# cherise215/advchain

Hardware: AMD Instinct MI355X
Metric: augmented images/sec (N adv steps, chain=noise+bias+morph+affine) (higher is better)
Workload: dtype f32

## Files before the change

advchain_amd/_lib.py:

```python
import ctypes
import os
from ctypes import c_char_p, c_double, c_float, c_int, c_int64, c_void_p

_HERE = os.path.dirname(os.path.abspath(__file__))
LIB_PATH = os.path.join(_HERE, "csrc", "libadvchain_hip.so")

_P, _I, _L, _F, _D = c_void_p, c_int, c_int64, c_float, c_double

PROTOTYPES = {
    "advchain_version": (_I, []),
    "advchain_last_error": (c_char_p, []),
    "advchain_set_deterministic": (None, [_I]),
    "advchain_get_deterministic": (_I, []),
    "advchain_grid_sample_fwd": (_I, [_P, _P, _P, _L, _L, _I, _P, _P, _I, _I, _I, _P]),
    "advchain_grid_sample_fwd_ride": (_I, [_P, _P, _P, _P, _P, _L, _L, _I, _P, _P, _I, _I, _I, _I, _P]),
    "advchain_scatter_workspace": (_L, [_L, _I, _P]),
    "advchain_grid_sample_bwd": (_I, [_P, _P, _P, _P, _P, _P, _L, _L, _I, _P, _P, _I, _I, _I, _I, _P]),
    "advchain_window_stage_workspace": (_L, [_L, _L, _I, _P]),
    "advchain_grid_sample_bwd_staged": (_I, [_P, _P, _P, _P, _P, _P, _L, _L, _I, _P, _P, _I, _I, _I, _I, _P, _P]),
    "advchain_last_bwd_route": (_I, []),
    "advchain_det_warp_workspace": (_L, [_L, _L, _I, _P]),
    "advchain_grid_sample_bwd_det": (_I, [_P, _P, _P, _P, _P, _P, _L, _L, _I, _P, _P, _I, _I, _I, _P]),
    "advchain_compose_self_fwd": (_I, [_P, _P, _P, _L, _I, _P, _I, _P, _P]),
    "advchain_compose_self_bwd": (_I, [_P, _P, _P, _P, _I, _I, _L, _I, _P, _P]),
    "advchain_affine_warp_fwd": (_I, [_P, _P, _P, _L, _L, _I, _P, _I, _I, _P]),
    "advchain_affine_warp_fwd_ride": (_I, [_P, _P, _P, _P, _P, _L, _L, _I, _P, _I, _I, _I, _P]),
    "advchain_affine_warp_bwd_workspace": (_L, [_L, _I, _P]),
    "advchain_affine_warp_bwd": (_I, [_P, _P, _P, _P, _P, _P, _L, _L, _I, _P, _I, _I, _P]),
    "advchain_affine_warp_bwd_det": (_I, [_P, _P, _P, _P, _P, _P, _P, _L, _L, _I, _P, _I, _I, _P]),
    "advchain_affine_theta_fwd": (_I, [_P, _P, _F, _P, _P, _L, _I, _P]),
    "advchain_affine_theta_bwd": (_I, [_P, _P, _F, _P, _P, _P, _L, _I, _P]),
    "advchain_tp_interp_fwd": (_I, [_P, _P, _P, _P, _P, _P, _P, _L, _L, _I, _I, _F, _P, _P, _P]),
    "advchain_tp_interp_fwd_smoothed_pair": (_I, [_P, _P, _P, _P, _P, _P, _P, _P, _L, _L, _I, _F, _P, _P, _F, _P]),
    "advchain_band_reduce_axis": (_I, [_P, _P, _P, _P, _P, _P, _P, _P, _I, _L, _L, _F, _P]),
    "advchain_band_reduce_rows_dense": (_I, [_P, _P, _P, _P, _P, _L, _L, _L, _L, _F, _P]),
    "advchain_bias_field_fwd": (_I, [_P, _P, _P, _P, _P, _P, _P, _P, _P, _L, _L, _F, _I, _F, _P]),
    "advchain_bias_field_bwd": (_I, [_P, _P, _P, _P, _P, _P, _P, _P, _P, _P, _L, _L, _F, _I, _F, _P]),
    "advchain_bias_rows_per_wg": (_I, [_P, _L]),
    "advchain_bias_field_fwd_rows": (_I, [_P, _P, _P, _P, _P, _P, _P, _P, _P, _L, _L, _F, _I, _F, _I, _P]),
    "advchain_bias_field_bwd_rows": (_I, [_P, _P, _P, _P, _P, _P, _P, _P, _P, _P, _L, _L, _F, _I, _F, _I, _P]),
    "advchain_bias_field_bwd_reduced": (_I, [_P, _P, _P, _P, _P, _P, _P, _P, _P, _P, _L, _L, _F, _I, _F, _P, _P, _L, _I, _P]),
    "advchain_gauss_axis": (_I, [_P, _P, _P, _L, _L, _I, _P, _I, _P, _I, _I, _F, _P]),
    "advchain_gauss_axis_generic": (_I, [_P, _P, _L, _I, _P, _I, _P, _I, _F, _P]),
    "advchain_max_displacement": (_I, [_P, _P, _L, _I, _P, _P]),
    "advchain_grid_sample_bicubic2d_fwd": (_I, [_P, _P, _P, _L, _L, _P, _P, _I, _P]),
    "advchain_grid_sample_bicubic2d_bwd": (_I, [_P, _P, _P, _P, _P, _L, _L, _P, _P, _I, _P]),
    "advchain_affine_grid2d_fwd": (_I, [_P, _P, _L, _P, _P]),
    "advchain_affine_grid2d_bwd_workspace": (_L, [_L, _P]),
    "advchain_affine_grid2d_bwd": (_I, [_P, _P, _P, _L, _P, _P]),
    "advchain_slot_rows_max": (_I, [_P, _P, _L, _L, _I, _P]),
    "advchain_demons_compose_pair_fwd": (_I, [_P, _P, _P, _P, _P, _P, _P, _P, _P, _P, _P, _P, _P, _L, _I, _I, _P, _P, _F, _F, _I, _P]),
    "advchain_demons_compose_pair_bwd": (_I, [_P, _P, _P, _P, _P, _P, _P, _P, _P, _P, _P, _P, _P, _P, _P, _P, _P, _L, _P, _P, _P, _L,
                                              _I, _I, _P, _F, _F, _P]),
    "advchain_bounds_check": (_I, [_P, _P, _P, _L, _P, _P]),
    "advchain_expo_chain_fused_levels": (_I, [_L, _I, _P, _I, _P]),
    "advchain_expo_chain_fwd": (_I, [_P, _P, _P, _L, _I, _P, _I, _P, _P, _P, _P]),
    "advchain_expo_chain_bwd": (_I, [_P, _P, _P, _P, _P, _P, _P, _L, _I, _P, _I, _P]),
    "advchain_gauss_xy": (_I, [_P, _P, _P, _L, _L, _I, _P, _P, _I, _I, _F, _P, _P, _L]),
    "advchain_gauss_xy_staged": (_I, [_P, _P, _P, _L, _L, _I, _P, _P, _I, _I, _F, _P, _P, _L]),
    "advchain_gauss_xy_lanes": (_I, [_P, _P, _P, _L, _L, _I, _P, _P, _I, _I, _F, _P, _P, _L, _I, _I]),
    "advchain_gauss_xy_plan": (_I, [_I, _P, _L, _P, _P, _P]),
    "advchain_gauss_small": (_I, [_P, _P, _L, _I, _P, _P, _I, _F, _P]),
    "advchain_gauss_small_pair": (_I, [_P, _P, _L, _I, _P, _P, _F, _I, _P]),
    "advchain_axpy": (_I, [_P, _P, _P, _F, _L, _P]),
    "advchain_sign_axpy": (_I, [_P, _P, _P, _F, _L, _P, _P, _P]),
    "advchain_nonzero_mask": (_I, [_P, _P, _L, _P]),
    "advchain_consistency_finish": (_I, [_P, _P, _P, _P, _I, _P]),
    "advchain_norm_workspace": (_L, [_L, _L]),
    "advchain_norm_axpy": (_I, [_P, _P, _P, _P, _F, _L, _L, _P]),
    "advchain_norm_axpy_gated": (_I, [_P, _P, _P, _P, _F, _L, _L, _P, _P, _P]),
    "advchain_update_multi": (_I, [_P, _I, _P, _P]),
    "advchain_consistency_fwd": (_I, [_P, _P, _P, _P, _P, _P, _P, _L, _L, _I, _P, _I, _I, _I, _I, _P]),
    "advchain_consistency_bwd": (_I, [_P, _P, _P, _P, _P, _P, _F, _F, _F, _F, _I, _L, _L, _I, _P, _I, _P]),
    "advchain_consistency_fused_fwd": (_I, [_P, _P, _P, _P, _P, _L, _L, _I, _P, _I, _I, _I, _I, _P]),
    "advchain_consistency_fused_bwd": (_I, [_P, _P, _P, _P, _P, _P, _F, _F, _F, _F, _I, _L, _L, _I, _P, _I, _P]),
    "advchain_consistency_wide_fwd": (_I, [_P, _P, _P, _P, _P, _P, _L, _L, _I, _P, _I, _I, _I, _I, _P]),
    "advchain_consistency_wide_bwd": (_I, [_P, _P, _P, _P, _P, _P, _P, _F, _F, _F, _F, _I, _L, _L, _I, _P, _I, _P]),
    "advchain_consistency_ref_bwd": (_I, [_P, _P, _P, _P, _P, _P, _P, _F, _F, _F, _F, _I, _L, _L, _I, _P, _I, _P]),
    "advchain_set_ref_grad_reg_max_k": (None, [_I]),
    "advchain_get_ref_grad_reg_max_k": (_I, []),
    "advchain_consistency_lp_fwd": (_I, [_P, _I, _P, _I, _P, _P, _P, _P, _L, _L, _I, _P, _I, _I, _I, _I, _P]),
    "advchain_consistency_lp_bwd": (_I, [_P, _I, _P, _I, _P, _P, _P, _P, _P, _F, _F, _F, _F, _I, _L, _L, _I, _P, _I, _P]),
    "advchain_consistency_lp_ref_bwd": (_I, [_P, _I, _P, _I, _P, _P, _P, _P, _P, _F, _F, _F, _F, _I, _L, _L, _I, _P, _I, _P]),
    "advchain_consistency_cw_fwd": (_I, [_P, _I, _P, _I, _P, _P, _P, _P, _L, _L, _I, _P, _I, _I, _I, _I, _P, _P]),
    "advchain_consistency_cw_bwd": (_I, [_P, _I, _P, _I, _P, _P, _P, _P, _P, _F, _F, _F, _F, _I, _L, _L, _I, _P, _I, _P, _P]),
    "advchain_consistency_cw_ref_bwd": (_I, [_P, _I, _P, _I, _P, _P, _P, _P, _P, _F, _F, _F, _F, _I, _L, _L, _I, _P, _I, _P, _P]),
    "advchain_consistency_fused_fwd_bf16": (_I, [_P, _P, _P, _P, _P, _L, _L, _I, _P, _P]),
    "advchain_consistency_fused_bwd_bf16": (_I, [_P, _P, _P, _P, _P, _P, _F, _F, _F, _L, _L, _I, _P, _P]),
    "advchain_seg_loss_workspace": (_L, [_L, _I, _P]),
    "advchain_ce2d_fwd": (_I, [_P, _I, _P, _P, _P, _P, _P, _P, _L, _L, _P, _F, _P]),
    "advchain_ce2d_bwd": (_I, [_P, _I, _P, _P, _P, _P, _P, _P, _P, _L, _L, _P, _F, _P]),
    "advchain_contour_fwd": (_I, [_P, _P, _P, _P, _P, _P, _P, _L, _L, _I, _P, _I, _I, _P]),
    "advchain_contour_bwd": (_I, [_P, _P, _P, _P, _L, _L, _I, _P, _I, _P]),
    "advchain_one_hot": (_I, [_P, _P, _L, _L, _L, _P]),
    "advchain_dice_workspace": (_L, [_L, _L, _I, _P]),
    "advchain_dice_fwd": (_I, [_P, _I, _P, _P, _P, _P, _P, _P, _P, _L, _L, _I, _P, _I, _F, _F, _F, _P]),
    "advchain_dice_bwd": (_I, [_P, _I, _P, _P, _P, _P, _P, _P, _P, _P, _L, _L, _I, _P, _F, _F, _P]),
    "advchain_edt": (_I, [_P, _I, _P, _I, _P, _L, _I, _P, _P]),
    "advchain_signed_maps_workspace": (_L, [_L, _L, _I, _P]),
    "advchain_signed_maps": (_I, [_P, _P, _P, _P, _L, _L, _I, _P, _P]),
    "advchain_surface_metrics_workspace": (_L, [_L, _L, _I, _P]),
    "advchain_surface_metrics": (_I, [_P, _P, _P, _D, _P, _P, _P, _P, _P, _P, _P, _P, _P, _L, _L, _I, _P, _P]),
    "advchain_surface_dice_route": (_I, [_L, _L, _I, _P, _P, _D, _I]),
    "advchain_surface_dice_workspace": (_L, [_L, _L, _I, _P, _P, _D, _I]),
    "advchain_surface_dice": (_I, [_P, _P, _P, _P, _D, _I, _P, _P, _P, _P, _L, _L, _I, _P, _P]),
    "advchain_components_workspace": (_L, [_L, _I, _P]),
    "advchain_components": (_I, [_P, _P, _P, _P, _P, _L, _I, _P, _I, _L, _L, _P]),
    "advchain_keep_largest": (_I, [_P, _P, _P, _P, _L, _L, _I, _P, _I, _L, _P]),
    "advchain_remove_small": (_I, [_P, _P, _P, _L, _I, _P, _I, _L, _L, _L, _P]),
    "advchain_fill_holes_workspace": (_L, [_L, _I, _P]),
    "advchain_fill_holes": (_I, [_P, _P, _P, _P, _P, _P, _L, _L, _I, _P, _I, _L, _L, _P]),
    "advchain_instance_match_workspace": (_L, [_L, _I, _P]),
    "advchain_instance_match": (_I, [_P] * 14 + [_L, _L, _I, _P, _I, _L, _D, _P]),
    "advchain_betti_workspace": (_L, [_L, _I, _P]),
    "advchain_betti": (_I, [_P, _P, _P, _P, _P, _P, _L, _L, _I, _P, _I, _P]),
    "advchain_morph_workspace": (_L, [_I, _L, _L, _I, _P]),
    "advchain_morph": (_I, [_P, _P, _D, _I, _P, _P, _L, _L, _L, _I, _P, _P]),
    "advchain_boundary_workspace": (_L, [_L, _L, _I, _P]),
    "advchain_boundary_fwd": (_I, [_P, _I, _P, _P, _P, _P, _P, _P, _L, _L, _I, _P, _I, _P]),
    "advchain_boundary_bwd": (_I, [_P, _I, _P, _P, _P, _P, _P, _P, _L, _L, _I, _P, _I, _P]),
    "advchain_image_diff2d_fwd": (_I, [_P, _P, _P, _L, _L, _P, _P]),
    "advchain_image_diff2d_bwd": (_I, [_P, _P, _P, _L, _L, _P, _P]),
    "advchain_jacobian_det2d_fwd": (_I, [_P, _P, _L, _P, _P]),
    "advchain_jacobian_det2d_bwd": (_I, [_P, _P, _P, _L, _P, _P]),
    "advchain_expo_start": (_I, [_P, _P, _F, _L, _I, _P, _P]),
    "advchain_image_diff3d_fwd": (_I, [_P, _P, _P, _P, _L, _L, _P, _P]),
    "advchain_image_diff3d_bwd": (_I, [_P, _P, _P, _P, _L, _L, _P, _P]),
    "advchain_jacobian_det_fwd": (_I, [_P, _P, _L, _I, _P, _I, _P]),
    "advchain_jacobian_det_bwd": (_I, [_P, _P, _P, _P, _L, _I, _P, _I, _P]),
    "advchain_jacobian_det_workspace": (_L, [_L, _I, _P]),
    "advchain_jacobian_stats_workspace": (_L, [_L, _I, _P]),
    "advchain_jacobian_stats": (_I, [_P, _P, _P, _P, _P, _P, _L, _I, _P, _I, _P]),
    "advchain_sumsq_ordered": (_I, [_P, _L, _P, _P, _P]),
    "advchain_bicubic2d_det_workspace": (_L, [_L, _L, _P]),
    "advchain_grid_sample_bicubic2d_bwd_det": (_I, [_P, _P, _P, _P, _P, _P, _L, _L, _P, _P, _I, _P]),
    "advchain_tp_interp_sumsq_partials": (_L, [_P, _L]),
    "advchain_tp_interp_sumsq_ordered": (_I, [_P, _P, _P, _P, _P, _P, _L, _L, _P, _P, _P]),
    "advchain_consistency_fwd_partials": (_L, [_L, _L, _I, _P, _I, _I, _I]),
    "advchain_consistency_fwd_ord": (_I, [_P, _P, _P, _P, _P, _P, _P, _L, _P, _L, _L, _I, _P, _I, _I, _I, _I, _P]),
    "advchain_consistency_fused_fwd_partials": (_L, [_L, _L, _I, _P, _I, _I, _I, _I]),
    "advchain_consistency_fused_fwd_ord": (_I, [_P, _P, _P, _P, _P, _L, _P, _L, _L, _I, _P, _I, _I, _I, _I, _P]),
    "advchain_consistency_wide_fwd_partials": (_L, [_L, _L, _I, _P, _I, _I]),
    "advchain_consistency_wide_fwd_ord": (_I, [_P, _P, _P, _P, _P, _P, _L, _P, _L, _L, _I, _P, _I, _I, _I, _I, _P]),
    "advchain_consistency_lp_fwd_partials": (_L, [_L, _L, _I, _P, _I]),
    "advchain_consistency_lp_fwd_ord": (_I, [_P, _I, _P, _I, _P, _P, _P, _P, _L, _P, _L, _L, _I, _P, _I, _I, _I, _I, _P, _P]),
    "advchain_consistency_finish_ord": (_I, [_P, _L, _P, _P, _P, _P, _P]),
}

class UpdateDesc(ctypes.Structure):
    _fields_ = [("base", c_void_p), ("x", c_void_p), ("out", c_void_p), ("old", c_void_p), ("N", c_int64), ("M", c_int64),
                ("kind", ctypes.c_int32), ("step", c_float)]


_lib = None


class AdvchainHipError(RuntimeError):
    pass


class _Lib(object):

    def __init__(self, cdll):
        self._cdll = cdll
        self._raw = {}
        self.records = []

    def _bind(self, name, res, args):
        fn = getattr(self._cdll, name)
        fn.restype = res
        fn.argtypes = args
        self._raw[name] = fn
        setattr(self, name, fn)

    def timed(self, names=None, every=1):
        import contextlib
        import torch

        @contextlib.contextmanager
        def ctx():
            chosen = [n for n in self._raw if (names is None or n in names) and self._raw[n].restype is c_int
                      and len(self._raw[n].argtypes) > 0]
            for n in chosen:
                raw = self._raw[n]

                count = [0]

                def wrapped(*a, _raw=raw, _n=n, _count=count):
                    _count[0] += 1
                    if _count[0] % every:
                        return _raw(*a)
                    e0 = torch.cuda.Event(enable_timing=True)
                    e1 = torch.cuda.Event(enable_timing=True)
                    e0.record()
                    rc = _raw(*a)
                    e1.record()
                    self.records.append((_n, a, e0, e1))
                    return rc
                setattr(self, n, wrapped)
            try:
                yield self
            finally:
                for n in chosen:
                    setattr(self, n, self._raw[n])
        return ctx()


def load():
    global _lib
    if _lib is not None:
        return _lib
    if not os.path.exists(LIB_PATH):
        raise AdvchainHipError(
            "libadvchain_hip.so not found at %s -- build it with `python -m advchain_amd.build` "
            "(there is no CPU / PyTorch fallback for the advchain_amd kernels)" % LIB_PATH)
    import torch
    tl = os.path.join(os.path.dirname(torch.__file__), "lib", "libamdhip64.so")
    if os.path.exists(tl):
        ctypes.CDLL(tl, mode=ctypes.RTLD_GLOBAL)
    lib = _Lib(ctypes.CDLL(LIB_PATH))
    for name, (res, args) in PROTOTYPES.items():
        lib._bind(name, res, args)
    _lib = lib
    return lib


def check(rc, what):
    if rc != 0:
        msg = load().advchain_last_error()
        raise AdvchainHipError("%s failed (rc=%d): %s" % (what, rc, msg.decode() if msg else ""))


_DIMS = {}


def dims_array(dims):
    key = tuple(dims)
    arr = _DIMS.get(key)
    if arr is None:
        arr = _DIMS[key] = (c_int64 * len(key))(*[int(d) for d in key])
    return arr


def float_array(vals):
    return (c_float * len(vals))(*[float(v) for v in vals])
```

advchain_amd/csrc/fields.hip:

```cpp
#include "sampler_common.h"

namespace advchain {

constexpr int kBandMax = 8;

struct BandAxis {
  const int* start;
  const float* w;
  const int* lo;
  const int* hi;
  int S, g, B;
};
struct BandTables { BandAxis a[3]; };

__device__ __forceinline__ void decode3(int v, const Dims& d, int& i0, int& i1, int& i2) {
  i2 = v % d.s2;
  const int r = v / d.s2;
  i1 = r % d.s1;
  i0 = r / d.s1;
}

__device__ __forceinline__ float tp_eval(const float* __restrict__ coef, const BandTables& T, int i0, int i1, int i2) {
  const BandAxis& A0 = T.a[0];
  const BandAxis& A1 = T.a[1];
  const BandAxis& A2 = T.a[2];
  const int s0 = A0.start[i0], s1 = A1.start[i1], s2 = A2.start[i2];
  const float* w0 = A0.w + i0 * A0.B;
  const float* w1 = A1.w + i1 * A1.B;
  const float* w2 = A2.w + i2 * A2.B;
  float acc = 0.f;
  for (int a = 0; a < A0.B; ++a) {
    float acc1 = 0.f;
    for (int b = 0; b < A1.B; ++b) {
      const float* row = coef + ((int64_t)(s0 + a) * A1.g + (s1 + b)) * A2.g + s2;
      float acc2 = 0.f;
      for (int c = 0; c < A2.B; ++c) acc2 += row[c] * w2[c];
      acc1 += acc2 * w1[b];
    }
    acc += acc1 * w0[a];
  }
  return acc;
}

constexpr int kTpChunk = 32;
constexpr int kTpMaxLds = 2048;

struct TpGeom { int XT, ROWS; };

__host__ __device__ inline TpGeom tp_geom(int S2) {
  TpGeom g;
  (void)S2;
  g.XT = 64;
  g.ROWS = kBlock / g.XT;
  return g;
}

template <int VEC, class Epi>
__device__ __forceinline__ void tp_rows(const float* __restrict__ coef, const BandTables& T, const Dims& full, int i0,
                                        int i1_begin, int i1_end, float* lds, Epi&& epi) {
  const BandAxis& A0 = T.a[0];
  const BandAxis& A1 = T.a[1];
  const BandAxis& A2 = T.a[2];
  const int ncol = full.s2 / VEC;
  int XT = 64;
  if (VEC > 1) { XT = 1; while (XT < ncol && XT < 64) XT *= 2; }
  const int ROWS = kBlock / XT;
  const int tx = threadIdx.x % XT, ry = threadIdx.x / XT;
  const int g2 = A2.g;
  __shared__ int s1_s[kTpChunk];
  __shared__ float w1_s[kTpChunk * kBandMax];
  const int nrow = i1_end - i1_begin;
  for (int e = threadIdx.x; e < nrow * (A1.B + 1); e += kBlock) {
    const int r = e / (A1.B + 1), b = e - r * (A1.B + 1);
    if (b == 0) s1_s[r] = A1.start[i1_begin + r];
    else w1_s[r * kBandMax + b - 1] = A1.w[(i1_begin + r) * A1.B + b - 1];
  }
  const int s0 = A0.start[i0];
  const float* w0 = A0.w + i0 * A0.B;
  int s2f[VEC];
  float w2f[VEC][kBandMax];
#pragma unroll
  for (int q = 0; q < VEC; ++q) {
    const int col = min(tx * VEC + q, full.s2 - 1);
    s2f[q] = A2.start[col];
#pragma unroll
    for (int c = 0; c < kBandMax; ++c) w2f[q][c] = c < A2.B ? A2.w[col * A2.B + c] : 0.f;
  }
  __syncthreads();
  const int RPP = max(1, min(kTpChunk, kTpMaxLds / max(g2, 1)));
  for (int base = i1_begin; base < i1_end; base += RPP) {
    for (int e = threadIdx.x; e < RPP * g2; e += kBlock) {
      const int r = e / g2, k = e - r * g2;
      const int i1 = base + r;
      float acc = 0.f;
      if (i1 < i1_end) {
        const int s1 = s1_s[i1 - i1_begin];
        const float* w1 = w1_s + (i1 - i1_begin) * kBandMax;
        if (A0.B == 2 && A1.B == 2) {
          const float* cb = coef + ((int64_t)s0 * A1.g + s1) * g2 + k;
          const float c00 = cb[0], c01 = cb[g2], c10 = cb[(int64_t)A1.g * g2], c11 = cb[(int64_t)A1.g * g2 + g2];
          const float u0 = w1[0], u1 = w1[1], v0 = w0[0], v1 = w0[1];
          acc += v0 * (0.f + u0 * c00 + u1 * c01);
          acc += v1 * (0.f + u0 * c10 + u1 * c11);
        } else {
          for (int a = 0; a < A0.B; ++a) {
            float acc1 = 0.f;
            for (int b = 0; b < A1.B; ++b) acc1 += w1[b] * coef[((int64_t)(s0 + a) * A1.g + (s1 + b)) * g2 + k];
            acc += w0[a] * acc1;
          }
        }
      }
      lds[e] = acc;
    }
    __syncthreads();
    for (int xg = tx; xg < ncol; xg += XT) {
      int s2[VEC];
      float w2[VEC][kBandMax];
#pragma unroll
      for (int q = 0; q < VEC; ++q) {
        if (xg == tx) {
          s2[q] = s2f[q];
#pragma unroll
          for (int c = 0; c < kBandMax; ++c) w2[q][c] = w2f[q][c];
        } else {
          s2[q] = A2.start[xg * VEC + q];
#pragma unroll
          for (int c = 0; c < kBandMax; ++c) w2[q][c] = c < A2.B ? A2.w[(xg * VEC + q) * A2.B + c] : 0.f;
        }
      }
      for (int r = ry; r < RPP; r += ROWS) {
        const int i1 = base + r;
        if (i1 >= i1_end) break;
        float val[VEC];
#pragma unroll
        for (int q = 0; q < VEC; ++q) {
          float v = 0.f;
#pragma unroll
          for (int c = 0; c < kBandMax; ++c)
            if (c < A2.B) v += w2[q][c] * lds[r * g2 + s2[q] + c];
          val[q] = v;
        }
        epi(i1, xg * VEC, val);
      }
    }
    __syncthreads();
  }
}

struct SumsqOrdered {};
template <class... ORD>
__device__ __forceinline__ void tp_sumsq_put(float* __restrict__ sumsq, float v) {
  if constexpr (sizeof...(ORD) == 0)
    atomic_add_f32(sumsq + (blockIdx.x + blockIdx.y * 3u + blockIdx.z * 7u) % kSumSlots, v);
  else
    sumsq[((int64_t)blockIdx.z * gridDim.y + blockIdx.y) * gridDim.x + blockIdx.x] = v;
}
static __global__ void __launch_bounds__(kBlock) k_tp_partials_sum(const float* __restrict__ partials, int64_t nb, float* __restrict__ out) {
  __shared__ float smem[4];
  float v[1] = {0.f};
  for (int64_t i = threadIdx.x; i < nb; i += kBlock) v[0] += partials[i];
  block_sum<1>(v, smem);
  if (threadIdx.x == 0) out[0] = v[0];
}

template <int VEC, class... ORD>
__global__ void __launch_bounds__(kBlock)
k_tp_interp_fwd(const float* __restrict__ coef, float* __restrict__ out, BandTables T, Dims full, int C,
                int add_identity, float scale, float* __restrict__ sumsq, float* __restrict__ disp_out) {
  __shared__ float lds[kTpMaxLds];
  __shared__ float smem[4];
  const int plane = blockIdx.z, i0 = blockIdx.y;
  const int i1b = blockIdx.x * kTpChunk, i1e = min(i1b + kTpChunk, full.s1);
  const int64_t G = (int64_t)T.a[0].g * T.a[1].g * T.a[2].g;
  const int V = (int)full.voxels();
  const int c = plane % C;
  float sq[1] = {0.f};
  float dmax = 0.f;
  const float to_vox = fabsf(scale) * 0.5f * (float)((c == 0 ? full.s2 : (c == 1 ? full.s1 : full.s0)) - 1);
  tp_rows<VEC>(coef + (int64_t)plane * G, T, full, i0, i1b, i1e, lds, [&](int i1, int x, const float (&val)[VEC]) {
    float o[VEC];
#pragma unroll
    for (int q = 0; q < VEC; ++q) {
      sq[0] += val[q] * val[q];
      dmax = fmaxf(dmax, fabsf(val[q]));
      float base = 0.f;
      if (add_identity) base = c == 0 ? lin_coord(x + q, full.s2) : (c == 1 ? lin_coord(i1, full.s1) : lin_coord(i0, full.s0));
      o[q] = base + scale * val[q];
    }
    if (out) store_vec<VEC>(out + (int64_t)plane * V + ((int64_t)i0 * full.s1 + i1) * full.s2 + x, o);
  });
  if (disp_out) wave_max_to_slots(fminf(dmax * to_vox, 1.0e9f), disp_out);
  if (sumsq) {
    block_sum<1>(sq, smem);
    if (threadIdx.x == 0) tp_sumsq_put<ORD...>(sumsq, sq[0]);
  }
}

constexpr int kGsFuseMax = 1024;
struct GaussW9 { float w[9]; };
template <int VEC>
__global__ void __launch_bounds__(kBlock)
k_tp_interp_fwd_gs(const float* __restrict__ vel, float* __restrict__ s1, float* __restrict__ out, BandTables T, Dims full, int C,
                   int add_identity, float scale, float* __restrict__ disp_out, GaussW9 gw, float gscale, int P) {
  __shared__ float lds[kTpMaxLds];
  __shared__ float gs[2][kGsFuseMax];
  const int plane = blockIdx.z, i0 = blockIdx.y;
  const int i1b = blockIdx.x * kTpChunk, i1e = min(i1b + kTpChunk, full.s1);
  const int g1 = T.a[1].g, g2 = T.a[2].g, Vg = g1 * g2;
  const int V = (int)full.voxels();
  const int c = plane % C;
  {
    const float* src = vel + (int64_t)(plane % P) * Vg;
    const float sc = plane >= P ? -gscale : gscale;
    for (int i = threadIdx.x; i < Vg; i += kBlock) gs[0][i] = src[i] * sc;
    __syncthreads();
    int cur = 0;
#pragma unroll
    for (int pass = 0; pass < 2; ++pass) {
      const int Sa = pass == 0 ? g2 : g1, st = pass == 0 ? 1 : g2;
      for (int i = threadIdx.x; i < Vg; i += kBlock) {
        const int ia = (i / st) % Sa;
        float acc = 0.f;
#pragma unroll
        for (int k = -4; k <= 4; ++k) {
          const int j = ia + k;
          if (j >= 0 && j < Sa) acc += gw.w[k + 4] * gs[cur][i + k * st];
        }
        gs[cur ^ 1][i] = acc;
      }
      __syncthreads();
      cur ^= 1;
    }
    if (s1 && blockIdx.x == 0 && blockIdx.y == 0)
      for (int i = threadIdx.x; i < Vg; i += kBlock) s1[(int64_t)plane * Vg + i] = gs[0][i];
  }
  float dmax = 0.f;
  const float to_vox = fabsf(scale) * 0.5f * (float)((c == 0 ? full.s2 : (c == 1 ? full.s1 : full.s0)) - 1);
  tp_rows<VEC>(gs[0], T, full, i0, i1b, i1e, lds, [&](int i1, int x, const float (&val)[VEC]) {
    float o[VEC];
#pragma unroll
    for (int q = 0; q < VEC; ++q) {
      dmax = fmaxf(dmax, fabsf(val[q]));
      float base = 0.f;
      if (add_identity) base = c == 0 ? lin_coord(x + q, full.s2) : (c == 1 ? lin_coord(i1, full.s1) : lin_coord(i0, full.s0));
      o[q] = base + scale * val[q];
    }
    store_vec<VEC>(out + (int64_t)plane * V + ((int64_t)i0 * full.s1 + i1) * full.s2 + x, o);
  });
  if (disp_out) wave_max_to_slots(fminf(dmax * to_vox, 1.0e9f), disp_out);
}

constexpr int kTpZB = 4;
template <int VEC, class... ORD>
__global__ void __launch_bounds__(kBlock)
k_tp_interp_fwd_planes(const float* __restrict__ coef, float* __restrict__ out, BandTables T, Dims full, int C, int add_identity,
                       float scale, float* __restrict__ sumsq, float* __restrict__ disp_out) {
  __shared__ float lds[2][kTpMaxLds];
  __shared__ int s1_s[kTpChunk], s0_s[kTpZB];
  __shared__ float w1_s[kTpChunk * 2], w0_s[kTpZB * 2];
  __shared__ float smem[4];
  const BandAxis& A0 = T.a[0];
  const BandAxis& A1 = T.a[1];
  const BandAxis& A2 = T.a[2];
  const int plane = blockIdx.z;
  const int z0 = blockIdx.y * kTpZB, z1 = min(z0 + kTpZB, full.s0);
  const int i1b = blockIdx.x * kTpChunk, i1e = min(i1b + kTpChunk, full.s1);
  const int64_t G = (int64_t)A0.g * A1.g * A2.g;
  const int V = (int)full.voxels();
  const int c = plane % C;
  const float* cf = coef + (int64_t)plane * G;
  const int g2 = A2.g, nrow = i1e - i1b, NE = nrow * g2;
  constexpr int EPT = kTpMaxLds / kBlock;
  const int ncol = full.s2 / VEC;
  int XT = 64;
  if (VEC > 1) { XT = 1; while (XT < ncol && XT < 64) XT *= 2; }
  const int ROWS = kBlock / XT;
  const int tx = threadIdx.x % XT, ry = threadIdx.x / XT;
  for (int e = threadIdx.x; e < nrow * 3; e += kBlock) {
    const int r = e / 3, b = e - r * 3;
    if (b == 0) s1_s[r] = A1.start[i1b + r];
    else w1_s[r * 2 + b - 1] = A1.w[(i1b + r) * 2 + b - 1];
  }
  if (threadIdx.x < (z1 - z0) * 3) {
    const int r = threadIdx.x / 3, b = threadIdx.x - r * 3;
    if (b == 0) s0_s[r] = A0.start[z0 + r];
    else w0_s[r * 2 + b - 1] = A0.w[(z0 + r) * 2 + b - 1];
  }
  int s2f[VEC];
  float w2f[VEC][2];
#pragma unroll
  for (int q = 0; q < VEC; ++q) {
    const int col = min(tx * VEC + q, full.s2 - 1);
    s2f[q] = A2.start[col];
    w2f[q][0] = A2.w[col * 2];
    w2f[q][1] = A2.w[col * 2 + 1];
  }
  __syncthreads();
  float cc[EPT][4];
  auto request = [&](int zi) {
    const int s0 = s0_s[zi];
#pragma unroll
    for (int j = 0; j < EPT; ++j) {
      if (j * kBlock >= NE) break;
      const int e = min(threadIdx.x + j * kBlock, NE - 1);
      const int r = e / g2, k = e - r * g2;
      const float* cb = cf + ((int64_t)s0 * A1.g + s1_s[r]) * g2 + k;
      cc[j][0] = cb[0]; cc[j][1] = cb[g2]; cc[j][2] = cb[(int64_t)A1.g * g2]; cc[j][3] = cb[(int64_t)A1.g * g2 + g2];
    }
  };
  auto blend = [&](int zi, float* dst) {
    const float v0 = w0_s[zi * 2], v1 = w0_s[zi * 2 + 1];
#pragma unroll
    for (int j = 0; j < EPT; ++j) {
      const int e = threadIdx.x + j * kBlock;
      if (e >= NE) continue;
      const int r = e / g2;
      const float u0 = w1_s[r * 2], u1 = w1_s[r * 2 + 1];
      float acc = 0.f;
      acc += v0 * (0.f + u0 * cc[j][0] + u1 * cc[j][1]);
      acc += v1 * (0.f + u0 * cc[j][2] + u1 * cc[j][3]);
      dst[e] = acc;
    }
  };
  float sq[1] = {0.f};
  float dmax = 0.f;
  const bool track = sumsq != nullptr || disp_out != nullptr;
  const float to_vox = fabsf(scale) * 0.5f * (float)((c == 0 ? full.s2 : (c == 1 ? full.s1 : full.s0)) - 1);
  request(0);
  blend(0, lds[0]);
  __syncthreads();
  for (int zi = 0; zi < z1 - z0; ++zi) {
    const int i0 = z0 + zi;
    const float* cur = lds[zi & 1];
    const bool more = zi + 1 < z1 - z0;
    if (more) request(zi + 1);
    for (int xg = tx; xg < ncol; xg += XT) {
      int s2[VEC];
      float w2[VEC][2];
#pragma unroll
      for (int q = 0; q < VEC; ++q) {
        if (xg == tx) { s2[q] = s2f[q]; w2[q][0] = w2f[q][0]; w2[q][1] = w2f[q][1]; }
        else { s2[q] = A2.start[xg * VEC + q]; w2[q][0] = A2.w[(xg * VEC + q) * 2]; w2[q][1] = A2.w[(xg * VEC + q) * 2 + 1]; }
      }
      float basex[VEC];
#pragma unroll
      for (int q = 0; q < VEC; ++q) basex[q] = (add_identity && c == 0) ? lin_coord(xg * VEC + q, full.s2) : 0.f;
      const float basez = (add_identity && c == 2) ? lin_coord(i0, full.s0) : 0.f;
      float* orow = out ? out + (int64_t)plane * V + ((int64_t)i0 * full.s1 + i1b) * full.s2 + xg * VEC : nullptr;
      for (int r = ry; r < nrow; r += ROWS) {
        const float basey = (add_identity && c == 1) ? lin_coord(i1b + r, full.s1) : basez;
        const float* lr = cur + r * g2;
        float o[VEC];
#pragma unroll
        for (int q = 0; q < VEC; ++q) {
          float v = 0.f;
          v += w2[q][0] * lr[s2[q]];
          v += w2[q][1] * lr[s2[q] + 1];
          if (track) {
            sq[0] += v * v;
            dmax = fmaxf(dmax, fabsf(v));
          }
          o[q] = (c == 0 ? basex[q] : basey) + scale * v;
        }
        if (out) store_vec<VEC>(orow + r * full.s2, o);
      }
    }
    if (more) blend(zi + 1, lds[(zi + 1) & 1]);
    __syncthreads();
  }
  if (disp_out) wave_max_to_slots(fminf(dmax * to_vox, 1.0e9f), disp_out);
  if (sumsq) {
    block_sum<1>(sq, smem);
    if (threadIdx.x == 0) tp_sumsq_put<ORD...>(sumsq, sq[0]);
  }
}

constexpr int kBrMaxW = 4096;

__device__ __forceinline__ int stage_band(const BandAxis& A, float* Wd, int* lo_s) {
  const int lane = threadIdx.x & 63;
  if (A.g > 64) return 0;
  int WB = lane < A.g ? A.hi[lane] - A.lo[lane] : 0;
#pragma unroll
  for (int o = 32; o > 0; o >>= 1) WB = max(WB, __shfl_xor(WB, o, 64));
  if (A.g * WB > kBrMaxW) return 0;
  for (int i = threadIdx.x; i < A.g * WB; i += blockDim.x) {
    const int k = i / WB, j = i - k * WB;
    const int s2 = A.lo[k] + j;
    float w = 0.f;
    if (s2 < A.hi[k]) {
      const int b = k - A.start[s2];
      if (b >= 0 && b < A.B) w = A.w[s2 * A.B + b];
    }
    Wd[i] = w;
  }
  for (int i = threadIdx.x; i < A.g; i += blockDim.x) lo_s[i] = A.lo[i];
  __syncthreads();
  return WB;
}

__global__ void __launch_bounds__(kBlock)
k_band_reduce_axis(const float* __restrict__ in, const float* __restrict__ in2, float* __restrict__ out, int64_t outer,
                   int inner, BandAxis A, float scale) {
  __shared__ float Wd[kBrMaxW];
  __shared__ int lo_s[64];
  const int WB = stage_band(A, Wd, lo_s);
  const int64_t t = (int64_t)blockIdx.x * kBlock + threadIdx.x;
  const int64_t total = outer * A.g * inner;
  if (t >= total) return;
  const int i = (int)(t % inner);
  const int64_t r = t / inner;
  const int k = (int)(r % A.g);
  const int64_t o = r / A.g;
  const float* p = in + (o * A.S) * inner + i;
  const float* p2 = in2 ? in2 + (o * A.S) * inner + i : nullptr;
  float acc = 0.f;
  if (WB > 0) {
    const int lo = lo_s[k];
    const int len = min(WB, A.S - lo);
    const float* w = Wd + k * WB;
    for (int j = 0; j < len; ++j) {
      float x = p[(int64_t)(lo + j) * inner];
      if (p2) x -= p2[(int64_t)(lo + j) * inner];
      acc = fmaf(x, w[j], acc);
    }
  } else {
    const int lo = A.lo[k], hi = A.hi[k];
    for (int s = lo; s < hi; ++s) {
      const int b = k - A.start[s];
      if (b >= 0 && b < A.B) {
        float x = p[(int64_t)s * inner];
        if (p2) x -= p2[(int64_t)s * inner];
        acc += x * A.w[s * A.B + b];
      }
    }
  }
  out[t] = acc * scale;
}

constexpr int kBrSlabFloats = 12288;
__global__ void __launch_bounds__(kBlock)
k_band_reduce_axis_slab(const float* __restrict__ in, const float* __restrict__ in2, float* __restrict__ out, int inner, int IC,
                        BandAxis A, float scale) {
  extern __shared__ __attribute__((aligned(16))) float slab[];
  __shared__ float Wd[kBrMaxW];
  __shared__ int lo_s[64];
  const int64_t o = blockIdx.x;
  const int c0 = blockIdx.y * IC, cols = min(IC, inner - c0);
  const int q = cols >> 2, n4 = A.S * q, pitch = IC + 1;
  const float* p = in + o * (int64_t)A.S * inner + c0;
  const float* p2 = in2 ? in2 + o * (int64_t)A.S * inner + c0 : nullptr;
  constexpr int U = 4;
  float4 v[U];
  auto fetch = [&](int idx) -> float4 {
    const int e = min(idx, n4 - 1);
    const int sr = e / q, x4 = e - sr * q;
    float4 a = *reinterpret_cast<const float4*>(p + (int64_t)sr * inner + 4 * x4);
    if (p2) {
      const float4 b = *reinterpret_cast<const float4*>(p2 + (int64_t)sr * inner + 4 * x4);
      a.x -= b.x; a.y -= b.y; a.z -= b.z; a.w -= b.w;
    }
    return a;
  };
  auto put = [&](int idx, const float4& a) {
    if (idx >= n4) return;
    const int sr = idx / q, x4 = idx - sr * q;
    float* dst = slab + sr * pitch + 4 * x4;
    dst[0] = a.x; dst[1] = a.y; dst[2] = a.z; dst[3] = a.w;
  };
#pragma unroll
  for (int u = 0; u < U; ++u) v[u] = fetch(threadIdx.x + u * kBlock);
  const int WB = stage_band(A, Wd, lo_s);
#pragma unroll
  for (int u = 0; u < U; ++u) put(threadIdx.x + u * kBlock, v[u]);
  for (int i0 = threadIdx.x + U * kBlock; i0 < n4; i0 += U * kBlock) {
#pragma unroll
    for (int u = 0; u < U; ++u) v[u] = fetch(i0 + u * kBlock);
#pragma unroll
    for (int u = 0; u < U; ++u) put(i0 + u * kBlock, v[u]);
  }
  __syncthreads();
  for (int t = threadIdx.x; t < A.g * cols; t += kBlock) {
    const int k = t / cols, i = t - k * cols;
    float acc = 0.f;
    if (WB > 0) {
      const int lo = lo_s[k];
      const int len = min(WB, A.S - lo);
      const float* w = Wd + k * WB;
      const float* x = slab + lo * pitch + i;
      for (int j = 0; j < len; ++j) acc = fmaf(x[j * pitch], w[j], acc);
    } else {
      const int lo = A.lo[k], hi = A.hi[k];
      for (int sr = lo; sr < hi; ++sr) {
        const int b = k - A.start[sr];
        if (b >= 0 && b < A.B) acc += slab[sr * pitch + i] * A.w[sr * A.B + b];
      }
    }
    out[(o * A.g + k) * (int64_t)inner + c0 + i] = acc * scale;
  }
}

constexpr int kBrThreads = 128;
template <int KG>
__global__ void __launch_bounds__(kBrThreads)
k_band_reduce_rows(const float* __restrict__ in, const float* __restrict__ in2, float* __restrict__ out, int64_t rows,
                   BandAxis A, float scale, int iters) {
  extern __shared__ __attribute__((aligned(16))) float slabs[];
  __shared__ float Wd[kBrMaxW];
  __shared__ int lo_s[64];
  constexpr int RW = 64 / KG, NWV = kBrThreads / 64;
  const int lane = threadIdx.x & 63, wave = threadIdx.x >> 6;
  const int S = A.S, g = A.g, B = A.B;
  const int WB = stage_band(A, Wd, lo_s);
  const bool dense = WB > 0;
  const int q = S >> 2;
  const int pitch = S + 1;
  float* my = slabs + wave * RW * pitch;
  const int r = lane % RW, kg = lane / RW;
  for (int it = 0; it < iters; ++it) {
    const int64_t base = (((int64_t)blockIdx.x * iters + it) * NWV + wave) * RW;
    __syncthreads();
    for (int idx = lane; idx < RW * q; idx += 64) {
      const int rr = idx / q, x4 = idx - rr * q;
      const int64_t gr = base + rr;
      float4 v = make_float4(0.f, 0.f, 0.f, 0.f);
      if (gr < rows) {
        v = *reinterpret_cast<const float4*>(in + gr * S + 4 * x4);
        if (in2) {
          const float4 u = *reinterpret_cast<const float4*>(in2 + gr * S + 4 * x4);
          v = make_float4(v.x - u.x, v.y - u.y, v.z - u.z, v.w - u.w);
        }
      }
      float* dst = my + rr * pitch + 4 * x4;
      dst[0] = v.x; dst[1] = v.y; dst[2] = v.z; dst[3] = v.w;
    }
    __syncthreads();
    const int64_t gr = base + r;
    if (gr < rows) {
      const float* x = my + r * pitch;
      if (dense) {
        for (int k0 = kg; k0 < g; k0 += 2 * KG) {
          const int k1 = k0 + KG;
          const bool two = k1 < g;
          const int lo0 = lo_s[k0], lo1 = lo_s[two ? k1 : k0];
          const float* w0 = Wd + k0 * WB;
          const float* w1 = Wd + (two ? k1 : k0) * WB;
          float a0 = 0.f, a1 = 0.f;
          int j = 0;
          for (; j + 8 <= WB; j += 8) {
            float x0[8], x1[8], c0[8], c1[8];
#pragma unroll
            for (int u = 0; u < 8; ++u) {
              x0[u] = x[min(lo0 + j + u, S - 1)]; c0[u] = w0[j + u];
              x1[u] = x[min(lo1 + j + u, S - 1)]; c1[u] = w1[j + u];
            }
#pragma unroll
            for (int u = 0; u < 8; ++u) { a0 = fmaf(x0[u], c0[u], a0); a1 = fmaf(x1[u], c1[u], a1); }
          }
          for (; j < WB; ++j) {
            a0 = fmaf(x[min(lo0 + j, S - 1)], w0[j], a0);
            a1 = fmaf(x[min(lo1 + j, S - 1)], w1[j], a1);
          }
          out[gr * g + k0] = a0 * scale;
          if (two) out[gr * g + k1] = a1 * scale;
        }
      } else
      for (int k = kg; k < g; k += KG) {
        const int lo = A.lo[k];
        float acc = 0.f;
        {
          for (int s2 = lo; s2 < A.hi[k]; ++s2) {
            const int b = k - A.start[s2];
            if (b >= 0 && b < B) acc = fmaf(x[s2], A.w[s2 * B + b], acc);
          }
        }
        out[gr * g + k] = acc * scale;
      }
    }
  }
}

template <int KG>
__global__ void __launch_bounds__(kBrThreads)
k_band_reduce_rows_dense(const float* __restrict__ in, const float* __restrict__ in2, float* __restrict__ out, int64_t rows,
                         const float* __restrict__ wd, const int* __restrict__ lo_g, int S, int g, int WB, float scale, int iters) {
  extern __shared__ __attribute__((aligned(16))) float slabs[];
  __shared__ int lo_s[64];
  constexpr int RW = 64 / KG, NWV = kBrThreads / 64;
  constexpr int QMAX = 8;
  const int lane = threadIdx.x & 63, wave = threadIdx.x >> 6;
  const int q = S >> 2;
  const int pitch = S + 1;
  float* my = slabs + wave * RW * pitch;
  float* Wd = slabs + NWV * RW * pitch;
  const int r = lane % RW, kg = lane / RW;
  const int nq = RW * q;
  float4 v[QMAX];
  auto request = [&](int it) {
    const int64_t base = (((int64_t)blockIdx.x * iters + it) * NWV + wave) * RW;
#pragma unroll
    for (int u = 0; u < QMAX; ++u) {
      const int idx = lane + 64 * u;
      const int rr = idx / q, x4 = idx - rr * q;
      const int64_t gr = base + rr;
      const bool ok = idx < nq && gr < rows;
      const int64_t off = ok ? gr * S + 4 * x4 : 0;
      float4 a = *reinterpret_cast<const float4*>(in + off);
      if (in2) {
        const float4 b = *reinterpret_cast<const float4*>(in2 + off);
        a = make_float4(a.x - b.x, a.y - b.y, a.z - b.z, a.w - b.w);
      }
      v[u] = ok ? a : make_float4(0.f, 0.f, 0.f, 0.f);
    }
  };
  request(0);
  for (int i = threadIdx.x; i < g * WB; i += kBrThreads) Wd[i] = wd[i];
  if (threadIdx.x < g) lo_s[threadIdx.x] = lo_g[threadIdx.x];
  for (int it = 0; it < iters; ++it) {
    const int64_t base = (((int64_t)blockIdx.x * iters + it) * NWV + wave) * RW;
    if (it > 0) __syncthreads();
#pragma unroll
    for (int u = 0; u < QMAX; ++u) {
      const int idx = lane + 64 * u;
      if (idx >= nq) continue;
      const int rr = idx / q, x4 = idx - rr * q;
      float* dst = my + rr * pitch + 4 * x4;
      dst[0] = v[u].x; dst[1] = v[u].y; dst[2] = v[u].z; dst[3] = v[u].w;
    }
    __syncthreads();
    if (it + 1 < iters) request(it + 1);
    const int64_t gr = base + r;
    if (gr < rows) {
      const float* x = my + r * pitch;
      for (int k0 = kg; k0 < g; k0 += 2 * KG) {
        const int k1 = k0 + KG;
        const bool two = k1 < g;
        const int lo0 = lo_s[k0], lo1 = lo_s[two ? k1 : k0];
        const float* w0 = Wd + k0 * WB;
        const float* w1 = Wd + (two ? k1 : k0) * WB;
        float a0 = 0.f, a1 = 0.f;
        int j = 0;
        for (; j + 8 <= WB; j += 8) {
          float x0[8], x1[8], c0[8], c1[8];
#pragma unroll
          for (int u = 0; u < 8; ++u) {
            x0[u] = x[min(lo0 + j + u, S - 1)]; c0[u] = w0[j + u];
            x1[u] = x[min(lo1 + j + u, S - 1)]; c1[u] = w1[j + u];
          }
#pragma unroll
          for (int u = 0; u < 8; ++u) { a0 = fmaf(x0[u], c0[u], a0); a1 = fmaf(x1[u], c1[u], a1); }
        }
        for (; j < WB; ++j) {
          a0 = fmaf(x[min(lo0 + j, S - 1)], w0[j], a0);
          a1 = fmaf(x[min(lo1 + j, S - 1)], w1[j], a1);
        }
        out[gr * g + k0] = a0 * scale;
        if (two) out[gr * g + k1] = a1 * scale;
      }
    }
  }
}

__device__ __forceinline__ float bias_value(float L, int use_log, float eps, float& e, bool& pass) {
  e = use_log ? expf(L) : 1.f + L;
  const float b = e - 1.f;
  pass = (b >= -eps) && (b <= eps);
  return 1.f + fminf(fmaxf(b, -eps), eps);
}

template <int VEC>
__global__ void __launch_bounds__(kBlock)
k_bias_fwd(const float* __restrict__ cp, const float* __restrict__ data, float* __restrict__ out,
           float* __restrict__ field, BandTables T, Dims full, int C, float eps, int use_log, float cp_scale, int rows) {
  __shared__ float lds[kTpMaxLds];
  const int n = blockIdx.z, i0 = blockIdx.y;
  const int i1b = blockIdx.x * rows, i1e = min(i1b + rows, full.s1);
  const int64_t G = (int64_t)T.a[0].g * T.a[1].g * T.a[2].g;
  const int V = (int)full.voxels();
  tp_rows<VEC>(cp + (int64_t)n * G, T, full, i0, i1b, i1e, lds, [&](int i1, int x, const float (&val)[VEC]) {
    const int v = (i0 * full.s1 + i1) * full.s2 + x;
    float b[VEC];
#pragma unroll
    for (int q = 0; q < VEC; ++q) {
      float e;
      bool pass;
      b[q] = bias_value(cp_scale * val[q], use_log, eps, e, pass);
    }
    store_vec<VEC>(field + (int64_t)n * V + v, b);
    if (data) {
      for (int c = 0; c < C; ++c) {
        const int64_t o = ((int64_t)n * C + c) * V + v;
        float dv[VEC];
        load_vec<VEC>(data + o, dv);
#pragma unroll
        for (int q = 0; q < VEC; ++q) dv[q] *= b[q];
        store_vec<VEC>(out + o, dv);
      }
    }
  });
}

constexpr int kBiasRedWq = kBrMaxW / 4 / kBlock;
template <int VEC, bool RED>
__global__ void __launch_bounds__(kBlock)
k_bias_bwd(const float* __restrict__ cp, const float* __restrict__ data, const float* __restrict__ gout,
           float* __restrict__ gL, float* __restrict__ gdata, BandTables T, Dims full, int C, float eps, int use_log,
           float cp_scale, int rows, float* __restrict__ t1, const float* __restrict__ wd, const int* __restrict__ lo_g, int WB) {
  __shared__ float lds[kTpMaxLds];
  extern __shared__ __attribute__((aligned(16))) float red_lds[];
  __shared__ int lo_s[64];
  const int n = blockIdx.z, i0 = blockIdx.y;
  const int i1b = blockIdx.x * rows, i1e = min(i1b + rows, full.s1);
  const int64_t G = (int64_t)T.a[0].g * T.a[1].g * T.a[2].g;
  const int V = (int)full.voxels();
  const int g2 = T.a[2].g;
  const int nw = RED ? g2 * WB : 0;
  const int pitch = full.s2 + 1;
  float* Wd = red_lds;
  float* slab = red_lds + ((nw + 3) & ~3);
  const bool wvec = (nw & 3) == 0 && (reinterpret_cast<uintptr_t>(wd) & 15) == 0;
  float4 wq[kBiasRedWq];
  int lo_r = 0;
  if constexpr (RED) {
#pragma unroll
    for (int u = 0; u < kBiasRedWq; ++u) {
      const int idx = threadIdx.x + kBlock * u;
      wq[u] = wvec && 4 * idx < nw ? *reinterpret_cast<const float4*>(wd + 4 * idx) : make_float4(0.f, 0.f, 0.f, 0.f);
    }
    if (threadIdx.x < g2) lo_r = lo_g[threadIdx.x];
  }
  tp_rows<VEC>(cp + (int64_t)n * G, T, full, i0, i1b, i1e, lds, [&](int i1, int x, const float (&val)[VEC]) {
    const int v = (i0 * full.s1 + i1) * full.s2 + x;
    float b[VEC], e[VEC], sgo[VEC];
    bool pass[VEC];
#pragma unroll
    for (int q = 0; q < VEC; ++q) {
      b[q] = bias_value(cp_scale * val[q], use_log, eps, e[q], pass[q]);
      sgo[q] = 0.f;
    }
    for (int c = 0; c < C; ++c) {
      const int64_t o = ((int64_t)n * C + c) * V + v;
      float go[VEC], dv[VEC];
      load_vec<VEC>(gout + o, go);
      load_vec<VEC>(data + o, dv);
#pragma unroll
      for (int q = 0; q < VEC; ++q) { sgo[q] += go[q] * dv[q]; go[q] *= b[q]; }
      if (gdata) store_vec<VEC>(gdata + o, go);
    }
    if (RED || gL) {
      float gl[VEC];
#pragma unroll
      for (int q = 0; q < VEC; ++q) gl[q] = pass[q] ? sgo[q] * (use_log ? e[q] : 1.f) * cp_scale : 0.f;
      if constexpr (RED) {
        float* dst = slab + (i1 - i1b) * pitch + x;
#pragma unroll
        for (int q = 0; q < VEC; ++q) dst[q] = gl[q];
      } else {
        store_vec<VEC>(gL + (int64_t)n * V + v, gl);
      }
    }
  });
  if constexpr (RED) {
    if (wvec) {
#pragma unroll
      for (int u = 0; u < kBiasRedWq; ++u) {
        const int idx = threadIdx.x + kBlock * u;
        if (4 * idx < nw) *reinterpret_cast<float4*>(Wd + 4 * idx) = wq[u];
      }
    } else {
      for (int i = threadIdx.x; i < nw; i += kBlock) Wd[i] = wd[i];
    }
    if (threadIdx.x < g2) lo_s[threadIdx.x] = lo_r;
    __syncthreads();
    const int nrow = i1e - i1b, S2 = full.s2;
    for (int e = threadIdx.x; e < nrow * g2; e += kBlock) {
      const int r = e % nrow, k = e / nrow;
      const float* x = slab + r * pitch;
      const float* w = Wd + k * WB;
      const int lo = lo_s[k];
      float a = 0.f;
      int j = 0;
      for (; j + 16 <= WB; j += 16) {
        float xv[16], cv[16];
#pragma unroll
        for (int u = 0; u < 16; ++u) { xv[u] = x[min(lo + j + u, S2 - 1)]; cv[u] = w[j + u]; }
#pragma unroll
        for (int u = 0; u < 16; ++u) a = fmaf(xv[u], cv[u], a);
      }
      for (; j < WB; ++j) a = fmaf(x[min(lo + j, S2 - 1)], w[j], a);
      t1[(((int64_t)n * full.s0 + i0) * full.s1 + i1b + r) * g2 + k] = a;
    }
  }
}

struct GaussW { float w[9]; };

__device__ __forceinline__ float border_identity(float pos, int S, float& slope) {
  float mult;
  const float x = source_index<PAD_BORDER>(pos, S, mult);
  const float f = floorf(x);
  const int i0 = (int)f;
  const int i1 = min(i0 + 1, S - 1);
  const float a = lin_coord(i0, S), b = lin_coord(i1, S);
  slope = mult * (b - a);
  return ((f + 1.f) - x) * a + (x - f) * b;
}

template <int PRE, int POST>
__global__ void __launch_bounds__(kBlock)
k_gauss_axis(const float* __restrict__ in, float* __restrict__ out, const float* __restrict__ aux, int64_t total,
             Dims d, int C, int axis, GaussW gw, float scale) {
  const int64_t t = (int64_t)blockIdx.x * kBlock + threadIdx.x;
  if (t >= total) return;
  const int V = (int)d.voxels();
  const int plane = (int)(t / V);
  const int v = (int)(t - (int64_t)plane * V);
  int idx[3];
  decode3(v, d, idx[0], idx[1], idx[2]);
  const int S[3] = {d.s0, d.s1, d.s2};
  const int stride = axis == 2 ? 1 : (axis == 1 ? d.s2 : d.s1 * d.s2);
  const int c = plane % C;
  const int caxis = 2 - c;
  const int ia = idx[axis];
  float tap[9];
#pragma unroll
  for (int k = -4; k <= 4; ++k) {
    const int jc = min(max(ia + k, 0), S[axis] - 1);
    tap[k + 4] = in[t + (int64_t)(jc - ia) * stride];
  }
  float acc = 0.f;
#pragma unroll
  for (int k = -4; k <= 4; ++k) {
    const int j = ia + k;
    float x = tap[k + 4];
    if (PRE == 1) x *= scale;
    if (PRE == 2) {
      const int ci = (caxis == axis) ? j : idx[caxis];
      float slope;
      x = border_identity(x, S[caxis], slope) - lin_coord(ci, S[caxis]);
    }
    acc += (j >= 0 && j < S[axis]) ? gw.w[k + 4] * x : 0.f;
  }
  if (POST == 1) acc += lin_coord(idx[caxis], S[caxis]);
  if (POST == 2) {
    float slope;
    border_identity(aux[t], S[caxis], slope);
    acc *= slope;
  }
  out[t] = acc;
}

template <int PRE, int POST, int AXIS>
__global__ void __launch_bounds__(kBlock)
k_gauss_axis_v4(const float* __restrict__ in, float* __restrict__ out, const float* __restrict__ aux, int64_t total4,
                Dims d, int C, GaussW gw, float scale, int row_in_wave) {
  const int64_t t4 = (int64_t)blockIdx.x * kBlock + threadIdx.x;
  int64_t t;
  if (AXIS == 2 && row_in_wave == 2) {
    const int q = d.s2 >> 2, rpw = 64 / q;
    const int lane = (int)(t4 & 63);
    const int rl = lane / q;
    const int64_t row = (t4 >> 6) * rpw + rl;
    if (rl >= rpw || row >= total4 / q) return;
    t = row * d.s2 + (lane - rl * q) * 4;
  } else {
    if (t4 >= total4) return;
    t = t4 * 4;
  }
  const int V = (int)d.voxels();
  const int plane = (int)(t / V);
  const int v = (int)(t - (int64_t)plane * V);
  int idx[3];
  decode3(v, d, idx[0], idx[1], idx[2]);
  const int S[3] = {d.s0, d.s1, d.s2};
  const int c = plane % C;
  const int caxis = 2 - c;
  auto pre = [&](float x, int i0, int i1, int i2) -> float {
    if (PRE == 1) return x * scale;
    if (PRE == 2) {
      const int ci = caxis == 2 ? i2 : (caxis == 1 ? i1 : i0);
      float slope;
      return border_identity(x, S[caxis], slope) - lin_coord(ci, S[caxis]);
    }
    return x;
  };
  float acc[4] = {0.f, 0.f, 0.f, 0.f};
  if (AXIS == 2 && row_in_wave) {
    const float4 q = *reinterpret_cast<const float4*>(in + t);
    float win[12];
    win[4] = pre(q.x, idx[0], idx[1], idx[2]);
    win[5] = pre(q.y, idx[0], idx[1], idx[2] + 1);
    win[6] = pre(q.z, idx[0], idx[1], idx[2] + 2);
    win[7] = pre(q.w, idx[0], idx[1], idx[2] + 3);
    const bool first = idx[2] == 0, last = idx[2] + 4 >= d.s2;
#pragma unroll
    for (int k = 0; k < 4; ++k) {
      const float pv = lane_prev_f(win[4 + k]), nx = lane_next_f(win[4 + k]);
      win[k] = first ? 0.f : pv;
      win[8 + k] = last ? 0.f : nx;
    }
#pragma unroll
    for (int o = 0; o < 4; ++o)
#pragma unroll
      for (int k = 0; k < 9; ++k) acc[o] += gw.w[k] * win[o + k];
  } else if (AXIS == 2) {
    float win[12];
    float4 qb[3];
#pragma unroll
    for (int b = 0; b < 3; ++b) {
      const int x0 = idx[2] + (b - 1) * 4;
      qb[b] = *reinterpret_cast<const float4*>(in + t + ((x0 >= 0 && x0 < d.s2) ? (b - 1) * 4 : 0));
    }
#pragma unroll
    for (int b = 0; b < 3; ++b) {
      const int x0 = idx[2] + (b - 1) * 4;
      const bool inr = x0 >= 0 && x0 < d.s2;
      win[b * 4 + 0] = inr ? pre(qb[b].x, idx[0], idx[1], x0) : 0.f;
      win[b * 4 + 1] = inr ? pre(qb[b].y, idx[0], idx[1], x0 + 1) : 0.f;
      win[b * 4 + 2] = inr ? pre(qb[b].z, idx[0], idx[1], x0 + 2) : 0.f;
      win[b * 4 + 3] = inr ? pre(qb[b].w, idx[0], idx[1], x0 + 3) : 0.f;
    }
#pragma unroll
    for (int o = 0; o < 4; ++o)
#pragma unroll
      for (int k = 0; k < 9; ++k) acc[o] += gw.w[k] * win[o + k];
  } else {
    const int stride = AXIS == 1 ? d.s2 : d.s1 * d.s2;
    const int ia = idx[AXIS];
    float4 q[9];
#pragma unroll
    for (int k = -4; k <= 4; ++k) {
      const int jc = min(max(ia + k, 0), S[AXIS] - 1);
      q[k + 4] = *reinterpret_cast<const float4*>(in + t + (int64_t)(jc - ia) * stride);
    }
#pragma unroll
    for (int k = -4; k <= 4; ++k) {
      const int j = ia + k;
      const bool inr = j >= 0 && j < S[AXIS];
      const int j0 = AXIS == 0 ? j : idx[0], j1 = AXIS == 1 ? j : idx[1];
      const float w = gw.w[k + 4];
      acc[0] += inr ? w * pre(q[k + 4].x, j0, j1, idx[2]) : 0.f;
      acc[1] += inr ? w * pre(q[k + 4].y, j0, j1, idx[2] + 1) : 0.f;
      acc[2] += inr ? w * pre(q[k + 4].z, j0, j1, idx[2] + 2) : 0.f;
      acc[3] += inr ? w * pre(q[k + 4].w, j0, j1, idx[2] + 3) : 0.f;
    }
  }
  if (POST == 1) {
#pragma unroll
    for (int o = 0; o < 4; ++o) acc[o] += lin_coord(caxis == 2 ? idx[2] + o : idx[caxis], S[caxis]);
  }
  if (POST == 2) {
    const float4 a = *reinterpret_cast<const float4*>(aux + t);
    const float av[4] = {a.x, a.y, a.z, a.w};
#pragma unroll
    for (int o = 0; o < 4; ++o) {
      float slope;
      border_identity(av[o], S[caxis], slope);
      acc[o] *= slope;
    }
  }
  *reinterpret_cast<float4*>(out + t) = make_float4(acc[0], acc[1], acc[2], acc[3]);
}

template <int PRE, int POST>
__global__ void __launch_bounds__(kBlock)
k_gauss_xy(const float* __restrict__ in, float* __restrict__ out, const float* __restrict__ aux, Dims d, int C, GaussW gw,
           float scale, int TY, const float* __restrict__ in_hi, int planes_lo) {
  extern __shared__ float gx_lds[];
  const int W = d.s2, Q = W >> 2, PA = W + 8;
  const int R = TY + 8;
  float* A = gx_lds;
  float* B = gx_lds + R * PA;
  const int plane = blockIdx.z, iz = blockIdx.y;
  const int y0 = blockIdx.x * TY;
  const int caxis = 2 - plane % C;
  const int Sc = caxis == 2 ? d.s2 : (caxis == 1 ? d.s1 : d.s0);
  const int64_t base = ((int64_t)plane * d.s0 + iz) * d.s1 * (int64_t)W;
  const float* src = (in_hi && plane >= planes_lo) ? in_hi + (((int64_t)(plane - planes_lo) * d.s0 + iz) * d.s1 * (int64_t)W) : in + base;
  for (int e = threadIdx.x; e < R * 2; e += kBlock)
    *reinterpret_cast<float4*>(A + (e >> 1) * PA + ((e & 1) ? W + 4 : 0)) = make_float4(0.f, 0.f, 0.f, 0.f);
  for (int e = threadIdx.x; e < R * Q; e += kBlock) {
    const int r = e / Q, q = e - r * Q;
    const int gy = y0 - 4 + r;
    const bool inr = gy >= 0 && gy < d.s1;
    const float4 v = *reinterpret_cast<const float4*>(src + (int64_t)min(max(gy, 0), d.s1 - 1) * W + 4 * q);
    float t[4] = {v.x, v.y, v.z, v.w};
#pragma unroll
    for (int o = 0; o < 4; ++o) {
      if (PRE == 1) t[o] *= scale;
      if (PRE == 2) {
        float sl;
        t[o] = border_identity(t[o], Sc, sl) - lin_coord(caxis == 2 ? 4 * q + o : (caxis == 1 ? gy : iz), Sc);
      }
      if (!inr) t[o] = 0.f;
    }
    *reinterpret_cast<float4*>(A + r * PA + 4 + 4 * q) = make_float4(t[0], t[1], t[2], t[3]);
  }
  __syncthreads();
  for (int e = threadIdx.x; e < R * Q; e += kBlock) {
    const int r = e / Q, q = e - r * Q;
    const float* a = A + r * PA + 4 * q;
    const float4 a0 = *reinterpret_cast<const float4*>(a), a1 = *reinterpret_cast<const float4*>(a + 4),
                 a2 = *reinterpret_cast<const float4*>(a + 8);
    const float win[12] = {a0.x, a0.y, a0.z, a0.w, a1.x, a1.y, a1.z, a1.w, a2.x, a2.y, a2.z, a2.w};
    float acc[4] = {0.f, 0.f, 0.f, 0.f};
#pragma unroll
    for (int o = 0; o < 4; ++o)
#pragma unroll
      for (int k = 0; k < 9; ++k) acc[o] += gw.w[k] * win[o + k];
    *reinterpret_cast<float4*>(B + r * W + 4 * q) = make_float4(acc[0], acc[1], acc[2], acc[3]);
  }
  __syncthreads();
  for (int e = threadIdx.x; e < TY * Q; e += kBlock) {
    const int ry = e / Q, q = e - ry * Q;
    const int gy = y0 + ry;
    if (gy >= d.s1) continue;
    float acc[4] = {0.f, 0.f, 0.f, 0.f};
#pragma unroll
    for (int k = 0; k < 9; ++k) {
      const float4 b = *reinterpret_cast<const float4*>(B + (ry + k) * W + 4 * q);
      acc[0] += gw.w[k] * b.x; acc[1] += gw.w[k] * b.y; acc[2] += gw.w[k] * b.z; acc[3] += gw.w[k] * b.w;
    }
    const int64_t off = base + (int64_t)gy * W + 4 * q;
    if (POST == 1) {
#pragma unroll
      for (int o = 0; o < 4; ++o) acc[o] += lin_coord(caxis == 2 ? 4 * q + o : (caxis == 1 ? gy : iz), Sc);
    }
    if (POST == 2) {
      const float4 a4 = *reinterpret_cast<const float4*>(aux + off);
      const float av[4] = {a4.x, a4.y, a4.z, a4.w};
#pragma unroll
      for (int o = 0; o < 4; ++o) {
        float slope;
        border_identity(av[o], Sc, slope);
// ... 136 lines not shown
  for (int j0 = ja; j0 < jb; j0 += U) {
    float4 nw[U];
#pragma unroll
    for (int u = 0; u < U; ++u) nw[u] = fetch(j0 + 4 + u);
#pragma unroll
    for (int u = 0; u < U; ++u) w[8 + u] = prep(nw[u], j0 + 4 + u);
#pragma unroll
    for (int u = 0; u < U; ++u) {
      const int j = j0 + u;
      if (j >= jb) break;
      float acc[4] = {0.f, 0.f, 0.f, 0.f};
#pragma unroll
      for (int k = 0; k < 9; ++k) {
        acc[0] += gw.w[k] * w[u + k].x;
        acc[1] += gw.w[k] * w[u + k].y;
        acc[2] += gw.w[k] * w[u + k].z;
        acc[3] += gw.w[k] * w[u + k].w;
      }
      if (POST == 1) {
#pragma unroll
        for (int o = 0; o < 4; ++o) acc[o] += lin_coord(caxis == 2 ? ix + o : (caxis == 1 ? iy : j), Sc);
      }
      if (POST == 2) {
        const float4 a = *reinterpret_cast<const float4*>(ax + (int64_t)j * stride);
        const float av[4] = {a.x, a.y, a.z, a.w};
#pragma unroll
        for (int o = 0; o < 4; ++o) {
          float slope;
          border_identity(av[o], Sc, slope);
          acc[o] *= slope;
        }
      }
      *reinterpret_cast<float4*>(dst + (int64_t)j * stride) = make_float4(acc[0], acc[1], acc[2], acc[3]);
    }
#pragma unroll
    for (int k = 0; k < 8; ++k) w[k] = w[U + k];
  }
}

constexpr int kGaussSmallMax = 4096;

template <int NT>
__global__ void __launch_bounds__(NT)
k_gauss_small(const float* __restrict__ in, float* __restrict__ out, Dims d, int ndim, GaussW gw, float scale, int mirror,
              int P) {
  __shared__ float buf[2][kGaussSmallMax];
  const int V = (int)d.voxels();
  const int S[3] = {d.s0, d.s1, d.s2};
  const int stride[3] = {d.s1 * d.s2, d.s2, 1};
  const int b = blockIdx.x;
  float first[(kGaussSmallMax + NT - 1) / NT];
  const int rounds = mirror == 2 ? 2 : 1;
  for (int round = 0; round < rounds; ++round) {
    const float* src = in + (int64_t)(mirror == 1 ? b % P : b + round * P) * V;
    const float sc = (mirror == 1 && b >= P) ? -scale : scale;
    if (round) __syncthreads();
    for (int i = threadIdx.x; i < V; i += NT) buf[0][i] = src[i] * sc;
    __syncthreads();
    int cur = 0;
    for (int pass = 0; pass < ndim; ++pass) {
      const int axis = 2 - pass;
      const int Sa = S[axis], st = stride[axis];
      for (int i = threadIdx.x; i < V; i += NT) {
        const int ia = (i / st) % Sa;
        float acc = 0.f;
#pragma unroll
        for (int k = -4; k <= 4; ++k) {
          const int j = ia + k;
          if (j >= 0 && j < Sa) acc += gw.w[k + 4] * buf[cur][i + k * st];
        }
        buf[cur ^ 1][i] = acc;
      }
      __syncthreads();
      cur ^= 1;
    }
    float* dst = out + (int64_t)b * V;
    if (mirror != 2) {
      for (int i = threadIdx.x; i < V; i += NT) dst[i] = buf[cur][i];
    } else if (round == 0) {
#pragma unroll
      for (int q = 0; q < (kGaussSmallMax + NT - 1) / NT; ++q) {
        const int i = threadIdx.x + q * NT;
        first[q] = i < V ? buf[cur][i] : 0.f;
      }
    } else {
#pragma unroll
      for (int q = 0; q < (kGaussSmallMax + NT - 1) / NT; ++q) {
        const int i = threadIdx.x + q * NT;
        if (i < V) dst[i] = first[q] - buf[cur][i];
      }
    }
  }
}

__global__ void __launch_bounds__(kBlock)
k_axpy(const float* __restrict__ x, const float* __restrict__ y, float* __restrict__ out, float a, int64_t n4,
       int64_t n) {
  const int64_t i = (int64_t)blockIdx.x * kBlock + threadIdx.x;
  if (i < n4) {
    const float4 p = reinterpret_cast<const float4*>(y)[i];
    float4 q = x ? reinterpret_cast<const float4*>(x)[i] : make_float4(0.f, 0.f, 0.f, 0.f);
    q.x += a * p.x; q.y += a * p.y; q.z += a * p.z; q.w += a * p.w;
    reinterpret_cast<float4*>(out)[i] = q;
  }
  const int64_t j = n4 * 4 + i;
  if (j < n) out[j] = (x ? x[j] : 0.f) + a * y[j];
}

__global__ void __launch_bounds__(kBlock)
k_sign_axpy(const float* __restrict__ base, const float* __restrict__ x, float* __restrict__ out, float a, int64_t n,
            const float* __restrict__ gate, const float* __restrict__ old) {
  const int64_t i = (int64_t)blockIdx.x * kBlock + threadIdx.x;
  if (i >= n) return;
  if (gate && !(fabsf(gate[0]) <= 3.0e38f)) { out[i] = old[i]; return; }
  const float v = x[i];
  const float sg = v > 0.f ? 1.f : (v < 0.f ? -1.f : v);
  out[i] = (base ? base[i] : 0.f) + a * sg;
}

__global__ void __launch_bounds__(kBlock)
k_nonzero_mask(const float* __restrict__ x, float* __restrict__ out, int64_t n) {
  const int64_t i = (int64_t)blockIdx.x * kBlock + threadIdx.x;
  if (i < n) out[i] = x[i] != 0.f ? 1.f : 0.f;
}

__global__ void __launch_bounds__(kBlock)
k_sumsq_partial(const float* __restrict__ x, float* __restrict__ partial, int64_t M, int chunk) {
  __shared__ float smem[4];
  const int n = blockIdx.y, b = blockIdx.x;
  const float* xn = x + (int64_t)n * M;
  const int64_t lo = (int64_t)b * chunk, hi = min(lo + chunk, M);
  float s[1] = {0.f};
  for (int64_t i = lo + threadIdx.x; i < hi; i += kBlock) { const float q = xn[i]; s[0] += q * q; }
  block_sum<1>(s, smem);
  if (threadIdx.x == 0) partial[(int64_t)n * gridDim.x + b] = s[0];
}

__global__ void __launch_bounds__(kBlock)
k_norm_axpy(const float* __restrict__ base, const float* __restrict__ x, const float* __restrict__ partial,
            int nb, float step, float* __restrict__ out, int64_t M, int chunk, const float* __restrict__ gate,
            const float* __restrict__ old) {
  __shared__ float smem[4];
  __shared__ float inv_s;
  const int n = blockIdx.y, b = blockIdx.x;
  float s[1] = {0.f};
  for (int i = threadIdx.x; i < nb; i += kBlock) s[0] += partial[(int64_t)n * nb + i];
  block_sum<1>(s, smem);
  if (threadIdx.x == 0) inv_s = step / (sqrtf(s[0]) + 1e-20f);
  __syncthreads();
  const float inv = inv_s;
  const int64_t lo = (int64_t)b * chunk, hi = min(lo + chunk, M);
  const int64_t off = (int64_t)n * M;
  if (gate && !(fabsf(gate[0]) <= 3.0e38f)) {
    for (int64_t i = lo + threadIdx.x; i < hi; i += kBlock) out[off + i] = old[off + i];
    return;
  }
  for (int64_t i = lo + threadIdx.x; i < hi; i += kBlock) out[off + i] = (base ? base[off + i] : 0.f) + inv * x[off + i];
}

__global__ void __launch_bounds__(kBlock)
k_norm_axpy_row(const float* __restrict__ base, const float* __restrict__ x, float step, float* __restrict__ out, int64_t M,
                const float* __restrict__ gate, const float* __restrict__ old) {
  __shared__ float smem[4];
  __shared__ float inv_s;
  const int64_t off = (int64_t)blockIdx.x * M;
  float s[1] = {0.f};
  for (int64_t i = threadIdx.x; i < M; i += kBlock) { const float q = x[off + i]; s[0] += q * q; }
  block_sum<1>(s, smem);
  if (threadIdx.x == 0) inv_s = step / (sqrtf(s[0]) + 1e-20f);
  __syncthreads();
  const float inv = inv_s;
  if (gate && !(fabsf(gate[0]) <= 3.0e38f)) {
    for (int64_t i = threadIdx.x; i < M; i += kBlock) out[off + i] = old[off + i];
    return;
  }
  for (int64_t i = threadIdx.x; i < M; i += kBlock) out[off + i] = (base ? base[off + i] : 0.f) + inv * x[off + i];
}

struct UpdDesc {
  const float* base;
  const float* x;
  float* out;
  const float* old;
  long long M;
  int rows, kind, block0;
  float step;
};
constexpr int kUpdMax = 8;
struct UpdPack {
  UpdDesc d[kUpdMax];
  int n;
};

__global__ void __launch_bounds__(1024) k_update_multi(UpdPack p, const float* __restrict__ gate) {
  __shared__ float wsum[16];
  __shared__ float inv_s;
  int i = 0;
#pragma unroll
  for (int k = 1; k < kUpdMax; ++k)
    if (k < p.n && (int)blockIdx.x >= p.d[k].block0) i = k;
  const UpdDesc u = p.d[i];
  const long long off = (long long)((int)blockIdx.x - u.block0) * u.M;
  const float* __restrict__ x = u.x + off;
  const float* __restrict__ base = u.base ? u.base + off : nullptr;
  float* __restrict__ out = u.out + off;
  const int tid = threadIdx.x;
  if (gate && !(fabsf(gate[0]) <= 3.0e38f)) {
    for (long long j = tid; j < u.M; j += 1024) out[j] = u.old[off + j];
    return;
  }
  if (u.kind == 1) {
    for (long long j = tid; j < u.M; j += 1024) {
      const float v = x[j];
      const float sg = v > 0.f ? 1.f : (v < 0.f ? -1.f : v);
      out[j] = (base ? base[j] : 0.f) + u.step * sg;
    }
    return;
  }
  const bool al = ((reinterpret_cast<uintptr_t>(x) | reinterpret_cast<uintptr_t>(out) | reinterpret_cast<uintptr_t>(base)) & 15) == 0 &&
                  (u.M & 3) == 0;
  constexpr int UB = 8;
  float s = 0.f;
  if (al) {
    const long long M4 = u.M >> 2;
    for (long long j0 = tid; j0 < M4; j0 += (long long)UB * 1024) {
      float4 q[UB];
#pragma unroll
      for (int k = 0; k < UB; ++k) {
        const long long j = j0 + (long long)k * 1024;
        q[k] = reinterpret_cast<const float4*>(x)[j < M4 ? j : M4 - 1];
      }
#pragma unroll
      for (int k = 0; k < UB; ++k)
        if (j0 + (long long)k * 1024 < M4) s += (q[k].x * q[k].x + q[k].y * q[k].y) + (q[k].z * q[k].z + q[k].w * q[k].w);
    }
  } else {
    for (long long j = tid; j < u.M; j += 1024) { const float q = x[j]; s += q * q; }
  }
#pragma unroll
  for (int o = 32; o > 0; o >>= 1) s += __shfl_xor(s, o, 64);
  if ((tid & 63) == 0) wsum[tid >> 6] = s;
  __syncthreads();
  if (tid == 0) {
    float t = 0.f;
#pragma unroll
    for (int w = 0; w < 16; ++w) t += wsum[w];
    inv_s = u.step / (sqrtf(t) + 1e-20f);
  }
  __syncthreads();
  const float inv = inv_s;
  if (al) {
    const long long M4 = u.M >> 2;
    for (long long j0 = tid; j0 < M4; j0 += (long long)UB * 1024) {
      float4 q[UB], b[UB];
#pragma unroll
      for (int k = 0; k < UB; ++k) {
        const long long j = j0 + (long long)k * 1024, jc = j < M4 ? j : M4 - 1;
        q[k] = reinterpret_cast<const float4*>(x)[jc];
        b[k] = base ? reinterpret_cast<const float4*>(base)[jc] : make_float4(0.f, 0.f, 0.f, 0.f);
      }
#pragma unroll
      for (int k = 0; k < UB; ++k) {
        const long long j = j0 + (long long)k * 1024;
        if (j < M4)
          reinterpret_cast<float4*>(out)[j] = make_float4(b[k].x + inv * q[k].x, b[k].y + inv * q[k].y, b[k].z + inv * q[k].z,
                                                          b[k].w + inv * q[k].w);
      }
    }
  } else {
    for (long long j = tid; j < u.M; j += 1024) out[j] = (base ? base[j] : 0.f) + inv * x[j];
  }
}

}

using namespace advchain;

struct advchain_update_desc {
  const float* base;
  const float* x;
  float* out;
  const float* old;
  int64_t N;
  int64_t M;
  int32_t kind;
  float step;
};

static bool unpack_tables(const int32_t* itab, const float* ftab, const int64_t* S, const int64_t* g, const int64_t* B,
                          BandTables& T) {
  const int32_t* ip = itab;
  const float* fp = ftab;
  for (int a = 0; a < 3; ++a) {
    if (S[a] < 1 || g[a] < 1 || B[a] < 1 || B[a] > kBandMax || B[a] > g[a]) return false;
    T.a[a].S = (int)S[a]; T.a[a].g = (int)g[a]; T.a[a].B = (int)B[a];
    T.a[a].start = ip; ip += S[a];
    T.a[a].lo = ip; ip += g[a];
    T.a[a].hi = ip; ip += g[a];
    T.a[a].w = fp; fp += S[a] * B[a];
  }
  return true;
}

template <class... ORD>
static int tp_interp_fwd_launch(const float* coef, float* out, const int32_t* itab, const float* ftab,
                                const int64_t* S, const int64_t* g, const int64_t* B, int64_t planes, int64_t C, int add_identity,
                                float scale, float* sumsq, float* disp_out, int64_t* nwg, void* stream) {
  ADVCHAIN_CHECK_ARG(coef && itab && ftab && (out || sumsq), "tp_interp_fwd: null pointer");
  ADVCHAIN_CHECK_ARG(planes >= 0 && planes < 65536 && C >= 1 && S[0] < 65536, "tp_interp_fwd: bad planes/C");
  BandTables T;
  ADVCHAIN_CHECK_ARG(unpack_tables(itab, ftab, S, g, B, T), "tp_interp_fwd: bad band tables");
  *nwg = 0;
  if (planes == 0) return ADVCHAIN_OK;
  Dims full{(int)S[0], (int)S[1], (int)S[2]};
  ADVCHAIN_CHECK_ARG(full.voxels() < (1ll << 31), "tp_interp_fwd: volume too large");
  ADVCHAIN_CHECK_ARG(T.a[2].g <= kTpMaxLds, "tp_interp_fwd: coefficient row too long");
  dim3 grid((unsigned)((full.s1 + kTpChunk - 1) / kTpChunk), (unsigned)full.s0, (unsigned)planes);
  if (full.s0 >= 2 * kTpZB && T.a[0].B == 2 && T.a[1].B == 2 && T.a[2].B == 2 && kTpChunk * T.a[2].g <= kTpMaxLds) {
    dim3 gp(grid.x, (unsigned)((full.s0 + kTpZB - 1) / kTpZB), (unsigned)planes);
    *nwg = (int64_t)gp.x * gp.y * gp.z;
    if (full.s2 % 4 == 0 && (full.s2 >= 128 || full.s2 % 64 != 0) && (reinterpret_cast<uintptr_t>(out) & 15) == 0)
      hipLaunchKernelGGL((k_tp_interp_fwd_planes<4, ORD...>), gp, dim3(kBlock), 0, (hipStream_t)stream, coef, out, T, full, (int)C, add_identity,
                         scale, sumsq, disp_out);
    else
      hipLaunchKernelGGL((k_tp_interp_fwd_planes<1, ORD...>), gp, dim3(kBlock), 0, (hipStream_t)stream, coef, out, T, full, (int)C, add_identity,
                         scale, sumsq, disp_out);
    ADVCHAIN_LAUNCH_CHECK();
    return ADVCHAIN_OK;
  }
  *nwg = (int64_t)grid.x * grid.y * grid.z;
  if (full.s2 % 4 == 0 && full.s2 >= 128 && (reinterpret_cast<uintptr_t>(out) & 15) == 0)
    hipLaunchKernelGGL((k_tp_interp_fwd<4, ORD...>), grid, dim3(kBlock), 0, (hipStream_t)stream, coef, out, T, full, (int)C,
                       add_identity, scale, sumsq, disp_out);
  else
    hipLaunchKernelGGL((k_tp_interp_fwd<1, ORD...>), grid, dim3(kBlock), 0, (hipStream_t)stream, coef, out, T, full, (int)C,
                       add_identity, scale, sumsq, disp_out);
  ADVCHAIN_LAUNCH_CHECK();
  return ADVCHAIN_OK;
}

extern "C" {

int advchain_tp_interp_fwd(const float* coef, float* out, const int32_t* itab, const float* ftab, const int64_t* S,
                           const int64_t* g, const int64_t* B, int64_t planes, int64_t C, int ndim, int add_identity,
                           float scale, float* sumsq, float* disp_out, void* stream) {
  (void)ndim;
  int64_t nwg;
  return tp_interp_fwd_launch<>(coef, out, itab, ftab, S, g, B, planes, C, add_identity, scale, sumsq, disp_out,
                                &nwg, stream);
}

int64_t advchain_tp_interp_sumsq_partials(const int64_t* S, int64_t planes) {
  if (!S || planes < 0 || planes >= 65536 || S[0] < 1 || S[1] < 1 || S[2] < 1 || S[0] >= 65536) return -1;
  return ((S[1] + kTpChunk - 1) / kTpChunk) * S[0] * planes;
}

int advchain_tp_interp_sumsq_ordered(const float* coef, const int32_t* itab, const float* ftab, const int64_t* S, const int64_t* g,
                                     const int64_t* B, int64_t planes, int64_t C, float* partials, float* out, void* stream) {
  ADVCHAIN_CHECK_ARG(partials && out, "tp_interp_sumsq_ordered: null pointer");
  ADVCHAIN_CHECK_ARG(S && g && B, "tp_interp_sumsq_ordered: null dims");
  int64_t nwg = 0;
  const int rc = tp_interp_fwd_launch<SumsqOrdered>(coef, nullptr, itab, ftab, S, g, B, planes, C, 0,
                                                    1.f, partials, nullptr, &nwg, stream);
  if (rc != ADVCHAIN_OK) return rc;
  hipLaunchKernelGGL(k_tp_partials_sum, dim3(1), dim3(kBlock), 0, (hipStream_t)stream, partials, nwg, out);
  ADVCHAIN_LAUNCH_CHECK();
  return ADVCHAIN_OK;
}

int advchain_tp_interp_fwd_smoothed_pair(const float* vel, float* s1, float* out, const int32_t* itab, const float* ftab,
                                         const int64_t* S, const int64_t* g, const int64_t* B, int64_t P, int64_t C,
                                         int add_identity, float scale, float* disp_out, const float* weights9, float gscale,
                                         void* stream) {
  ADVCHAIN_CHECK_ARG(vel && out && itab && ftab && weights9, "tp_interp_fwd_smoothed_pair: null pointer");
  ADVCHAIN_CHECK_ARG(P >= 0 && 2 * P < 65536 && C >= 1, "tp_interp_fwd_smoothed_pair: bad planes/C");
  BandTables T;
  ADVCHAIN_CHECK_ARG(unpack_tables(itab, ftab, S, g, B, T), "tp_interp_fwd_smoothed_pair: bad band tables");
  if (S[0] != 1 || g[0] != 1 || g[1] * g[2] > kGsFuseMax || T.a[2].g > kTpMaxLds) return ADVCHAIN_ERR_UNSUPPORTED;
  if (P == 0) return ADVCHAIN_OK;
  Dims full{(int)S[0], (int)S[1], (int)S[2]};
  ADVCHAIN_CHECK_ARG(full.voxels() < (1ll << 31), "tp_interp_fwd_smoothed_pair: volume too large");
  GaussW9 gw;
  for (int k = 0; k < 9; ++k) gw.w[k] = weights9[k];
  dim3 grid((unsigned)((full.s1 + kTpChunk - 1) / kTpChunk), 1u, (unsigned)(2 * P));
  if (full.s2 % 4 == 0 && full.s2 >= 128 && (reinterpret_cast<uintptr_t>(out) & 15) == 0)
    hipLaunchKernelGGL(k_tp_interp_fwd_gs<4>, grid, dim3(kBlock), 0, (hipStream_t)stream, vel, s1, out, T, full, (int)C, add_identity,
                       scale, disp_out, gw, gscale, (int)P);
  else
    hipLaunchKernelGGL(k_tp_interp_fwd_gs<1>, grid, dim3(kBlock), 0, (hipStream_t)stream, vel, s1, out, T, full, (int)C, add_identity,
                       scale, disp_out, gw, gscale, (int)P);
  ADVCHAIN_LAUNCH_CHECK();
  return ADVCHAIN_OK;
}

int advchain_band_reduce_axis(const float* in, const float* in2, float* out, const int32_t* itab, const float* ftab,
                              const int64_t* S, const int64_t* g, const int64_t* B, int axis, int64_t outer,
                              int64_t inner, float scale, void* stream) {
  ADVCHAIN_CHECK_ARG(in && out && itab && ftab, "band_reduce_axis: null pointer");
  ADVCHAIN_CHECK_ARG(axis >= 0 && axis < 3 && outer >= 0 && inner >= 1 && inner < (1ll << 31), "band_reduce_axis: bad axis/outer/inner");
  BandTables T;
  ADVCHAIN_CHECK_ARG(unpack_tables(itab, ftab, S, g, B, T), "band_reduce_axis: bad band tables");
  const int64_t total = outer * T.a[axis].g * inner;
  if (total == 0) return ADVCHAIN_OK;
  const BandAxis& A = T.a[axis];
  const bool aligned = ((reinterpret_cast<uintptr_t>(in) | reinterpret_cast<uintptr_t>(in2)) & 15) == 0;
  if (inner == 1 && A.S % 4 == 0 && A.S <= 1024 && A.g <= 64 && aligned) {
    int KG = A.g >= 4 ? 4 : (A.g >= 2 ? 2 : 1);
    while (KG < 16 && KG * 2 <= A.g && ((size_t)(64 / KG) * (A.S + 1) * sizeof(float) > 16 * 1024 + 512 || outer / (64 / KG) < 4096)) KG *= 2;
    const int RW = 64 / KG;
    int iters = (int)(outer / ((int64_t)RW * (kBrThreads / 64) * 2048));
    iters = iters < 1 ? 1 : (iters > 4 ? 4 : iters);
    const int64_t rows_per_block = (int64_t)(kBrThreads / 64) * RW * iters;
    const size_t lds = (size_t)(kBrThreads / 64) * RW * (A.S + 1) * sizeof(float);
    dim3 grid(advchain_blocks(outer, (int)rows_per_block)), block(kBrThreads);
    hipStream_t st = (hipStream_t)stream;
    switch (KG) {
      case 1: hipLaunchKernelGGL(k_band_reduce_rows<1>, grid, block, lds, st, in, in2, out, outer, A, scale, iters); break;
      case 2: hipLaunchKernelGGL(k_band_reduce_rows<2>, grid, block, lds, st, in, in2, out, outer, A, scale, iters); break;
      case 4: hipLaunchKernelGGL(k_band_reduce_rows<4>, grid, block, lds, st, in, in2, out, outer, A, scale, iters); break;
      case 8: hipLaunchKernelGGL(k_band_reduce_rows<8>, grid, block, lds, st, in, in2, out, outer, A, scale, iters); break;
      default: hipLaunchKernelGGL(k_band_reduce_rows<16>, grid, block, lds, st, in, in2, out, outer, A, scale, iters); break;
    }
    ADVCHAIN_LAUNCH_CHECK();
    return ADVCHAIN_OK;
  }
  if (total <= 131072 && inner > 1 && inner % 4 == 0 && aligned && outer < (1ll << 31) && (int64_t)A.S * 5 <= kBrSlabFloats) {
    int IC = (int)inner;
    while ((int64_t)A.S * (IC + 1) > kBrSlabFloats) IC = (IC / 2 + 3) / 4 * 4;
    const int chunks = (int)((inner + IC - 1) / IC);
    if (chunks <= 65535) {
      const size_t lds = (size_t)A.S * (IC + 1) * sizeof(float);
      hipLaunchKernelGGL(k_band_reduce_axis_slab, dim3((unsigned)outer, (unsigned)chunks), dim3(kBlock), lds, (hipStream_t)stream, in, in2,
                         out, (int)inner, IC, A, scale);
      ADVCHAIN_LAUNCH_CHECK();
      return ADVCHAIN_OK;
    }
  }
  hipLaunchKernelGGL(k_band_reduce_axis, dim3(advchain_blocks(total, kBlock)), dim3(kBlock), 0, (hipStream_t)stream, in,
                     in2, out, outer, (int)inner, T.a[axis], scale);
  ADVCHAIN_LAUNCH_CHECK();
  return ADVCHAIN_OK;
}

int advchain_band_reduce_rows_dense(const float* in, const float* in2, float* out, const float* wd, const int32_t* lo,
                                    int64_t rows, int64_t S, int64_t g, int64_t WB, float scale, void* stream) {
  ADVCHAIN_CHECK_ARG(in && out && wd && lo, "band_reduce_rows_dense: null pointer");
  ADVCHAIN_CHECK_ARG(rows >= 0 && S >= 1 && g >= 1 && WB >= 1, "band_reduce_rows_dense: bad shape");
  if (rows == 0) return ADVCHAIN_OK;
  const bool aligned = ((reinterpret_cast<uintptr_t>(in) | reinterpret_cast<uintptr_t>(in2)) & 15) == 0;
  if (S % 4 != 0 || S > 1024 || g > 64 || g * WB > kBrMaxW || !aligned) return ADVCHAIN_ERR_UNSUPPORTED;
  int KG = g >= 4 ? 4 : (g >= 2 ? 2 : 1);
  while (KG < 16 && ((64 / KG) * (S / 4) > 512 || rows / (64 / KG) < 4096)) KG *= 2;
  const int RW = 64 / KG;
  if (RW * (S / 4) > 512) return ADVCHAIN_ERR_UNSUPPORTED;
  int iters = (int)(rows / ((int64_t)RW * (kBrThreads / 64) * 2048));
  iters = iters < 1 ? 1 : (iters > 4 ? 4 : iters);
  const int64_t rows_per_block = (int64_t)(kBrThreads / 64) * RW * iters;
  const size_t lds = ((size_t)(kBrThreads / 64) * RW * (S + 1) + (size_t)(g * WB)) * sizeof(float);
  dim3 grid(advchain_blocks(rows, (int)rows_per_block)), block(kBrThreads);
  hipStream_t st = (hipStream_t)stream;
#define BRD_GO(KG_) hipLaunchKernelGGL(k_band_reduce_rows_dense<KG_>, grid, block, lds, st, in, in2, out, rows, wd, lo, (int)S, (int)g, (int)WB, scale, iters)
  switch (KG) {
    case 1: BRD_GO(1); break;
    case 2: BRD_GO(2); break;
    case 4: BRD_GO(4); break;
    case 8: BRD_GO(8); break;
    default: BRD_GO(16); break;
  }
#undef BRD_GO
  ADVCHAIN_LAUNCH_CHECK();
  return ADVCHAIN_OK;
}

constexpr int64_t kBiasMinWg = 512;
static int bias_rows_rule(int64_t S0, int64_t S1, int64_t N) {
  for (int rows = 32; rows > 4; rows /= 2)
    if (((S1 + rows - 1) / rows) * S0 * N >= kBiasMinWg) return rows;
  return 4;
}
static inline bool bias_rows_ok(int rows) { return rows == 0 || rows == 4 || rows == 8 || rows == 16 || rows == 32; }

int advchain_bias_rows_per_wg(const int64_t* S, int64_t N) {
  if (!S || N < 0 || N >= 65536 || S[0] < 1 || S[1] < 1 || S[2] < 1) return -1;
  return bias_rows_rule(S[0], S[1], N);
}

int advchain_bias_field_fwd_rows(const float* cp, const float* data, float* out, float* field, const int32_t* itab,
                                 const float* ftab, const int64_t* S, const int64_t* g, const int64_t* B, int64_t N,
                                 int64_t C, float eps, int use_log, float cp_scale, int rows_per_wg, void* stream) {
  ADVCHAIN_CHECK_ARG(cp && field && itab && ftab && (!data || out), "bias_field_fwd: null pointer");
  ADVCHAIN_CHECK_ARG(S && g && B, "bias_field_fwd: null dims");
  ADVCHAIN_CHECK_ARG(N >= 0 && N < 65536 && C >= 1, "bias_field_fwd: bad N/C");
  ADVCHAIN_CHECK_ARG(bias_rows_ok(rows_per_wg), "bias_field_fwd: rows_per_wg must be 0, 4, 8, 16 or 32");
  BandTables T;
  ADVCHAIN_CHECK_ARG(unpack_tables(itab, ftab, S, g, B, T), "bias_field_fwd: bad band tables");
  if (N == 0) return ADVCHAIN_OK;
  Dims full{(int)S[0], (int)S[1], (int)S[2]};
  ADVCHAIN_CHECK_ARG(full.voxels() < (1ll << 31), "bias_field_fwd: volume too large");
  ADVCHAIN_CHECK_ARG(T.a[2].g <= kTpMaxLds, "bias_field_fwd: too many control points per row");
  const int rows = rows_per_wg ? rows_per_wg : bias_rows_rule(S[0], S[1], N);
  ADVCHAIN_CHECK_ARG(S[0] < 65536 && (S[1] + rows - 1) / rows < (1ll << 31), "bias_field_fwd: grid too large");
  dim3 grid((unsigned)((full.s1 + rows - 1) / rows), (unsigned)full.s0, (unsigned)N);
  if (full.s2 % 4 == 0 && ((reinterpret_cast<uintptr_t>(data) | reinterpret_cast<uintptr_t>(out) | reinterpret_cast<uintptr_t>(field)) & 15) == 0)
    hipLaunchKernelGGL(k_bias_fwd<4>, grid, dim3(kBlock), 0, (hipStream_t)stream, cp, data, out, field, T, full, (int)C, eps,
                       use_log, cp_scale, rows);
  else
    hipLaunchKernelGGL(k_bias_fwd<1>, grid, dim3(kBlock), 0, (hipStream_t)stream, cp, data, out, field, T, full, (int)C, eps,
                       use_log, cp_scale, rows);
  ADVCHAIN_LAUNCH_CHECK();
  return ADVCHAIN_OK;
}

int advchain_bias_field_fwd(const float* cp, const float* data, float* out, float* field, const int32_t* itab,
                            const float* ftab, const int64_t* S, const int64_t* g, const int64_t* B, int64_t N,
                            int64_t C, float eps, int use_log, float cp_scale, void* stream) {
  return advchain_bias_field_fwd_rows(cp, data, out, field, itab, ftab, S, g, B, N, C, eps, use_log, cp_scale, 0, stream);
}

int advchain_bias_field_bwd_rows(const float* cp, const float* data, const float* grad_out, float* grad_L, float* grad_data,
                                 const int32_t* itab, const float* ftab, const int64_t* S, const int64_t* g,
                                 const int64_t* B, int64_t N, int64_t C, float eps, int use_log, float cp_scale,
                                 int rows_per_wg, void* stream) {
  ADVCHAIN_CHECK_ARG(cp && data && grad_out && itab && ftab && (grad_L || grad_data), "bias_field_bwd: null pointer");
  ADVCHAIN_CHECK_ARG(S && g && B, "bias_field_bwd: null dims");
  ADVCHAIN_CHECK_ARG(N >= 0 && N < 65536 && C >= 1, "bias_field_bwd: bad N/C");
  ADVCHAIN_CHECK_ARG(bias_rows_ok(rows_per_wg), "bias_field_bwd: rows_per_wg must be 0, 4, 8, 16 or 32");
  BandTables T;
  ADVCHAIN_CHECK_ARG(unpack_tables(itab, ftab, S, g, B, T), "bias_field_bwd: bad band tables");
  if (N == 0) return ADVCHAIN_OK;
  Dims full{(int)S[0], (int)S[1], (int)S[2]};
  ADVCHAIN_CHECK_ARG(full.voxels() < (1ll << 31), "bias_field_bwd: volume too large");
  ADVCHAIN_CHECK_ARG(T.a[2].g <= kTpMaxLds, "bias_field_bwd: too many control points per row");
  const int rows = rows_per_wg ? rows_per_wg : bias_rows_rule(S[0], S[1], N);
  ADVCHAIN_CHECK_ARG(S[0] < 65536 && (S[1] + rows - 1) / rows < (1ll << 31), "bias_field_bwd: grid too large");
  dim3 grid((unsigned)((full.s1 + rows - 1) / rows), (unsigned)full.s0, (unsigned)N);
  if (full.s2 % 4 == 0 && ((reinterpret_cast<uintptr_t>(data) | reinterpret_cast<uintptr_t>(grad_out) |
                            reinterpret_cast<uintptr_t>(grad_L) | reinterpret_cast<uintptr_t>(grad_data)) & 15) == 0)
    hipLaunchKernelGGL((k_bias_bwd<4, false>), grid, dim3(kBlock), 0, (hipStream_t)stream, cp, data, grad_out, grad_L, grad_data, T,
                       full, (int)C, eps, use_log, cp_scale, rows, (float*)nullptr, (const float*)nullptr, (const int*)nullptr, 0);
  else
    hipLaunchKernelGGL((k_bias_bwd<1, false>), grid, dim3(kBlock), 0, (hipStream_t)stream, cp, data, grad_out, grad_L, grad_data, T,
                       full, (int)C, eps, use_log, cp_scale, rows, (float*)nullptr, (const float*)nullptr, (const int*)nullptr, 0);
  ADVCHAIN_LAUNCH_CHECK();
  return ADVCHAIN_OK;
}

int advchain_bias_field_bwd(const float* cp, const float* data, const float* grad_out, float* grad_L, float* grad_data,
                            const int32_t* itab, const float* ftab, const int64_t* S, const int64_t* g,
                            const int64_t* B, int64_t N, int64_t C, float eps, int use_log, float cp_scale,
                            void* stream) {
  return advchain_bias_field_bwd_rows(cp, data, grad_out, grad_L, grad_data, itab, ftab, S, g, B, N, C, eps, use_log, cp_scale, 0,
                                      stream);
}

constexpr size_t kBiasRedLds = 48 * 1024;
int advchain_bias_field_bwd_reduced(const float* cp, const float* data, const float* grad_out, float* t1, float* grad_data,
                                    const int32_t* itab, const float* ftab, const int64_t* S, const int64_t* g,
                                    const int64_t* B, int64_t N, int64_t C, float eps, int use_log, float cp_scale,
                                    const float* wd, const int32_t* lo, int64_t WB, int rows_per_wg, void* stream) {
  ADVCHAIN_CHECK_ARG(cp && data && grad_out && itab && ftab && wd && lo, "bias_field_bwd_reduced: null pointer");
  ADVCHAIN_CHECK_ARG(S && g && B, "bias_field_bwd_reduced: null dims");
  ADVCHAIN_CHECK_ARG(N >= 0 && N < 65536 && C >= 1 && WB >= 1, "bias_field_bwd_reduced: bad N/C/WB");
  ADVCHAIN_CHECK_ARG(bias_rows_ok(rows_per_wg), "bias_field_bwd_reduced: rows_per_wg must be 0, 4, 8, 16 or 32");
  BandTables T;
  ADVCHAIN_CHECK_ARG(unpack_tables(itab, ftab, S, g, B, T), "bias_field_bwd_reduced: bad band tables");
  if (!t1) return ADVCHAIN_ERR_UNSUPPORTED;
  const bool aligned = ((reinterpret_cast<uintptr_t>(data) | reinterpret_cast<uintptr_t>(grad_out) |
                         reinterpret_cast<uintptr_t>(grad_data)) & 15) == 0;
  if (S[2] % 4 != 0 || S[2] > 1024 || g[2] > 64 || g[2] * WB > kBrMaxW || !aligned) return ADVCHAIN_ERR_UNSUPPORTED;
  const size_t wbytes = (size_t)((g[2] * WB + 3) / 4 * 4) * sizeof(float);
  int rows = rows_per_wg ? rows_per_wg : bias_rows_rule(S[0], S[1], N);
  while (rows > 4 && wbytes + (size_t)rows * (S[2] + 1) * sizeof(float) > kBiasRedLds) rows /= 2;
  const size_t lds = wbytes + (size_t)rows * (S[2] + 1) * sizeof(float);
  if (lds > kBiasRedLds) return ADVCHAIN_ERR_UNSUPPORTED;
  if (N == 0) return ADVCHAIN_OK;
  Dims full{(int)S[0], (int)S[1], (int)S[2]};
  ADVCHAIN_CHECK_ARG(full.voxels() < (1ll << 31), "bias_field_bwd_reduced: volume too large");
  ADVCHAIN_CHECK_ARG(S[0] < 65536 && (S[1] + rows - 1) / rows < (1ll << 31), "bias_field_bwd_reduced: grid too large");
  dim3 grid((unsigned)((full.s1 + rows - 1) / rows), (unsigned)full.s0, (unsigned)N);
  hipLaunchKernelGGL((k_bias_bwd<4, true>), grid, dim3(kBlock), lds, (hipStream_t)stream, cp, data, grad_out, (float*)nullptr,
                     grad_data, T, full, (int)C, eps, use_log, cp_scale, rows, t1, wd, (const int*)lo, (int)WB);
  ADVCHAIN_LAUNCH_CHECK();
  return ADVCHAIN_OK;
}

constexpr int kGenericMaxTaps = 129;
struct GaussWN { float w[kGenericMaxTaps]; };

namespace advchain {
__global__ void __launch_bounds__(kBlock) k_gauss_axis_generic(const float* __restrict__ in, float* __restrict__ out, int64_t total,
                                                               Dims d, int axis, GaussWN gw, int ntaps, float scale) {
  const int64_t i = (int64_t)blockIdx.x * kBlock + threadIdx.x;
  if (i >= total) return;
  const int V = (int)d.voxels();
  const int v = (int)(i % V);
  const int x = v % d.s2, y = (v / d.s2) % d.s1, z = v / (d.s2 * d.s1);
  const int S = axis == 2 ? d.s2 : (axis == 1 ? d.s1 : d.s0);
  const int c = axis == 2 ? x : (axis == 1 ? y : z);
  const int stride = axis == 2 ? 1 : (axis == 1 ? d.s2 : d.s1 * d.s2);
  const int R = ntaps / 2;
  const float* p = in + (i - (int64_t)c * stride);
  float acc = 0.f;
  for (int t = 0; t < ntaps; ++t) {
    const int q = c + t - R;
    if (q >= 0 && q < S) acc = fmaf(gw.w[t], p[(int64_t)q * stride] * scale, acc);
  }
  out[i] = acc;
}
}

int advchain_gauss_axis_generic(const float* in, float* out, int64_t planes, int ndim, const int64_t* dims, int axis,
                                const float* weights, int ntaps, float scale, void* stream) {
  ADVCHAIN_CHECK_ARG(in && out && in != out && weights, "gauss_axis_generic: null/aliased pointer");
  ADVCHAIN_CHECK_ARG(dims_ok(ndim, dims), "gauss_axis_generic: bad dims");
  ADVCHAIN_CHECK_ARG(axis >= 0 && axis < 3, "gauss_axis_generic: bad axis");
  ADVCHAIN_CHECK_ARG(ntaps >= 1 && ntaps <= kGenericMaxTaps && (ntaps & 1) == 1, "gauss_axis_generic: the window must have 1..129 taps, odd");
  const Dims d = make_dims(ndim, dims);
  ADVCHAIN_CHECK_ARG(d.voxels() < (1ll << 31), "gauss_axis_generic: volume too large");
  const int64_t total = planes * d.voxels();
  if (total == 0) return ADVCHAIN_OK;
  GaussWN gw;
  for (int k = 0; k < ntaps; ++k) gw.w[k] = weights[k];
  hipLaunchKernelGGL(advchain::k_gauss_axis_generic, dim3(advchain_blocks(total, kBlock)), dim3(kBlock), 0, (hipStream_t)stream, in, out,
                     total, d, axis, gw, ntaps, scale);
  ADVCHAIN_LAUNCH_CHECK();
  return ADVCHAIN_OK;
}

int advchain_gauss_axis(const float* in, float* out, const float* aux, int64_t planes, int64_t C, int ndim,
                        const int64_t* dims, int axis, const float* weights9, int pre, int post, float scale,
                        void* stream) {
  ADVCHAIN_CHECK_ARG(in && out && in != out && weights9, "gauss_axis: null/aliased pointer");
  ADVCHAIN_CHECK_ARG(dims_ok(ndim, dims), "gauss_axis: bad dims");
  ADVCHAIN_CHECK_ARG(axis >= 0 && axis < 3 && C >= 1 && C <= 3, "gauss_axis: bad axis/C");
  ADVCHAIN_CHECK_ARG(pre >= 0 && pre <= 2 && post >= 0 && post <= 2 && (post != 2 || aux), "gauss_axis: bad pre/post");
  const Dims d = make_dims(ndim, dims);
  const int64_t total = planes * d.voxels();
  ADVCHAIN_CHECK_ARG(d.voxels() < (1ll << 31), "gauss_axis: volume too large");
  if (total == 0) return ADVCHAIN_OK;
  GaussW gw;
  for (int k = 0; k < 9; ++k) gw.w[k] = weights9[k];
  hipStream_t st = (hipStream_t)stream;
  dim3 blk(kBlock);
  const bool v4 = (d.s2 % 4 == 0) && ((reinterpret_cast<uintptr_t>(in) | reinterpret_cast<uintptr_t>(out) |
                                       reinterpret_cast<uintptr_t>(aux)) & 15) == 0;
  dim3 grid(advchain_blocks(v4 ? total / 4 : total, kBlock));
  int riw = (v4 && d.s2 >= 4 && 64 % (d.s2 / 4) == 0 && (total / 4) % 64 == 0) ? 1 : 0;
  if (!riw && v4 && axis == 2 && d.s2 >= 8 && d.s2 / 4 <= 64) {
    riw = 2;
    const int64_t rows = total / d.s2, rpw = 64 / (d.s2 / 4);
    grid = dim3(advchain_blocks(((rows + rpw - 1) / rpw) * 64, kBlock));
  }
  if (v4 && axis == 0 && d.s0 >= 32) {
    const int zc = 27;
    const int nchunk = (d.s0 + zc - 1) / zc;
    const int64_t threads = planes * nchunk * d.s1 * (d.s2 / 4);
    dim3 gm(advchain_blocks(threads, kBlock));
#define GM(PRE, POST) hipLaunchKernelGGL((k_gauss_march_z<PRE, POST>), gm, blk, 0, st, in, out, aux, planes, d, (int)C, gw, scale, zc, nchunk)
    switch (pre * 3 + post) {
      case 0: GM(0, 0); break;
      case 1: GM(0, 1); break;
      case 2: GM(0, 2); break;
      case 3: GM(1, 0); break;
      case 4: GM(1, 1); break;
      case 5: GM(1, 2); break;
      case 6: GM(2, 0); break;
      case 7: GM(2, 1); break;
      default: GM(2, 2); break;
    }
#undef GM
    ADVCHAIN_LAUNCH_CHECK();
    return ADVCHAIN_OK;
  }
#define GA(PRE, POST)                                                                                                     \
  do {                                                                                                                    \
    if (!v4) hipLaunchKernelGGL((k_gauss_axis<PRE, POST>), grid, blk, 0, st, in, out, aux, total, d, (int)C, axis, gw, scale); \
    else if (axis == 2) hipLaunchKernelGGL((k_gauss_axis_v4<PRE, POST, 2>), grid, blk, 0, st, in, out, aux, total / 4, d, (int)C, gw, scale, riw); \
    else if (axis == 1) hipLaunchKernelGGL((k_gauss_axis_v4<PRE, POST, 1>), grid, blk, 0, st, in, out, aux, total / 4, d, (int)C, gw, scale, 0); \
    else hipLaunchKernelGGL((k_gauss_axis_v4<PRE, POST, 0>), grid, blk, 0, st, in, out, aux, total / 4, d, (int)C, gw, scale, 0); \
  } while (0)
  switch (pre * 3 + post) {
    case 0: GA(0, 0); break;
    case 1: GA(0, 1); break;
    case 2: GA(0, 2); break;
    case 3: GA(1, 0); break;
    case 4: GA(1, 1); break;
    case 5: GA(1, 2); break;
    case 6: GA(2, 0); break;
    case 7: GA(2, 1); break;
    default: GA(2, 2); break;
  }
#undef GA
  ADVCHAIN_LAUNCH_CHECK();
  return ADVCHAIN_OK;
}

}

bool advchain_gauss_xy_takes(int ndim, const int64_t* dims, int64_t planes) {
  if (!dims_ok(ndim, dims)) return false;
  const Dims d = make_dims(ndim, dims);
  if ((d.s2 & 3) != 0 || d.s2 < 8 || d.s2 > 512 || d.s1 < 8 || planes > 65535 || d.s0 > 65535) return false;
  int TY = 32;
  while (TY > 8 && (size_t)(TY + 8) * (2 * d.s2 + 8) * 4 > 53248) TY >>= 1;
  if (TY > d.s1) TY = (d.s1 + 7) / 8 * 8;
  return (size_t)(TY + 8) * (2 * d.s2 + 8) * sizeof(float) <= 65536;
}

static bool gauss_xy_lane_shape(const Dims& d) {
  const int Q = d.s2 >> 2;
  return (d.s2 & 3) == 0 && Q >= 2 && Q <= 64 && (Q & (Q - 1)) == 0 && d.s1 >= 8;
}
static bool gauss_xy_lane_tile_ok(int ty, int nt) {
  return (ty == 16 && (nt == 256 || nt == 512)) || (ty == 32 && (nt == 256 || nt == 512)) || (ty == 64 && nt == 1024);
}
static bool gauss_xy_lane_rule(const Dims& d, int64_t planes, int& ty, int& nt) {
  (void)planes;
  if (!gauss_xy_lane_shape(d) || d.s2 != 256) return false;
  ty = 32; nt = 512;
  return true;
}
static inline int gauss_xy_clamp_ty(int TY, const Dims& d) { return TY > d.s1 ? (d.s1 + 7) / 8 * 8 : TY; }

enum { kGxyAuto = 0, kGxyStaged = 1, kGxyLanes = 2 };

static int gauss_xy_launch(const float* in, float* out, const float* aux, int64_t planes, int64_t C, int ndim, const int64_t* dims,
                           const float* weights9, int pre, int post, float scale, void* stream, const float* in_hi, int64_t planes_lo,
                           int want, int ty, int nt) {
  ADVCHAIN_CHECK_ARG(in && out && in != out && weights9, "gauss_xy: null/aliased pointer");
  ADVCHAIN_CHECK_ARG(dims_ok(ndim, dims), "gauss_xy: bad dims");
  ADVCHAIN_CHECK_ARG(C >= 1 && C <= 3 && pre >= 0 && pre <= 2 && post >= 0 && post <= 2 && (post != 2 || aux), "gauss_xy: bad C/pre/post");
  ADVCHAIN_CHECK_ARG(post == 0 || ndim == 2, "gauss_xy: post belongs to the last axis");
  const Dims d = make_dims(ndim, dims);
  if ((d.s2 & 3) != 0 || d.s2 < 8 || d.s2 > 512 || d.s1 < 8 || planes > 65535 || d.s0 > 65535 ||
      ((reinterpret_cast<uintptr_t>(in) | reinterpret_cast<uintptr_t>(out) | reinterpret_cast<uintptr_t>(aux) |
        reinterpret_cast<uintptr_t>(in_hi)) & 15) != 0)
    return ADVCHAIN_ERR_UNSUPPORTED;
  ADVCHAIN_CHECK_ARG(!in_hi || (planes_lo > 0 && planes_lo < planes), "gauss_xy: bad split of the input planes");
  if (want == kGxyLanes) {
    ADVCHAIN_CHECK_ARG(gauss_xy_lane_tile_ok(ty, nt), "gauss_xy_lanes: (ty, nt) must be (16,256), (16,512), (32,256), (32,512) or (64,1024)");
    if (!gauss_xy_lane_shape(d)) return ADVCHAIN_ERR_UNSUPPORTED;
  }
  if (planes == 0 || d.voxels() == 0) return ADVCHAIN_OK;
  GaussW gw;
  for (int k = 0; k < 9; ++k) gw.w[k] = weights9[k];
  hipStream_t st = (hipStream_t)stream;
  if (want == kGxyLanes || (want == kGxyAuto && gauss_xy_lane_rule(d, planes, ty, nt))) {
    const int TY = gauss_xy_clamp_ty(ty, d);
    const size_t lds = (size_t)(TY + 8) * d.s2 * sizeof(float);
    dim3 grid((unsigned)((d.s1 + TY - 1) / TY), (unsigned)d.s0, (unsigned)planes);
#define GXL(PRE, POST, NT_, U_) do { \
    auto kern = k_gauss_xy_lanes<PRE, POST, NT_, U_>; \
    if (lds > 65536) (void)hipFuncSetAttribute(reinterpret_cast<const void*>(kern), hipFuncAttributeMaxDynamicSharedMemorySize, (int)lds); \
    hipLaunchKernelGGL(kern, grid, dim3(NT_), lds, st, in, out, aux, d, (int)C, gw, scale, TY, in_hi, (int)planes_lo); } while (0)
#define GXL_TILE(PRE, POST) do { \
    if (ty == 16 && nt == 256) GXL(PRE, POST, 256, 6); \
    else if (ty == 16) GXL(PRE, POST, 512, 3); \
    else if (ty == 32 && nt == 256) GXL(PRE, POST, 256, 10); \
    else if (ty == 32) GXL(PRE, POST, 512, 5); \
    else GXL(PRE, POST, 1024, 5); } while (0)
    switch (pre * 3 + post) {
      case 0: GXL_TILE(0, 0); break;
      case 1: GXL_TILE(0, 1); break;
      case 2: GXL_TILE(0, 2); break;
      case 3: GXL_TILE(1, 0); break;
      case 4: GXL_TILE(1, 1); break;
      case 5: GXL_TILE(1, 2); break;
      case 6: GXL_TILE(2, 0); break;
      case 7: GXL_TILE(2, 1); break;
      default: GXL_TILE(2, 2); break;
    }
#undef GXL_TILE
#undef GXL
    ADVCHAIN_LAUNCH_CHECK();
    return ADVCHAIN_OK;
  }
  int TY = 32;
  while (TY > 8 && (size_t)(TY + 8) * (2 * d.s2 + 8) * 4 > 53248) TY >>= 1;
  if (TY > d.s1) TY = (d.s1 + 7) / 8 * 8;
  const size_t lds = (size_t)(TY + 8) * (2 * d.s2 + 8) * sizeof(float);
  if (lds > 65536) return ADVCHAIN_ERR_UNSUPPORTED;
  dim3 grid((unsigned)((d.s1 + TY - 1) / TY), (unsigned)d.s0, (unsigned)planes);
#define GXY(PRE, POST) hipLaunchKernelGGL((k_gauss_xy<PRE, POST>), grid, dim3(kBlock), lds, st, in, out, aux, d, (int)C, gw, scale, TY, in_hi, (int)planes_lo)
  switch (pre * 3 + post) {
    case 0: GXY(0, 0); break;
    case 1: GXY(0, 1); break;
    case 2: GXY(0, 2); break;
    case 3: GXY(1, 0); break;
    case 4: GXY(1, 1); break;
    case 5: GXY(1, 2); break;
    case 6: GXY(2, 0); break;
    case 7: GXY(2, 1); break;
    default: GXY(2, 2); break;
  }
#undef GXY
  ADVCHAIN_LAUNCH_CHECK();
  return ADVCHAIN_OK;
}

extern "C" {

int advchain_gauss_xy(const float* in, float* out, const float* aux, int64_t planes, int64_t C, int ndim, const int64_t* dims,
                      const float* weights9, int pre, int post, float scale, void* stream, const float* in_hi, int64_t planes_lo) {
  return gauss_xy_launch(in, out, aux, planes, C, ndim, dims, weights9, pre, post, scale, stream, in_hi, planes_lo, kGxyAuto, 0, 0);
}

int advchain_gauss_xy_staged(const float* in, float* out, const float* aux, int64_t planes, int64_t C, int ndim,
                             const int64_t* dims, const float* weights9, int pre, int post, float scale, void* stream,
                             const float* in_hi, int64_t planes_lo) {
  return gauss_xy_launch(in, out, aux, planes, C, ndim, dims, weights9, pre, post, scale, stream, in_hi, planes_lo, kGxyStaged, 0, 0);
}

int advchain_gauss_xy_lanes(const float* in, float* out, const float* aux, int64_t planes, int64_t C, int ndim,
                            const int64_t* dims, const float* weights9, int pre, int post, float scale, void* stream,
                            const float* in_hi, int64_t planes_lo, int ty, int nt) {
  return gauss_xy_launch(in, out, aux, planes, C, ndim, dims, weights9, pre, post, scale, stream, in_hi, planes_lo, kGxyLanes, ty, nt);
}

int advchain_gauss_xy_plan(int ndim, const int64_t* dims, int64_t planes, int* form, int* ty, int* nt) {
  if (!form || !ty || !nt || !dims_ok(ndim, dims) || planes < 0) return -1;
  *form = 0; *ty = 0; *nt = 0;
  if (!advchain_gauss_xy_takes(ndim, dims, planes)) return 0;
  const Dims d = make_dims(ndim, dims);
  int t = 0, n = 0;
  if (gauss_xy_lane_rule(d, planes, t, n)) {
    *form = 2; *ty = gauss_xy_clamp_ty(t, d); *nt = n;
    return 0;
  }
  int TY = 32;
  while (TY > 8 && (size_t)(TY + 8) * (2 * d.s2 + 8) * 4 > 53248) TY >>= 1;
  *form = 1; *ty = gauss_xy_clamp_ty(TY, d); *nt = kBlock;
  return 0;
}

static int gauss_small_launch(const float* in, float* out, int64_t planes, int ndim, const int64_t* dims,
                              const float* weights9, int pre, float scale, int mirror, void* stream) {
  ADVCHAIN_CHECK_ARG(in && out && in != out && weights9, "gauss_small: null/aliased pointer");
  ADVCHAIN_CHECK_ARG(dims_ok(ndim, dims), "gauss_small: bad dims");
  ADVCHAIN_CHECK_ARG(pre == 0 || pre == 1, "gauss_small: pre must be 0 or 1");
  const Dims d = make_dims(ndim, dims);
  ADVCHAIN_CHECK_ARG(d.voxels() <= kGaussSmallMax, "gauss_small: plane larger than 4096 voxels");
  ADVCHAIN_CHECK_ARG(planes >= 0 && planes < (1ll << 30), "gauss_small: bad plane count");
  if (planes == 0) return ADVCHAIN_OK;
  GaussW gw;
  for (int k = 0; k < 9; ++k) gw.w[k] = weights9[k];
  const unsigned blocks = (unsigned)(mirror == 1 ? 2 * planes : planes);
  if (d.voxels() > 1024)
    hipLaunchKernelGGL(k_gauss_small<1024>, dim3(blocks), dim3(1024), 0, (hipStream_t)stream, in, out, d, ndim, gw,
                       pre == 1 ? scale : 1.f, mirror, (int)planes);
  else
    hipLaunchKernelGGL(k_gauss_small<kBlock>, dim3(blocks), dim3(kBlock), 0, (hipStream_t)stream, in, out, d, ndim, gw,
                       pre == 1 ? scale : 1.f, mirror, (int)planes);
  ADVCHAIN_LAUNCH_CHECK();
  return ADVCHAIN_OK;
}

int advchain_gauss_small(const float* in, float* out, int64_t planes, int ndim, const int64_t* dims,
                         const float* weights9, int pre, float scale, void* stream) {
  return gauss_small_launch(in, out, planes, ndim, dims, weights9, pre, scale, 0, stream);
}

int advchain_gauss_small_pair(const float* in, float* out, int64_t planes, int ndim, const int64_t* dims,
                              const float* weights9, float scale, int adjoint, void* stream) {
  return gauss_small_launch(in, out, planes, ndim, dims, weights9, 1, scale, adjoint ? 2 : 1, stream);
}

int advchain_sign_axpy(const float* base, const float* x, float* out, float a, int64_t n, const float* gate, const float* old,
                       void* stream) {
  ADVCHAIN_CHECK_ARG(x && out && n >= 0 && (!gate || old), "sign_axpy: null pointer");
  if (n == 0) return ADVCHAIN_OK;
  hipLaunchKernelGGL(k_sign_axpy, dim3(advchain_blocks(n, kBlock)), dim3(kBlock), 0, (hipStream_t)stream, base, x, out, a, n, gate, old);
  ADVCHAIN_LAUNCH_CHECK();
  return ADVCHAIN_OK;
}

int advchain_nonzero_mask(const float* x, float* out, int64_t n, void* stream) {
  ADVCHAIN_CHECK_ARG(x && out && n >= 0, "nonzero_mask: null pointer");
  if (n == 0) return ADVCHAIN_OK;
  hipLaunchKernelGGL(k_nonzero_mask, dim3(advchain_blocks(n, kBlock)), dim3(kBlock), 0, (hipStream_t)stream, x, out, n);
  ADVCHAIN_LAUNCH_CHECK();
  return ADVCHAIN_OK;
}

int advchain_axpy(const float* x, const float* y, float* out, float a, int64_t n, void* stream) {
// ... 62 lines not shown
```

advchain_amd/ops.py:

```python
import collections
import ctypes
import functools
import math
import numbers
import struct

import numpy as np
import torch

from . import _lib
from .bands import gaussian_weights_1d

_INTERP = {"bilinear": 0, "trilinear": 0, "linear": 0, "nearest": 1, "bicubic": 2}
_PAD = {"zeros": 0, "border": 1, "reflection": 2}
_GAUSS9 = _lib.float_array(gaussian_weights_1d(1.0))
_GAUSS9_CACHE = {}


GENERIC_MAX_TAPS = 129


def gauss9(sigma, taps=None):
    sigma = float(sigma)
    if taps is None:
        taps = 2 * int(4 * sigma + 0.5) + 1
    taps = int(taps)
    if sigma == 1.0 and taps == 9:
        return _GAUSS9
    w = _GAUSS9_CACHE.get((sigma, taps))
    if w is None:
        if not sigma > 0.0:
            raise ValueError("Gaussian smoothing needs sigma > 0, got %r" % (sigma,))
        if taps % 2 == 0:
            raise NotImplementedError("Gaussian smoothing with an even window (%d taps) is not implemented" % taps)
        if taps > GENERIC_MAX_TAPS:
            raise NotImplementedError("Gaussian smoothing with sigma=%g needs a %d-tap window (at most %d)"
                                      % (sigma, taps, GENERIC_MAX_TAPS))
        if len(_GAUSS9_CACHE) > 16:
            _GAUSS9_CACHE.clear()
        w = _GAUSS9_CACHE[(sigma, taps)] = _lib.float_array(gaussian_weights_1d(sigma, taps))
    return w


def _ptr(t):
    return None if t is None else ctypes.c_void_p(t.data_ptr())


_raw_stream = getattr(torch._C, "_cuda_getCurrentRawStream", None)
_raw_device = getattr(torch._C, "_cuda_getDevice", None)


def _stream():
    if _raw_stream is not None and _raw_device is not None:
        return ctypes.c_void_p(_raw_stream(_raw_device()))
    return ctypes.c_void_p(torch.cuda.current_stream().cuda_stream)


_STREAM_OBJ = {}


def _stream_obj():
    if _raw_stream is None or _raw_device is None:
        return torch.cuda.current_stream()
    dev = _raw_device()
    s = _STREAM_OBJ.get(dev)
    if s is None or s.cuda_stream != _raw_stream(dev):
        s = _STREAM_OBJ[dev] = torch.cuda.current_stream()
    return s


def _require_device(t, name):
    if not isinstance(t, torch.Tensor) or not t.is_cuda:
        raise _lib.AdvchainHipError("%s must be a CUDA/ROCm tensor: the advchain_amd kernels have no CPU path" % name)
    return t


def _dev(t, name="tensor"):
    _require_device(t, name)
    if t.dtype != torch.float32:
        raise _lib.AdvchainHipError("%s must be float32, got %s" % (name, t.dtype))
    return t if t.is_contiguous() else t.contiguous()


def _same_device(*tensors):
    dev = None
    for t in tensors:
        if t is None:
            continue
        if dev is None:
            dev = t.device
        elif t.device != dev:
            raise RuntimeError("Expected all tensors to be on the same device, but found at least two devices, "
                               "%s and %s!" % (dev, t.device))


def _on_tensor_device(fn):
    @functools.wraps(fn)
    def guarded(*args, **kwargs):
        for a in args:
            if isinstance(a, (tuple, list)) and a and isinstance(a[0], torch.Tensor):
                a = a[0]
            if isinstance(a, torch.Tensor):
                if a.is_cuda:
                    cur = _raw_device() if _raw_device is not None else torch.cuda.current_device()
                    if a.device.index != cur:
                        with torch.cuda.device(a.device):
                            return fn(*args, **kwargs)
                break
        return fn(*args, **kwargs)
    return guarded


def interp_code(interp):
    if interp not in _INTERP:
        raise NotImplementedError("interpolation mode %r is not implemented by the HIP sampler "
                                  "(supported: bilinear/trilinear, nearest, bicubic (2D))" % (interp,))
    return _INTERP[interp]


def pad_code(padding_mode):
    if padding_mode not in _PAD:
        raise NotImplementedError("padding_mode %r" % (padding_mode,))
    return _PAD[padding_mode]


def _hint_bits(disp):
    if disp is None or not disp == disp or disp < 0:
        return 0
    return min(int(disp) + 1, 255) << 8


def _fine_bits(disp):
    if disp is None or not disp == disp or disp < 0:
        return 0
    return max(1, min(int(disp * 1024.0) + 1, (1 << 22) - 1))


def raw_grid_sample_fwd(inp, grid, interp, padding, clamp_grid, disp_hint=None):
    N, C = inp.shape[:2]
    nd = inp.dim() - 2
    odims = grid.shape[2:]
    out = torch.empty((N, C) + tuple(odims), device=inp.device, dtype=torch.float32)
    _lib.check(_lib.load().advchain_grid_sample_fwd(_ptr(inp), _ptr(grid), _ptr(out), N, C, nd,
                                                    _lib.dims_array(inp.shape[2:]), _lib.dims_array(odims),
                                                    interp, padding, int(clamp_grid) | _hint_bits(disp_hint), _stream()),
               "grid_sample_fwd")
    return out


def raw_grid_sample_fwd_ride(inp, grid, ride, interp, padding, clamp_grid, nonzero, disp_hint=None):
    N, C = inp.shape[:2]
    nd = inp.dim() - 2
    odims = tuple(grid.shape[2:])
    out = torch.empty((N, C) + odims, device=inp.device, dtype=torch.float32)
    rout = torch.empty((N, 1) + odims, device=inp.device, dtype=torch.float32)
    _lib.check(_lib.load().advchain_grid_sample_fwd_ride(_ptr(inp), _ptr(grid), _ptr(out), _ptr(ride), _ptr(rout), N, C, nd,
                                                         _lib.dims_array(inp.shape[2:]), _lib.dims_array(odims), interp, padding,
                                                         int(clamp_grid) | _hint_bits(disp_hint), int(bool(nonzero)), _stream()),
               "grid_sample_fwd_ride")
    return out, rout


DISP_SLOTS = 4096
ADAPTIVE_HALO = True
PAIR_FIELDS = True
TILED_SCATTER = True
FUSED_LOSS = True
WIDE_LOSS_MIN_K = 17
REF_GRAD_REG_MAX_K = 4
FUSE_2D = True
COMPOSITE = True
RIDE_MASK = True
RIDE_INTERPS = ("bilinear", "trilinear", "linear", "nearest")
WINDOW_STAGED = True
WINDOW_STAGED_CHANNELS = (1, 2, 4)
BIAS_REDUCED = True
GAUSS_XY_LANES = True

BWD_ROUTES = ("none", "general", "rows", "gather", "march", "window_float", "window_int64", "window_staged", "tiled")


def last_bwd_route():
    return BWD_ROUTES[_lib.load().advchain_last_bwd_route()]


def set_deterministic(on):
    _lib.load().advchain_set_deterministic(1 if on else 0)


def is_deterministic():
    return bool(_lib.load().advchain_get_deterministic())


def _scatter_workspace(N, dims, device):
    n = _lib.load().advchain_scatter_workspace(N, len(dims), _lib.dims_array(dims))
    return torch.empty(n, device=device, dtype=torch.int32)


def _det_warp_workspace(N, C, dims, device):
    n = _lib.load().advchain_det_warp_workspace(N, C, len(dims), _lib.dims_array(dims))
    return torch.empty(max(1, n), device=device, dtype=torch.int32)


def _general_warp_kernel(C, interp, in_dims, out_dims):
    return C > 4 or interp != 0 or tuple(in_dims) != tuple(out_dims)


def raw_grid_sample_bwd(gout, inp, grid, interp, padding, clamp_grid, need_gin, need_ggrid, halo=0):
    N, C = inp.shape[:2]
    nd = inp.dim() - 2
    if need_gin and is_deterministic() and _general_warp_kernel(C, interp, inp.shape[2:], grid.shape[2:]):
        ws = _det_warp_workspace(N, C, inp.shape[2:], inp.device)
        gin = torch.empty_like(inp)
        ggrid = torch.empty_like(grid) if need_ggrid else None
        _lib.check(_lib.load().advchain_grid_sample_bwd_det(_ptr(gout), _ptr(inp), _ptr(grid), _ptr(gin), _ptr(ggrid), _ptr(ws),
                                                            N, C, nd, _lib.dims_array(inp.shape[2:]),
                                                            _lib.dims_array(grid.shape[2:]), interp, padding, int(clamp_grid),
                                                            _stream()), "grid_sample_bwd_det")
        return gin, ggrid
    tiled = TILED_SCATTER and need_gin
    ws = _scatter_workspace(N, inp.shape[2:], inp.device) if tiled else None
    gin = (torch.empty_like(inp) if tiled else torch.zeros_like(inp)) if need_gin else None
    ggrid = torch.empty_like(grid) if need_ggrid else None
    if (tiled and WINDOW_STAGED and nd == 2 and C in WINDOW_STAGED_CHANNELS and is_deterministic()
            and not _general_warp_kernel(C, interp, inp.shape[2:], grid.shape[2:])):
        lib = _lib.load()
        n = lib.advchain_window_stage_workspace(N, C, nd, _lib.dims_array(inp.shape[2:]))
        stage = torch.empty(max(4, n), device=inp.device, dtype=torch.int32)
        _lib.check(lib.advchain_grid_sample_bwd_staged(_ptr(gout), _ptr(inp), _ptr(grid), _ptr(gin), _ptr(ggrid), _ptr(ws),
                                                       N, C, nd, _lib.dims_array(inp.shape[2:]),
                                                       _lib.dims_array(grid.shape[2:]), interp, padding, int(clamp_grid),
                                                       int(halo), _stream(), _ptr(stage)), "grid_sample_bwd_staged")
        return gin, ggrid
    _lib.check(_lib.load().advchain_grid_sample_bwd(_ptr(gout), _ptr(inp), _ptr(grid), _ptr(gin), _ptr(ggrid), _ptr(ws),
                                                    N, C, nd, _lib.dims_array(inp.shape[2:]),
                                                    _lib.dims_array(grid.shape[2:]), interp, padding, int(clamp_grid),
                                                    int(halo), _stream()), "grid_sample_bwd")
    return gin, ggrid


def raw_compose_self_fwd(phi, phi0=None, final_mode=0, disp_out=None, disp_hint=None):
    N = phi.shape[0]
    nd = phi.dim() - 2
    out = torch.empty_like(phi)
    _lib.check(_lib.load().advchain_compose_self_fwd(_ptr(phi), _ptr(out), _ptr(phi0), N, nd,
                                                     _lib.dims_array(phi.shape[2:]), final_mode | _hint_bits(disp_hint), _ptr(disp_out),
                                                     _stream()), "compose_self_fwd")
    return out


def raw_compose_self_bwd(gout, phi, ws=None, chain=False, halo=0):
    N = phi.shape[0]
    nd = phi.dim() - 2
    if TILED_SCATTER and ws is None:
        ws, chain = _scatter_workspace(N, phi.shape[2:], phi.device), False
    gphi = torch.empty_like(phi) if ws is not None else torch.zeros_like(phi)
    _lib.check(_lib.load().advchain_compose_self_bwd(_ptr(gout), _ptr(phi), _ptr(gphi), _ptr(ws), int(bool(chain)), int(halo), N, nd,
                                                     _lib.dims_array(phi.shape[2:]), _stream()), "compose_self_bwd")
    return gphi


def raw_max_displacement(phi, out=None):
    if out is None:
        out = torch.zeros(1, device=phi.device, dtype=torch.float32)
    _lib.check(_lib.load().advchain_max_displacement(_ptr(phi), _ptr(out), phi.shape[0], phi.dim() - 2,
                                                     _lib.dims_array(phi.shape[2:]), _stream()), "max_displacement")
    return out


def raw_slot_rows_max(slots, reset=False, out=None):
    if out is None:
        out = torch.empty(slots.shape[0], device=slots.device, dtype=torch.float32)
    _lib.check(_lib.load().advchain_slot_rows_max(_ptr(slots), _ptr(out), slots.shape[0], slots.shape[1], int(bool(reset)),
                                                  _stream()), "slot_rows_max")
    return out


_PERSISTENT = {}


def _persistent_zeros(tag, shape, device):
    stream = _raw_stream(_raw_device()) if (_raw_stream and _raw_device) else torch.cuda.current_stream().cuda_stream
    key = (tag, tuple(shape), str(device), stream)
    plan = _PLAN
    if plan is not None and plan.is_frozen:
        key = key[:3]
        buf = plan.persistent.get(key)
        if buf is None:
            buf = plan.persistent[key] = torch.zeros(shape, device=device, dtype=torch.float32)
        return buf
    if plan is not None and plan.recording:
        plan.wanted_zeros.add(key[:3])
    buf = _PERSISTENT.get(key)
    if buf is None:
        if len(_PERSISTENT) > 64:
            _PERSISTENT.clear()
        buf = _PERSISTENT[key] = torch.zeros(shape, device=device, dtype=torch.float32)
    return buf


def _forget_persistent(buf):
    stores = [_PERSISTENT] + ([_PLAN.persistent] if _PLAN is not None else [])
    for store in stores:
        for k in [k for k, v in store.items() if v is buf]:
            del store[k]


def raw_gauss_small_pair(x, scale, adjoint=False, weights=None):
    if x[0, 0].numel() > 4096 or not x.is_contiguous() or (weights is not None and len(weights) != 9):
        return None
    nd = x.dim() - 2
    n_in = x.shape[0]
    n_out = n_in // 2 if adjoint else 2 * n_in
    out = torch.empty((n_out,) + tuple(x.shape[1:]), device=x.device, dtype=torch.float32)
    planes = (n_out if adjoint else n_in) * x.shape[1]
    _lib.check(_lib.load().advchain_gauss_small_pair(_ptr(x), _ptr(out), planes, nd, _lib.dims_array(x.shape[2:]),
                                                     weights or _GAUSS9, float(scale), int(bool(adjoint)), _stream()),
               "gauss_small_pair")
    return out


def raw_gauss_small_pair_into(x, out, scale, weights=None):
    _lib.check(_lib.load().advchain_gauss_small_pair(_ptr(x), _ptr(out), x.shape[0] * x.shape[1], x.dim() - 2,
                                                     _lib.dims_array(x.shape[2:]), weights or _GAUSS9, float(scale), 0, _stream()),
               "gauss_small_pair")


@_on_tensor_device
def sign_axpy(base, x, a, gate=None, old=None):
    x = _dev(x.detach(), "x")
    base = None if base is None else _dev(base.detach(), "base")
    gate, old = _gate_args(gate, old, x)
    out = torch.empty_like(x)
    _lib.check(_lib.load().advchain_sign_axpy(_ptr(base), _ptr(x), _ptr(out), float(a), x.numel(), _ptr(gate), _ptr(old),
                                              _stream()), "sign_axpy")
    return out


@_on_tensor_device
def nonzero_mask(x):
    x = _dev(x.detach(), "x")
    out = torch.empty_like(x)
    _lib.check(_lib.load().advchain_nonzero_mask(_ptr(x), _ptr(out), x.numel(), _stream()), "nonzero_mask")
    return out


_ONES = {}


def cached_ones(shape, device):
    key = (tuple(shape), str(device))
    plan = _PLAN
    store = plan.persistent if (plan is not None and plan.is_frozen) else _ONES
    t = store.get(("ones",) + key) if store is not _ONES else _ONES.get(key)
    if t is None:
        if store is _ONES:
            if len(_ONES) > 16:
                _ONES.clear()
            t = _ONES[key] = torch.ones(shape, device=device, dtype=torch.float32)
        else:
            t = _ONES.get(key)
            if t is None:
                t = torch.ones(shape, device=device, dtype=torch.float32)
            store[("ones",) + key] = t
    return t


_CLASS_W = {}


def class_weights_device(values, device):
    key = (str(device), values)
    t = _CLASS_W.get(key)
    if t is None:
        if len(_CLASS_W) > 64:
            _CLASS_W.clear()
        t = _CLASS_W[key] = torch.tensor(values, dtype=torch.float32, device=device)
    plan = _PLAN
    if plan is not None and plan.is_frozen:
        plan.persistent.setdefault(("class_w",) + key, t)
    return t


def squaring_halo(disp, d):
    if not disp == disp:
        return 0
    if disp < 0.999:
        return -1
    if d == 3:
        return _halo_3d(disp)
    if 16 - 0.001 <= disp < 32 - 0.001:
        return -24 if disp < 24 - 0.001 else -32
    return _halo_2d(disp)


def _halo_3d(disp):
    for h in (2, 3, 4):
        if disp < h - 0.001:
            return -h
    return 8


def _halo_2d(disp):
    for h in (2, 3, 4, 6, 8, 12, 16):
        if disp < h - 0.001:
            return -h
    return 16


def raw_gauss(x, C, pre=0, post=0, scale=1.0, aux=None, weights=None):
    w9 = weights or _GAUSS9
    x_hi = None
    if isinstance(x, (tuple, list)):
        x, x_hi = x
        shape = (x.shape[0] + x_hi.shape[0],) + tuple(x.shape[1:])
    else:
        shape = tuple(x.shape)
    nd = x.dim() - 2
    planes = shape[0] * shape[1]
    dims = _lib.dims_array(x.shape[2:])
    axes = [2, 1, 0][:nd]
    lib = _lib.load()
    if len(w9) != 9:
        if post != 0 or pre not in (0, 1):
            raise NotImplementedError("the fused prologue / epilogue of the Gaussian exists for the 9-tap window only")
        cur = torch.cat([x, x_hi], 0) if x_hi is not None else x
        cur = cur if cur.is_contiguous() else cur.contiguous()
        for i, ax in enumerate(axes):
            out = torch.empty_like(cur)
            _lib.check(lib.advchain_gauss_axis_generic(_ptr(cur), _ptr(out), planes, nd, dims, ax, w9, len(w9),
                                                       float(scale) if (pre == 1 and i == 0) else 1.0, _stream()),
                       "gauss_axis_generic")
            cur = out
        return cur
    if x_hi is not None and (x[0, 0].numel() <= 4096 or not (x.is_contiguous() and x_hi.is_contiguous())):
        x, x_hi = torch.cat([x, x_hi], 0), None
    if post == 0 and pre in (0, 1) and x[0, 0].numel() <= 4096:
        out = torch.empty_like(x)
        _lib.check(lib.advchain_gauss_small(_ptr(x), _ptr(out), planes, nd, dims, w9, pre, float(scale), _stream()),
                   "gauss_small")
        return out
    cur = x
    out = torch.empty(shape, device=x.device, dtype=torch.float32)
    gauss_xy = lib.advchain_gauss_xy if GAUSS_XY_LANES else lib.advchain_gauss_xy_staged
    rc = gauss_xy(_ptr(x),_ptr(out), _ptr(aux) if (post == 2 and nd == 2) else None, planes, C, nd, dims, w9,
                               pre, post if nd == 2 else 0, float(scale) if pre == 1 else 1.0, _stream(), _ptr(x_hi),
                               x.shape[0] * x.shape[1])
    if rc == 0:
        if nd == 2:
            return out
        out2 = torch.empty_like(out)
        _lib.check(lib.advchain_gauss_axis(_ptr(out), _ptr(out2), _ptr(aux) if post == 2 else None, planes, C, nd, dims, 0,
                                           w9, 0, post, 1.0, _stream()), "gauss_axis")
        return out2
    if rc != -2:
        _lib.check(rc, "gauss_xy")
    if x_hi is not None:
        x = cur = torch.cat([x, x_hi], 0)
    for i, ax in enumerate(axes):
        out = torch.empty_like(x)
        p = pre if i == 0 else 0
        q = post if i == len(axes) - 1 else 0
        _lib.check(lib.advchain_gauss_axis(_ptr(cur), _ptr(out), _ptr(aux) if q == 2 else None, planes, C, nd, dims, ax,
                                           w9, p, q, float(scale) if p == 1 else 1.0, _stream()), "gauss_axis")
        cur = out
    return cur


def raw_tp_interp(coef, tables, C, add_identity=False, scale=1.0, want_out=True, sumsq=None, disp_out=None, out=None):
    planes = coef.shape[0] * coef.shape[1]
    if want_out and out is None:
        out = torch.empty((coef.shape[0], coef.shape[1]) + tuple(tables.full_dims), device=coef.device,
                          dtype=torch.float32)
    _lib.check(_lib.load().advchain_tp_interp_fwd(_ptr(coef), _ptr(out), _ptr(tables.itab), _ptr(tables.ftab),
                                                  _lib.dims_array(tables.S), _lib.dims_array(tables.g),
                                                  _lib.dims_array(tables.B), planes, C, tables.ndim,
                                                  int(add_identity), float(scale), _ptr(sumsq), _ptr(disp_out),
                                                  _stream()),
               "tp_interp_fwd")
    return out


def field_sumsq(coef, tables, C):
    coef = _dev(coef, "coefficients")
    if is_deterministic():
        lib = _lib.load()
        planes = coef.shape[0] * coef.shape[1]
        S = _lib.dims_array(tables.S)
        partials = torch.empty(max(1, lib.advchain_tp_interp_sumsq_partials(S, planes)), device=coef.device, dtype=torch.float32)
        out = torch.empty(1, device=coef.device, dtype=torch.float32)
        _lib.check(lib.advchain_tp_interp_sumsq_ordered(_ptr(coef), _ptr(tables.itab), _ptr(tables.ftab), S,
                                                        _lib.dims_array(tables.g), _lib.dims_array(tables.B), planes, C,
                                                        _ptr(partials), _ptr(out), _stream()), "tp_interp_sumsq_ordered")
        return out
# ... 2181 lines not shown
```

include/advchain_hip.h:

```cpp
#ifndef ADVCHAIN_HIP_H_
#define ADVCHAIN_HIP_H_

#include <stdint.h>

#ifdef __cplusplus
extern "C" {
#endif

#define ADVCHAIN_INTERP_LINEAR 0
#define ADVCHAIN_INTERP_NEAREST 1
#define ADVCHAIN_INTERP_BICUBIC 2
#define ADVCHAIN_PAD_ZEROS 0
#define ADVCHAIN_PAD_BORDER 1
#define ADVCHAIN_PAD_REFLECTION 2

int advchain_version(void);
const char* advchain_last_error(void);

void advchain_set_deterministic(int on);
int advchain_get_deterministic(void);

int advchain_grid_sample_fwd(const float* in, const float* grid, float* out, int64_t N, int64_t C, int ndim,
                             const int64_t* in_dims, const int64_t* out_dims, int interp, int padding,
                             int clamp_grid, void* stream);
int advchain_grid_sample_fwd_ride(const float* in, const float* grid, float* out, const float* ride_in, float* ride_out,
                                  int64_t N, int64_t C, int ndim, const int64_t* in_dims, const int64_t* out_dims,
                                  int interp, int padding, int clamp_grid, int flags, void* stream);
int64_t advchain_scatter_workspace(int64_t N, int ndim, const int64_t* dims);
int advchain_grid_sample_bwd(const float* grad_out, const float* in, const float* grid, float* grad_in,
                             float* grad_grid, int32_t* workspace, int64_t N, int64_t C, int ndim,
                             const int64_t* in_dims, const int64_t* out_dims, int interp, int padding, int clamp_grid,
                             int halo, void* stream);
int64_t advchain_window_stage_workspace(int64_t N, int64_t C, int ndim, const int64_t* in_dims);
int advchain_grid_sample_bwd_staged(const float* grad_out, const float* in, const float* grid, float* grad_in,
                                    float* grad_grid, int32_t* workspace, int64_t N, int64_t C, int ndim,
                                    const int64_t* in_dims, const int64_t* out_dims, int interp, int padding, int clamp_grid,
                                    int halo, void* stream, int32_t* stage_ws);
#define ADVCHAIN_ROUTE_NONE 0
#define ADVCHAIN_ROUTE_GENERAL 1
#define ADVCHAIN_ROUTE_ROWS 2
#define ADVCHAIN_ROUTE_GATHER 3
#define ADVCHAIN_ROUTE_MARCH 4
#define ADVCHAIN_ROUTE_WINDOW_FLOAT 5
#define ADVCHAIN_ROUTE_WINDOW_INT64 6
#define ADVCHAIN_ROUTE_WINDOW_STAGED 7
#define ADVCHAIN_ROUTE_TILED 8
int advchain_last_bwd_route(void);
int64_t advchain_det_warp_workspace(int64_t N, int64_t C, int ndim, const int64_t* in_dims);
int advchain_grid_sample_bwd_det(const float* grad_out, const float* in, const float* grid, float* grad_in,
                                 float* grad_grid, int32_t* det_ws, int64_t N, int64_t C, int ndim,
                                 const int64_t* in_dims, const int64_t* out_dims, int interp, int padding, int clamp_grid,
                                 void* stream);

#define ADVCHAIN_DISP_SLOTS 4096
int advchain_compose_self_fwd(const float* phi, float* out, const float* phi0, int64_t N, int ndim,
                              const int64_t* dims, int final_mode, float* disp_out, void* stream);
int advchain_compose_self_bwd(const float* grad_out, const float* phi, float* grad_phi, int32_t* workspace, int chain,
                              int halo, int64_t N, int ndim, const int64_t* dims, void* stream);
int advchain_expo_chain_fused_levels(int64_t N, int ndim, const int64_t* dims, int n, const int32_t* hints);
int advchain_expo_chain_fwd(const float* phi0, float* fields, float* pos, int64_t N, int ndim, const int64_t* dims, int n,
                            float* disp_rows, const int32_t* hints, float* fuse_flag, void* stream);
int advchain_expo_chain_bwd(const float* grad_pos, const float* phi0, const float* fields, float* grad_phi0, float* scratch,
                            int32_t* workspace, const int32_t* halos, int64_t N, int ndim, const int64_t* dims, int n,
                            void* stream);
int advchain_demons_compose_pair_fwd(const float* vel, float* s1, float* phi0, float* fields, float* pos, float* q,
                                     float* disp, float* rows_max, const int32_t* itab, const float* ftab,
                                     const int64_t* S3, const int64_t* g3, const int64_t* B3, int64_t N, int ndim, int n,
                                     const int32_t* hints, const float* weights9_host, float scale, float inv, int fuse,
                                     void* stream);
int advchain_demons_compose_pair_bwd(const float* gq_lo, const float* gq_hi, const float* pos, const float* phi0,
                                     const float* fields, float* gpos, float* g, float* scratch, int32_t* ws, float* t1,
                                     float* gs1, float* gvel, const int32_t* halos, const int32_t* itab, const float* ftab,
                                     const float* wd, const int32_t* wlo, int64_t WB, const int64_t* S3, const int64_t* g3,
                                     const int64_t* B3, int64_t N, int ndim, int n, const float* weights9_host, float scale,
                                     float inv, void* stream);
int advchain_max_displacement(const float* phi, float* out, int64_t N, int ndim, const int64_t* dims, void* stream);
int advchain_slot_rows_max(float* slots, float* out, int64_t rows, int64_t cols, int reset, void* stream);
int advchain_bounds_check(const float* values, const float* lo, const float* hi, int64_t n, int32_t* flag, void* stream);

int advchain_affine_warp_fwd(const float* in, const float* theta, float* out, int64_t N, int64_t C, int ndim,
                             const int64_t* dims, int interp, int padding, void* stream);
int advchain_affine_warp_fwd_ride(const float* in, const float* theta, float* out, const float* ride_in, float* ride_out,
                                  int64_t N, int64_t C, int ndim, const int64_t* dims, int interp, int padding, int flags,
                                  void* stream);
int64_t advchain_affine_warp_bwd_workspace(int64_t N, int ndim, const int64_t* dims);
int advchain_affine_warp_bwd(const float* grad_out, const float* in, const float* theta, float* grad_in,
                             float* grad_theta, float* workspace, int64_t N, int64_t C, int ndim,
                             const int64_t* dims, int interp, int padding, void* stream);
int advchain_affine_warp_bwd_det(const float* grad_out, const float* in, const float* theta, float* grad_in,
                                 float* grad_theta, float* workspace, int32_t* det_ws, int64_t N, int64_t C, int ndim,
                                 const int64_t* dims, int interp, int padding, void* stream);

int advchain_grid_sample_bicubic2d_fwd(const float* in, const float* grid, float* out, int64_t N, int64_t C,
                                       const int64_t* in_dims, const int64_t* out_dims, int padding, void* stream);
int advchain_grid_sample_bicubic2d_bwd(const float* grad_out, const float* in, const float* grid, float* grad_in,
                                       float* grad_grid, int64_t N, int64_t C, const int64_t* in_dims,
                                       const int64_t* out_dims, int padding, void* stream);
int64_t advchain_bicubic2d_det_workspace(int64_t N, int64_t C, const int64_t* in_dims);
int advchain_grid_sample_bicubic2d_bwd_det(const float* grad_out, const float* in, const float* grid, float* grad_in,
                                           float* grad_grid, int32_t* det_ws, int64_t N, int64_t C, const int64_t* in_dims,
                                           const int64_t* out_dims, int padding, void* stream);
int advchain_affine_grid2d_fwd(const float* theta, float* grid, int64_t N, const int64_t* dims, void* stream);
int64_t advchain_affine_grid2d_bwd_workspace(int64_t N, const int64_t* dims);
int advchain_affine_grid2d_bwd(const float* grad_grid, float* grad_theta, float* workspace, int64_t N, const int64_t* dims,
                               void* stream);

int advchain_affine_theta_fwd(const float* param, const float* cfg_host, float param_scale, float* theta,
                              float* theta_inv, int64_t N, int ndim, void* stream);
int advchain_affine_theta_bwd(const float* param, const float* cfg_host, float param_scale, const float* grad_theta,
                              const float* grad_theta_inv, float* grad_param, int64_t N, int ndim, void* stream);

int advchain_tp_interp_fwd(const float* coef, float* out, const int32_t* itab, const float* ftab, const int64_t* S,
                           const int64_t* g, const int64_t* B, int64_t planes, int64_t C, int ndim, int add_identity,
                           float scale, float* sumsq, float* disp_out, void* stream);
int64_t advchain_tp_interp_sumsq_partials(const int64_t* S, int64_t planes);
int advchain_tp_interp_sumsq_ordered(const float* coef, const int32_t* itab, const float* ftab, const int64_t* S, const int64_t* g,
                                     const int64_t* B, int64_t planes, int64_t C, float* partials, float* out, void* stream);
int advchain_tp_interp_fwd_smoothed_pair(const float* vel, float* s1, float* out, const int32_t* itab, const float* ftab,
                                         const int64_t* S, const int64_t* g, const int64_t* B, int64_t P, int64_t C,
                                         int add_identity, float scale, float* disp_out, const float* weights9, float gscale,
                                         void* stream);
int advchain_band_reduce_axis(const float* in, const float* in2, float* out, const int32_t* itab, const float* ftab,
                              const int64_t* S, const int64_t* g, const int64_t* B, int axis, int64_t outer,
                              int64_t inner, float scale, void* stream);
int advchain_band_reduce_rows_dense(const float* in, const float* in2, float* out, const float* wd, const int32_t* lo,
                                    int64_t rows, int64_t S, int64_t g, int64_t WB, float scale, void* stream);

int advchain_bias_field_fwd(const float* cp, const float* data, float* out, float* field, const int32_t* itab,
                            const float* ftab, const int64_t* S, const int64_t* g, const int64_t* B, int64_t N,
                            int64_t C, float eps, int use_log, float cp_scale, void* stream);
int advchain_bias_field_bwd(const float* cp, const float* data, const float* grad_out, float* grad_L, float* grad_data,
                            const int32_t* itab, const float* ftab, const int64_t* S, const int64_t* g,
                            const int64_t* B, int64_t N, int64_t C, float eps, int use_log, float cp_scale,
                            void* stream);
int advchain_bias_rows_per_wg(const int64_t* S, int64_t N);
int advchain_bias_field_fwd_rows(const float* cp, const float* data, float* out, float* field, const int32_t* itab,
                                 const float* ftab, const int64_t* S, const int64_t* g, const int64_t* B, int64_t N,
                                 int64_t C, float eps, int use_log, float cp_scale, int rows_per_wg, void* stream);
int advchain_bias_field_bwd_rows(const float* cp, const float* data, const float* grad_out, float* grad_L, float* grad_data,
                                 const int32_t* itab, const float* ftab, const int64_t* S, const int64_t* g,
                                 const int64_t* B, int64_t N, int64_t C, float eps, int use_log, float cp_scale,
                                 int rows_per_wg, void* stream);
int advchain_bias_field_bwd_reduced(const float* cp, const float* data, const float* grad_out, float* t1, float* grad_data,
                                    const int32_t* itab, const float* ftab, const int64_t* S, const int64_t* g,
                                    const int64_t* B, int64_t N, int64_t C, float eps, int use_log, float cp_scale,
                                    const float* wd, const int32_t* lo, int64_t WB, int rows_per_wg, void* stream);

int advchain_gauss_axis(const float* in, float* out, const float* aux, int64_t planes, int64_t C, int ndim,
                        const int64_t* dims, int axis, const float* weights9_host, int pre, int post, float scale,
                        void* stream);

int advchain_gauss_axis_generic(const float* in, float* out, int64_t planes, int ndim, const int64_t* dims, int axis,
                                const float* weights_host, int ntaps, float scale, void* stream);

int advchain_gauss_xy(const float* in, float* out, const float* aux, int64_t planes, int64_t C, int ndim, const int64_t* dims,
                      const float* weights9, int pre, int post, float scale, void* stream, const float* in_hi,
                      int64_t planes_lo);
int advchain_gauss_xy_staged(const float* in, float* out, const float* aux, int64_t planes, int64_t C, int ndim,
                             const int64_t* dims, const float* weights9, int pre, int post, float scale, void* stream,
                             const float* in_hi, int64_t planes_lo);
int advchain_gauss_xy_lanes(const float* in, float* out, const float* aux, int64_t planes, int64_t C, int ndim,
                            const int64_t* dims, const float* weights9, int pre, int post, float scale, void* stream,
                            const float* in_hi, int64_t planes_lo, int ty, int nt);
int advchain_gauss_xy_plan(int ndim, const int64_t* dims, int64_t planes, int* form, int* ty, int* nt);
int advchain_gauss_small(const float* in, float* out, int64_t planes, int ndim, const int64_t* dims,
                         const float* weights9_host, int pre, float scale, void* stream);

int advchain_gauss_small_pair(const float* in, float* out, int64_t planes, int ndim, const int64_t* dims,
                              const float* weights9_host, float scale, int adjoint, void* stream);

int advchain_axpy(const float* x, const float* y, float* out, float a, int64_t n, void* stream);
int advchain_sign_axpy(const float* base, const float* x, float* out, float a, int64_t n, const float* gate, const float* old,
                       void* stream);
int advchain_nonzero_mask(const float* x, float* out, int64_t n, void* stream);
int64_t advchain_norm_workspace(int64_t N, int64_t M);
int advchain_norm_axpy(const float* base, const float* x, float* out, float* workspace, float step, int64_t N,
                       int64_t M, void* stream);
int advchain_norm_axpy_gated(const float* base, const float* x, float* out, float* workspace, float step, int64_t N,
                             int64_t M, const float* gate, const float* old, void* stream);
typedef struct advchain_update_desc {
  const float* base;
  const float* x;
  float* out;
  const float* old;
  int64_t N;
  int64_t M;
  int32_t kind;
  float step;
} advchain_update_desc;
int advchain_update_multi(const advchain_update_desc* descs, int n, const float* gate, void* stream);

int advchain_consistency_fwd(const float* pred, const float* ref, const float* mask, float* P, float* D, float* R,
                             float* sums, int64_t N, int64_t K, int ndim, const int64_t* dims, int mask_channels,
                             int ref_is_prob, int want_edges, int want_kl, void* stream);
int advchain_consistency_finish(float* slots, const float* coef4_host, float* sums, float* value, int reset, void* stream);
int advchain_consistency_bwd(const float* P, const float* D, const float* R, const float* mask,
                             const float* grad_scale, float* grad_pred, float c_mse, float c_a, float c_b, float c_kl,
                             int kl_is_gt, int64_t N, int64_t K, int ndim, const int64_t* dims, int mask_channels,
                             void* stream);
int advchain_consistency_fused_fwd(const float* pred, const float* ref, const float* mask, float* R, float* sums, int64_t N,
                                   int64_t K, int ndim, const int64_t* dims, int mask_channels, int ref_is_prob, int want_edges,
                                   int want_kl, void* stream);
int advchain_consistency_fused_bwd(const float* pred, const float* ref, const float* R, const float* mask,
                                   const float* grad_scale, float* grad_pred, float c_mse, float c_a, float c_b, float c_kl,
                                   int ref_is_prob, int64_t N, int64_t K, int ndim, const int64_t* dims, int mask_channels,
                                   void* stream);

int advchain_consistency_wide_fwd(const float* pred, const float* ref, const float* mask, float* stats, float* R, float* sums,
                                  int64_t N, int64_t K, int ndim, const int64_t* dims, int mask_channels, int ref_is_prob,
                                  int want_edges, int want_kl, void* stream);
int advchain_consistency_wide_bwd(const float* pred, const float* ref, const float* stats, const float* R, const float* mask,
                                  const float* grad_scale, float* grad_pred, float c_mse, float c_a, float c_b, float c_kl,
                                  int ref_is_prob, int64_t N, int64_t K, int ndim, const int64_t* dims, int mask_channels,
                                  void* stream);

int advchain_consistency_ref_bwd(const float* pred, const float* ref, const float* stats ,
                                 const float* R , const float* mask, const float* grad_scale,
                                 float* grad_ref, float c_mse, float c_a, float c_b, float c_kl, int ref_is_prob,
                                 int64_t N, int64_t K, int ndim, const int64_t* dims, int mask_channels, void* stream);
void advchain_set_ref_grad_reg_max_k(int k);
int advchain_get_ref_grad_reg_max_k(void);

int advchain_consistency_lp_fwd(const void* pred, int pred_bf16, const void* ref, int ref_bf16, const float* mask, float* stats,
                                float* R , float* sums, int64_t N, int64_t K, int ndim, const int64_t* dims,
                                int mask_channels, int ref_is_prob, int want_edges, int want_kl, void* stream);
int advchain_consistency_lp_bwd(const void* pred, int pred_bf16, const void* ref, int ref_bf16, const float* stats,
                                const float* R , const float* mask, const float* grad_scale, void* grad_pred,
                                float c_mse, float c_a, float c_b, float c_kl, int ref_is_prob, int64_t N, int64_t K, int ndim,
                                const int64_t* dims, int mask_channels, void* stream);
int advchain_consistency_lp_ref_bwd(const void* pred, int pred_bf16, const void* ref, int ref_bf16, const float* stats,
                                    const float* R , const float* mask, const float* grad_scale, void* grad_ref,
                                    float c_mse, float c_a, float c_b, float c_kl, int ref_is_prob, int64_t N, int64_t K,
                                    int ndim, const int64_t* dims, int mask_channels, void* stream);

int advchain_consistency_cw_fwd(const void* pred, int pred_bf16, const void* ref, int ref_bf16, const float* mask, float* stats,
                                float* R , float* sums, int64_t N, int64_t K, int ndim, const int64_t* dims,
                                int mask_channels, int ref_is_prob, int want_edges, int want_kl, const float* class_w,
                                void* stream);
int advchain_consistency_cw_bwd(const void* pred, int pred_bf16, const void* ref, int ref_bf16, const float* stats,
                                const float* R , const float* mask, const float* grad_scale, void* grad_pred,
                                float c_mse, float c_a, float c_b, float c_kl, int ref_is_prob, int64_t N, int64_t K, int ndim,
                                const int64_t* dims, int mask_channels, const float* class_w, void* stream);
int advchain_consistency_cw_ref_bwd(const void* pred, int pred_bf16, const void* ref, int ref_bf16, const float* stats,
                                    const float* R , const float* mask, const float* grad_scale, void* grad_ref,
                                    float c_mse, float c_a, float c_b, float c_kl, int ref_is_prob, int64_t N, int64_t K,
                                    int ndim, const int64_t* dims, int mask_channels, const float* class_w, void* stream);

int64_t advchain_consistency_fwd_partials(int64_t N, int64_t K, int ndim, const int64_t* dims, int mask_channels, int want_edges,
                                          int aligned16);
int advchain_consistency_fwd_ord(const float* pred, const float* ref, const float* mask, float* P, float* D, float* R,
                                 float* partials, int64_t stride, int32_t* counts, int64_t N, int64_t K, int ndim,
                                 const int64_t* dims, int mask_channels, int ref_is_prob, int want_edges, int want_kl, void* stream);
int64_t advchain_consistency_fused_fwd_partials(int64_t N, int64_t K, int ndim, const int64_t* dims, int has_mask, int mask_channels,
                                                int want_edges, int aligned16);
int advchain_consistency_fused_fwd_ord(const float* pred, const float* ref, const float* mask, float* R, float* partials,
                                       int64_t stride, int32_t* counts, int64_t N, int64_t K, int ndim, const int64_t* dims,
                                       int mask_channels, int ref_is_prob, int want_edges, int want_kl, void* stream);
int64_t advchain_consistency_wide_fwd_partials(int64_t N, int64_t K, int ndim, const int64_t* dims, int want_edges, int aligned16);
int advchain_consistency_wide_fwd_ord(const float* pred, const float* ref, const float* mask, float* stats, float* R,
                                      float* partials, int64_t stride, int32_t* counts, int64_t N, int64_t K, int ndim,
                                      const int64_t* dims, int mask_channels, int ref_is_prob, int want_edges, int want_kl,
                                      void* stream);
int64_t advchain_consistency_lp_fwd_partials(int64_t N, int64_t K, int ndim, const int64_t* dims, int want_edges);
int advchain_consistency_lp_fwd_ord(const void* pred, int pred_bf16, const void* ref, int ref_bf16, const float* mask, float* stats,
                                    float* R, float* partials, int64_t stride, int32_t* counts, int64_t N, int64_t K, int ndim,
                                    const int64_t* dims, int mask_channels, int ref_is_prob, int want_edges, int want_kl,
                                    const float* class_w , void* stream);
int advchain_consistency_finish_ord(const float* partials, int64_t stride, const int32_t* counts4_host, const float* coef4_host,
                                    float* sums, float* value, void* stream);

int advchain_consistency_fused_fwd_bf16(const void* pred, const void* ref, const float* mask, void* R, float* sums, int64_t N,
                                        int64_t K, int ndim, const int64_t* dims, void* stream);
int advchain_consistency_fused_bwd_bf16(const void* pred, const void* ref, const void* R, const float* mask,
                                        const float* grad_scale, void* grad_pred, float c_mse, float c_a, float c_b, int64_t N,
                                        int64_t K, int ndim, const int64_t* dims, void* stream);

int64_t advchain_seg_loss_workspace(int64_t N, int ndim, const int64_t* dims);
int advchain_ce2d_fwd(const void* logits, int logits_bf16, const int64_t* labels, const float* soft, const float* weight,
                      float* lse, float* workspace, float* value, int64_t N, int64_t K, const int64_t* dims, float denom,
                      void* stream);
int advchain_ce2d_bwd(const void* logits, int logits_bf16, const int64_t* labels, const float* soft, const float* weight,
                      const float* lse, const float* grad_scale, void* grad_logits, float* grad_soft, int64_t N, int64_t K,
                      const int64_t* dims, float denom, void* stream);
int advchain_contour_fwd(const float* input, const int64_t* labels, const float* soft, const float* mask, float* R,
                         float* workspace, float* value, int64_t N, int64_t K, int ndim, const int64_t* dims, int first_class,
                         int mask_channels, void* stream);
int advchain_contour_bwd(const float* R, const float* grad_scale, float* grad_input, float* grad_soft, int64_t N, int64_t K,
                         int ndim, const int64_t* dims, int first_class, void* stream);
int advchain_one_hot(const int64_t* labels, float* out, int64_t N, int64_t depth, int64_t V, void* stream);

#define ADVCHAIN_DICE_IGNORE_BACKGROUND 1
#define ADVCHAIN_DICE_BATCH 2
int64_t advchain_dice_workspace(int64_t N, int64_t K, int ndim, const int64_t* dims);
int advchain_dice_fwd(const void* logits, int logits_bf16, const int64_t* labels, const float* soft, const float* weight,
                      float* lse, float* coef, float* workspace, float* value, int64_t N, int64_t K, int ndim,
                      const int64_t* dims, int flags, float smooth, float dice_w, float ce_w, void* stream);
int advchain_dice_bwd(const void* logits, int logits_bf16, const int64_t* labels, const float* soft, const float* weight,
                      const float* lse, const float* coef, const float* grad_scale, void* grad_logits, float* grad_soft,
                      int64_t N, int64_t K, int ndim, const int64_t* dims, float dice_w, float ce_w, void* stream);

int advchain_edt(const void* mask, int mask_kind, const float* sampling, int squared, float* out, int64_t B, int ndim,
                 const int64_t* dims, void* stream);
int64_t advchain_signed_maps_workspace(int64_t N, int64_t K, int ndim, const int64_t* dims);
int advchain_signed_maps(const int64_t* labels, const float* sampling, float* out, float* workspace, int64_t N, int64_t K,
                         int ndim, const int64_t* dims, void* stream);

int64_t advchain_surface_metrics_workspace(int64_t N, int64_t K, int ndim, const int64_t* dims);
int advchain_surface_metrics(const int64_t* pred, const int64_t* target, const float* sampling, double q, float* hausdorff,
                             float* hausdorff_pct, float* assd, float* directed, int64_t* surface_voxels, double* max_squared,
                             int64_t* overlap, float* dice, void* workspace, int64_t N, int64_t K, int ndim,
                             const int64_t* dims, void* stream);

int advchain_surface_dice_route(int64_t N, int64_t K, int ndim, const int64_t* dims, const float* sampling, double tolerance_max,
                                int route);
int64_t advchain_surface_dice_workspace(int64_t N, int64_t K, int ndim, const int64_t* dims, const float* sampling,
                                        double tolerance_max, int route);
int advchain_surface_dice(const int64_t* pred, const int64_t* target, const float* sampling, const void* thresholds,
                          double tolerance_max, int route, float* surface_dice, int64_t* within, int64_t* surface_voxels,
                          void* workspace, int64_t N, int64_t K, int ndim, const int64_t* dims, void* stream);

int64_t advchain_components_workspace(int64_t N, int ndim, const int64_t* dims);
int advchain_components(const int64_t* labels, int32_t* out_labels, int64_t* count, int32_t* sizes, void* workspace, int64_t N,
                        int ndim, const int64_t* dims, int connectivity, int64_t background, int64_t num_classes, void* stream);
int advchain_keep_largest(const int64_t* labels, int64_t* out, void* workspace, void* winners, int64_t N, int64_t K, int ndim,
                          const int64_t* dims, int connectivity, int64_t background, void* stream);
int advchain_remove_small(const int64_t* labels, int64_t* out, void* workspace, int64_t N, int ndim, const int64_t* dims,
                          int connectivity, int64_t background, int64_t num_classes, int64_t min_size, void* stream);
int64_t advchain_fill_holes_workspace(int64_t N, int ndim, const int64_t* dims);
int advchain_fill_holes(const int64_t* labels, int64_t* out, int64_t* fill, int64_t* count, int64_t* voxels, void* workspace,
                        int64_t N, int64_t K, int ndim, const int64_t* dims, int connectivity, int64_t background,
                        int64_t max_size, void* stream);
int64_t advchain_instance_match_workspace(int64_t N, int ndim, const int64_t* dims);
int advchain_instance_match(const int64_t* pred, const int64_t* target, int64_t* components, int64_t* matched,
                            int64_t* overlapping, int64_t* iou_fixed, float* precision, float* recall, float* f1, float* sq,
                            float* pq, uint8_t* pred_status, uint8_t* target_status, void* workspace, int64_t N, int64_t K,
                            int ndim, const int64_t* dims, int connectivity, int64_t background, double iou_threshold,
                            void* stream);
int64_t advchain_betti_workspace(int64_t N, int ndim, const int64_t* dims);
int advchain_betti(const int64_t* pred, const int64_t* target, int64_t* betti, int64_t* euler, int64_t* error, void* workspace,
                   int64_t N, int64_t K, int ndim, const int64_t* dims, int connectivity, void* stream);

int64_t advchain_morph_workspace(int op, int64_t N, int64_t K, int ndim, const int64_t* dims);
int advchain_morph(const int64_t* labels, const float* sampling, double radius, int op, int64_t* out, void* workspace, int64_t N,
                   int64_t K, int64_t background, int ndim, const int64_t* dims, void* stream);

#define ADVCHAIN_BOUNDARY_IGNORE_BACKGROUND 1
int64_t advchain_boundary_workspace(int64_t N, int64_t K, int ndim, const int64_t* dims);
int advchain_boundary_fwd(const void* logits, int logits_bf16, const int64_t* labels, const float* maps, const float* weight,
                          float* saved, float* workspace, float* value, int64_t N, int64_t K, int ndim, const int64_t* dims,
                          int flags, void* stream);
int advchain_boundary_bwd(const void* logits, int logits_bf16, const int64_t* labels, const float* maps, const float* weight,
                          const float* saved, const float* grad_scale, void* grad_logits, int64_t N, int64_t K, int ndim,
                          const int64_t* dims, int flags, void* stream);

int advchain_image_diff2d_fwd(const float* in, float* dx, float* dy, int64_t N, int64_t C, const int64_t* dims, void* stream);
int advchain_image_diff2d_bwd(const float* grad_dx, const float* grad_dy, float* grad_in, int64_t N, int64_t C,
                              const int64_t* dims, void* stream);
int advchain_jacobian_det2d_fwd(const float* field, float* det, int64_t N, const int64_t* dims, void* stream);
int advchain_jacobian_det2d_bwd(const float* grad_det, const float* field, float* grad_field, int64_t N, const int64_t* dims,
                                void* stream);
int advchain_expo_start(const float* duv, float* phi0, float inv, int64_t N, int ndim, const int64_t* dims, void* stream);
#define ADVCHAIN_SUMSQ_PARTIALS 1024
int advchain_sumsq_ordered(const float* x, int64_t n, float* partials, float* out, void* stream);

#define ADVCHAIN_JACOBIAN_POSITIONS 1
#define ADVCHAIN_JACOBIAN_CLAMP 2
int advchain_image_diff3d_fwd(const float* in, float* dx, float* dy, float* dz, int64_t N, int64_t C, const int64_t* dims,
                              void* stream);
int advchain_image_diff3d_bwd(const float* grad_dx, const float* grad_dy, const float* grad_dz, float* grad_in, int64_t N,
                              int64_t C, const int64_t* dims, void* stream);
int advchain_jacobian_det_fwd(const float* field, float* det, int64_t N, int ndim, const int64_t* dims, int mode, void* stream);
int advchain_jacobian_det_bwd(const float* grad_det, const float* field, float* grad_field, float* workspace, int64_t N,
                              int ndim, const int64_t* dims, int mode, void* stream);
int64_t advchain_jacobian_det_workspace(int64_t N, int ndim, const int64_t* dims);
int64_t advchain_jacobian_stats_workspace(int64_t N, int ndim, const int64_t* dims);
int advchain_jacobian_stats(const float* field, int64_t* neg, int64_t* nonpos, float* min, float* max, float* workspace,
                            int64_t N, int ndim, const int64_t* dims, int mode, void* stream);

#ifdef __cplusplus
}
#endif
#endif
```

Baseline: 4464.

## Use wide packed band-table loads and early issue in tensor-product interpolation kernels

Adds a compile-time band-width specialization (bands of 2 or 4) that loads column and row band tables with 16-byte packed loads instead of scalar loads, and bounds the band loop by the template width. In the smoothed-pair kernel the table loads are issued before the Gaussian smoothing stage so their latency overlaps that work. Also exposes a configurable rows-per-workgroup entry point and a global toggle, on by default. The cost is more kernel instantiations and register pressure from the held request state.

```diff
diff --git a/advchain_amd/_lib.py b/advchain_amd/_lib.py
--- a/advchain_amd/_lib.py
+++ b/advchain_amd/_lib.py
@@ -32,11 +32,15 @@
     "advchain_affine_theta_bwd": (_I, [_P, _P, _F, _P, _P, _P, _L, _I, _P]),
     "advchain_tp_interp_fwd": (_I, [_P, _P, _P, _P, _P, _P, _P, _L, _L, _I, _I, _F, _P, _P, _P]),
     "advchain_tp_interp_fwd_smoothed_pair": (_I, [_P, _P, _P, _P, _P, _P, _P, _P, _L, _L, _I, _F, _P, _P, _F, _P]),
+    "advchain_tp_interp_fwd_smoothed_pair_rows": (_I, [_P, _P, _P, _P, _P, _P, _P, _P, _L, _L, _I, _F, _P, _P, _F, _I, _P]),
     "advchain_band_reduce_axis": (_I, [_P, _P, _P, _P, _P, _P, _P, _P, _I, _L, _L, _F, _P]),
     "advchain_band_reduce_rows_dense": (_I, [_P, _P, _P, _P, _P, _L, _L, _L, _L, _F, _P]),
     "advchain_bias_field_fwd": (_I, [_P, _P, _P, _P, _P, _P, _P, _P, _P, _L, _L, _F, _I, _F, _P]),
     "advchain_bias_field_bwd": (_I, [_P, _P, _P, _P, _P, _P, _P, _P, _P, _P, _L, _L, _F, _I, _F, _P]),
     "advchain_bias_rows_per_wg": (_I, [_P, _L]),
+    "advchain_set_tp_wide_loads": (None, [_I]),
+    "advchain_get_tp_wide_loads": (_I, []),
+    "advchain_tp_wide_band": (_I, [_L]),
     "advchain_bias_field_fwd_rows": (_I, [_P, _P, _P, _P, _P, _P, _P, _P, _P, _L, _L, _F, _I, _F, _I, _P]),
     "advchain_bias_field_bwd_rows": (_I, [_P, _P, _P, _P, _P, _P, _P, _P, _P, _P, _L, _L, _F, _I, _F, _I, _P]),
     "advchain_bias_field_bwd_reduced": (_I, [_P, _P, _P, _P, _P, _P, _P, _P, _P, _P, _L, _L, _F, _I, _F, _P, _P, _L, _I, _P]),
diff --git a/advchain_amd/csrc/fields.hip b/advchain_amd/csrc/fields.hip
--- a/advchain_amd/csrc/fields.hip
+++ b/advchain_amd/csrc/fields.hip
@@ -1,4 +1,6 @@
 #include "sampler_common.h"
+
+#include <atomic>
 
 namespace advchain {
 
@@ -55,9 +57,81 @@
   return g;
 }
 
-template <int VEC, class Epi>
-__device__ __forceinline__ void tp_rows(const float* __restrict__ coef, const BandTables& T, const Dims& full, int i0,
-                                        int i1_begin, int i1_end, float* lds, Epi&& epi) {
+struct __attribute__((packed, aligned(4))) IntQuad { int v[4]; };
+
+__device__ __forceinline__ IntQuad tp_load_quad(const void* p, int n) {
+  IntQuad q;
+  if (n >= 4) {
+    q = *reinterpret_cast<const IntQuad*>(p);
+  } else {
+    const int* pi = reinterpret_cast<const int*>(p);
+#pragma unroll
+    for (int j = 0; j < 4; ++j) q.v[j] = j < n ? pi[j] : 0;
+  }
+  return q;
+}
+
+template <int WB>
+__device__ __forceinline__ void tp_load_cols_wide(const BandAxis& A2, int xg, int (&s2)[4], float (&w2)[4][WB]) {
+  const IntQuad s = *reinterpret_cast<const IntQuad*>(A2.start + xg * 4);
+  IntQuad w[WB];
+#pragma unroll
+  for (int j = 0; j < WB; ++j) w[j] = *reinterpret_cast<const IntQuad*>(A2.w + (xg * 4) * WB + 4 * j);
+#pragma unroll
+  for (int q = 0; q < 4; ++q) {
+    s2[q] = s.v[q];
+#pragma unroll
+    for (int c = 0; c < WB; ++c) w2[q][c] = __int_as_float(w[(q * WB + c) / 4].v[(q * WB + c) % 4]);
+  }
+}
+
+template <int VEC, int WB>
+struct TpReq {
+  static_assert(WB == 0 || (VEC == 4 && (WB == 2 || WB == 4)), "wide band loads: VEC = 4, bands of 2 or 4");
+  static constexpr int NW = WB ? WB : kBandMax;
+  int s0;
+  int s2f[VEC];
+  float w2f[VEC][NW];
+  IntQuad rowq;
+
+  __device__ __forceinline__ void request(const BandTables& T, const Dims& full, int i0, int i1_begin, int i1_end) {
+    const BandAxis& A0 = T.a[0];
+    const BandAxis& A1 = T.a[1];
+    const BandAxis& A2 = T.a[2];
+    const int ncol = full.s2 / VEC;
+    int XT = 64;
+    if (VEC > 1) { XT = 1; while (XT < ncol && XT < 64) XT *= 2; }
+    const int tx = threadIdx.x % XT;
+    if constexpr (WB != 0) {
+      const int nrow = i1_end - i1_begin;
+      const int t = threadIdx.x;
+      rowq = IntQuad{{0, 0, 0, 0}};
+      if (t < 64) {
+        const int n = nrow * A1.B - 4 * t;
+        if (n > 0) rowq = tp_load_quad(A1.w + i1_begin * A1.B + 4 * t, n);
+      } else if (t < 64 + kTpChunk / 4) {
+        const int n = nrow - 4 * (t - 64);
+        if (n > 0) rowq = tp_load_quad(A1.start + i1_begin + 4 * (t - 64), n);
+      }
+      s0 = A0.start[i0];
+      tp_load_cols_wide<WB>(A2, min(tx, ncol - 1), s2f, w2f);
+    } else {
+      s0 = A0.start[i0];
+#pragma unroll
+      for (int q = 0; q < VEC; ++q) {
+        const int col = min(tx * VEC + q, full.s2 - 1);
+        s2f[q] = A2.start[col];
+#pragma unroll
+        for (int c = 0; c < kBandMax; ++c) w2f[q][c] = c < A2.B ? A2.w[col * A2.B + c] : 0.f;
+      }
+    }
+  }
+};
+
+template <int VEC, int WB, class Epi>
+__device__ __forceinline__ void tp_run(const float* __restrict__ coef, const BandTables& T, const Dims& full, int i0,
+                                       int i1_begin, int i1_end, float* lds, TpReq<VEC, WB>& rq, bool requested, Epi&& epi) {
+  constexpr int NW = TpReq<VEC, WB>::NW;
   const BandAxis& A0 = T.a[0];
   const BandAxis& A1 = T.a[1];
   const BandAxis& A2 = T.a[2];
@@ -70,22 +144,32 @@
   __shared__ int s1_s[kTpChunk];
   __shared__ float w1_s[kTpChunk * kBandMax];
   const int nrow = i1_end - i1_begin;
-  for (int e = threadIdx.x; e < nrow * (A1.B + 1); e += kBlock) {
-    const int r = e / (A1.B + 1), b = e - r * (A1.B + 1);
-    if (b == 0) s1_s[r] = A1.start[i1_begin + r];
-    else w1_s[r * kBandMax + b - 1] = A1.w[(i1_begin + r) * A1.B + b - 1];
-  }
-  const int s0 = A0.start[i0];
+  if constexpr (WB != 0) {
+    if (!requested) rq.request(T, full, i0, i1_begin, i1_end);
+    const int t = threadIdx.x;
+    if (t < 64) {
+#pragma unroll
+      for (int j = 0; j < 4; ++j) {
+        const int e = 4 * t + j;
+        if (e < nrow * A1.B) w1_s[(e / A1.B) * kBandMax + e % A1.B] = __int_as_float(rq.rowq.v[j]);
+      }
+    } else if (t < 64 + kTpChunk / 4) {
+#pragma unroll
+      for (int j = 0; j < 4; ++j) {
+        const int e = 4 * (t - 64) + j;
+        if (e < nrow) s1_s[e] = rq.rowq.v[j];
+      }
+    }
+  } else {
+    for (int e = threadIdx.x; e < nrow * (A1.B + 1); e += kBlock) {
+      const int r = e / (A1.B + 1), b = e - r * (A1.B + 1);
+      if (b == 0) s1_s[r] = A1.start[i1_begin + r];
+      else w1_s[r * kBandMax + b - 1] = A1.w[(i1_begin + r) * A1.B + b - 1];
+    }
+    if (!requested) rq.request(T, full, i0, i1_begin, i1_end);
+  }
+  const int s0 = rq.s0;
   const float* w0 = A0.w + i0 * A0.B;
-  int s2f[VEC];
-  float w2f[VEC][kBandMax];
-#pragma unroll
-  for (int q = 0; q < VEC; ++q) {
-    const int col = min(tx * VEC + q, full.s2 - 1);
-    s2f[q] = A2.start[col];
-#pragma unroll
-    for (int c = 0; c < kBandMax; ++c) w2f[q][c] = c < A2.B ? A2.w[col * A2.B + c] : 0.f;
-  }
   __syncthreads();
   const int RPP = max(1, min(kTpChunk, kTpMaxLds / max(g2, 1)));
   for (int base = i1_begin; base < i1_end; base += RPP) {
@@ -115,17 +199,30 @@
     __syncthreads();
     for (int xg = tx; xg < ncol; xg += XT) {
       int s2[VEC];
-      float w2[VEC][kBandMax];
-#pragma unroll
-      for (int q = 0; q < VEC; ++q) {
+      float w2[VEC][NW];
+      if constexpr (WB != 0) {
         if (xg == tx) {
-          s2[q] = s2f[q];
-#pragma unroll
-          for (int c = 0; c < kBandMax; ++c) w2[q][c] = w2f[q][c];
+#pragma unroll
+          for (int q = 0; q < VEC; ++q) {
+            s2[q] = rq.s2f[q];
+#pragma unroll
+            for (int c = 0; c < NW; ++c) w2[q][c] = rq.w2f[q][c];
+          }
         } else {
-          s2[q] = A2.start[xg * VEC + q];
-#pragma unroll
-          for (int c = 0; c < kBandMax; ++c) w2[q][c] = c < A2.B ? A2.w[(xg * VEC + q) * A2.B + c] : 0.f;
+          tp_load_cols_wide<NW>(A2, xg, s2, w2);
+        }
+      } else {
+#pragma unroll
+        for (int q = 0; q < VEC; ++q) {
+          if (xg == tx) {
+            s2[q] = rq.s2f[q];
+#pragma unroll
+            for (int c = 0; c < kBandMax; ++c) w2[q][c] = rq.w2f[q][c];
+          } else {
+            s2[q] = A2.start[xg * VEC + q];
+#pragma unroll
+            for (int c = 0; c < kBandMax; ++c) w2[q][c] = c < A2.B ? A2.w[(xg * VEC + q) * A2.B + c] : 0.f;
+          }
         }
       }
       for (int r = ry; r < RPP; r += ROWS) {
@@ -136,8 +233,8 @@
         for (int q = 0; q < VEC; ++q) {
           float v = 0.f;
 #pragma unroll
-          for (int c = 0; c < kBandMax; ++c)
-            if (c < A2.B) v += w2[q][c] * lds[r * g2 + s2[q] + c];
+          for (int c = 0; c < NW; ++c)
+            if (WB != 0 || c < A2.B) v += w2[q][c] * lds[r * g2 + s2[q] + c];
           val[q] = v;
         }
         epi(i1, xg * VEC, val);
@@ -145,6 +242,13 @@
     }
     __syncthreads();
   }
+}
+
+template <int VEC, int WB, class Epi>
+__device__ __forceinline__ void tp_rows(const float* __restrict__ coef, const BandTables& T, const Dims& full, int i0,
+                                        int i1_begin, int i1_end, float* lds, Epi&& epi) {
+  TpReq<VEC, WB> rq;
+  tp_run<VEC, WB>(coef, T, full, i0, i1_begin, i1_end, lds, rq, false, epi);
 }
 
 struct SumsqOrdered {};
@@ -163,7 +267,7 @@
   if (threadIdx.x == 0) out[0] = v[0];
 }
 
-template <int VEC, class... ORD>
+template <int VEC, int WB, class... ORD>
 __global__ void __launch_bounds__(kBlock)
 k_tp_interp_fwd(const float* __restrict__ coef, float* __restrict__ out, BandTables T, Dims full, int C,
                 int add_identity, float scale, float* __restrict__ sumsq, float* __restrict__ disp_out) {
@@ -177,7 +281,7 @@
   float sq[1] = {0.f};
   float dmax = 0.f;
   const float to_vox = fabsf(scale) * 0.5f * (float)((c == 0 ? full.s2 : (c == 1 ? full.s1 : full.s0)) - 1);
-  tp_rows<VEC>(coef + (int64_t)plane * G, T, full, i0, i1b, i1e, lds, [&](int i1, int x, const float (&val)[VEC]) {
+  tp_rows<VEC, WB>(coef + (int64_t)plane * G, T, full, i0, i1b, i1e, lds, [&](int i1, int x, const float (&val)[VEC]) {
     float o[VEC];
 #pragma unroll
     for (int q = 0; q < VEC; ++q) {
@@ -198,17 +302,19 @@
 
 constexpr int kGsFuseMax = 1024;
 struct GaussW9 { float w[9]; };
-template <int VEC>
+template <int VEC, int WB>
 __global__ void __launch_bounds__(kBlock)
 k_tp_interp_fwd_gs(const float* __restrict__ vel, float* __restrict__ s1, float* __restrict__ out, BandTables T, Dims full, int C,
-                   int add_identity, float scale, float* __restrict__ disp_out, GaussW9 gw, float gscale, int P) {
+                   int add_identity, float scale, float* __restrict__ disp_out, GaussW9 gw, float gscale, int P, int rows) {
   __shared__ float lds[kTpMaxLds];
   __shared__ float gs[2][kGsFuseMax];
   const int plane = blockIdx.z, i0 = blockIdx.y;
-  const int i1b = blockIdx.x * kTpChunk, i1e = min(i1b + kTpChunk, full.s1);
+  const int i1b = blockIdx.x * rows, i1e = min(i1b + rows, full.s1);
   const int g1 = T.a[1].g, g2 = T.a[2].g, Vg = g1 * g2;
   const int V = (int)full.voxels();
   const int c = plane % C;
+  TpReq<VEC, WB> rq;
+  if constexpr (WB != 0) rq.request(T, full, i0, i1b, i1e);
   {
     const float* src = vel + (int64_t)(plane % P) * Vg;
     const float sc = plane >= P ? -gscale : gscale;
@@ -236,7 +342,7 @@
   }
   float dmax = 0.f;
   const float to_vox = fabsf(scale) * 0.5f * (float)((c == 0 ? full.s2 : (c == 1 ? full.s1 : full.s0)) - 1);
-  tp_rows<VEC>(gs[0], T, full, i0, i1b, i1e, lds, [&](int i1, int x, const float (&val)[VEC]) {
+  tp_run<VEC, WB>(gs[0], T, full, i0, i1b, i1e, lds, rq, WB != 0, [&](int i1, int x, const float (&val)[VEC]) {
     float o[VEC];
 #pragma unroll
     for (int q = 0; q < VEC; ++q) {
@@ -668,7 +774,7 @@
   return 1.f + fminf(fmaxf(b, -eps), eps);
 }
 
-template <int VEC>
+template <int VEC, int WB>
 __global__ void __launch_bounds__(kBlock)
 k_bias_fwd(const float* __restrict__ cp, const float* __restrict__ data, float* __restrict__ out,
            float* __restrict__ field, BandTables T, Dims full, int C, float eps, int use_log, float cp_scale, int rows) {
@@ -677,7 +783,7 @@
   const int i1b = blockIdx.x * rows, i1e = min(i1b + rows, full.s1);
   const int64_t G = (int64_t)T.a[0].g * T.a[1].g * T.a[2].g;
   const int V = (int)full.voxels();
-  tp_rows<VEC>(cp + (int64_t)n * G, T, full, i0, i1b, i1e, lds, [&](int i1, int x, const float (&val)[VEC]) {
+  tp_rows<VEC, WB>(cp + (int64_t)n * G, T, full, i0, i1b, i1e, lds, [&](int i1, int x, const float (&val)[VEC]) {
     const int v = (i0 * full.s1 + i1) * full.s2 + x;
     float b[VEC];
 #pragma unroll
@@ -701,7 +807,7 @@
 }
 
 constexpr int kBiasRedWq = kBrMaxW / 4 / kBlock;
-template <int VEC, bool RED>
+template <int VEC, bool RED, int TW>
 __global__ void __launch_bounds__(kBlock)
 k_bias_bwd(const float* __restrict__ cp, const float* __restrict__ data, const float* __restrict__ gout,
            float* __restrict__ gL, float* __restrict__ gdata, BandTables T, Dims full, int C, float eps, int use_log,
@@ -729,7 +835,7 @@
     }
     if (threadIdx.x < g2) lo_r = lo_g[threadIdx.x];
   }
-  tp_rows<VEC>(cp + (int64_t)n * G, T, full, i0, i1b, i1e, lds, [&](int i1, int x, const float (&val)[VEC]) {
+  tp_rows<VEC, TW>(cp + (int64_t)n * G, T, full, i0, i1b, i1e, lds, [&](int i1, int x, const float (&val)[VEC]) {
     const int v = (i0 * full.s1 + i1) * full.s2 + x;
     float b[VEC], e[VEC], sgo[VEC];
     bool pass[VEC];
@@ -1472,6 +1578,14 @@
   return true;
 }
 
+static std::atomic<int> g_tp_wide{1};
+extern "C" int advchain_tp_wide_band(int64_t B2);
+static int tp_wide_band(const BandTables& T) {
+  return advchain_tp_wide_band(T.a[2].B);
+}
+#define TP_WIDE_GO(WB_, LAUNCH) \
+  switch (WB_) { case 2: { LAUNCH(2); } break; case 4: { LAUNCH(4); } break; default: { LAUNCH(0); } break; }
+
 template <class... ORD>
 static int tp_interp_fwd_launch(const float* coef, float* out, const int32_t* itab, const float* ftab,
                                 const int64_t* S, const int64_t* g, const int64_t* B, int64_t planes, int64_t C, int add_identity,
@@ -1499,17 +1613,23 @@
     return ADVCHAIN_OK;
   }
   *nwg = (int64_t)grid.x * grid.y * grid.z;
-  if (full.s2 % 4 == 0 && full.s2 >= 128 && (reinterpret_cast<uintptr_t>(out) & 15) == 0)
-    hipLaunchKernelGGL((k_tp_interp_fwd<4, ORD...>), grid, dim3(kBlock), 0, (hipStream_t)stream, coef, out, T, full, (int)C,
-                       add_identity, scale, sumsq, disp_out);
-  else
-    hipLaunchKernelGGL((k_tp_interp_fwd<1, ORD...>), grid, dim3(kBlock), 0, (hipStream_t)stream, coef, out, T, full, (int)C,
+  if (full.s2 % 4 == 0 && full.s2 >= 128 && (reinterpret_cast<uintptr_t>(out) & 15) == 0) {
+#define TP_GO(WB_) hipLaunchKernelGGL((k_tp_interp_fwd<4, WB_, ORD...>), grid, dim3(kBlock), 0, (hipStream_t)stream, coef, out, T, full, (int)C, \
+                                      add_identity, scale, sumsq, disp_out)
+    TP_WIDE_GO(tp_wide_band(T), TP_GO)
+#undef TP_GO
+  } else
+    hipLaunchKernelGGL((k_tp_interp_fwd<1, 0, ORD...>), grid, dim3(kBlock), 0, (hipStream_t)stream, coef, out, T, full, (int)C,
                        add_identity, scale, sumsq, disp_out);
   ADVCHAIN_LAUNCH_CHECK();
   return ADVCHAIN_OK;
 }
 
 extern "C" {
+
+void advchain_set_tp_wide_loads(int on) { g_tp_wide.store(on ? 1 : 0, std::memory_order_relaxed); }
+int advchain_get_tp_wide_loads(void) { return g_tp_wide.load(std::memory_order_relaxed); }
+int advchain_tp_wide_band(int64_t B2) { return (g_tp_wide.load(std::memory_order_relaxed) && (B2 == 2 || B2 == 4)) ? (int)B2 : 0; }
 
 int advchain_tp_interp_fwd(const float* coef, float* out, const int32_t* itab, const float* ftab, const int64_t* S,
                            const int64_t* g, const int64_t* B, int64_t planes, int64_t C, int ndim, int add_identity,
@@ -1538,11 +1658,14 @@
   return ADVCHAIN_OK;
 }
 
-int advchain_tp_interp_fwd_smoothed_pair(const float* vel, float* s1, float* out, const int32_t* itab, const float* ftab,
-                                         const int64_t* S, const int64_t* g, const int64_t* B, int64_t P, int64_t C,
-                                         int add_identity, float scale, float* disp_out, const float* weights9, float gscale,
-                                         void* stream) {
+int advchain_tp_interp_fwd_smoothed_pair_rows(const float* vel, float* s1, float* out, const int32_t* itab, const float* ftab,
+                                              const int64_t* S, const int64_t* g, const int64_t* B, int64_t P, int64_t C,
+                                              int add_identity, float scale, float* disp_out, const float* weights9, float gscale,
+                                              int rows_per_wg, void* stream) {
   ADVCHAIN_CHECK_ARG(vel && out && itab && ftab && weights9, "tp_interp_fwd_smoothed_pair: null pointer");
+  ADVCHAIN_CHECK_ARG(rows_per_wg == 0 || rows_per_wg == 4 || rows_per_wg == 8 || rows_per_wg == 16 || rows_per_wg == 32,
+                     "tp_interp_fwd_smoothed_pair: rows_per_wg must be 0, 4, 8, 16 or 32");
+  const int rows = rows_per_wg ? rows_per_wg : kTpChunk;
   ADVCHAIN_CHECK_ARG(P >= 0 && 2 * P < 65536 && C >= 1, "tp_interp_fwd_smoothed_pair: bad planes/C");
   BandTables T;
   ADVCHAIN_CHECK_ARG(unpack_tables(itab, ftab, S, g, B, T), "tp_interp_fwd_smoothed_pair: bad band tables");
@@ -1552,15 +1675,25 @@
   ADVCHAIN_CHECK_ARG(full.voxels() < (1ll << 31), "tp_interp_fwd_smoothed_pair: volume too large");
   GaussW9 gw;
   for (int k = 0; k < 9; ++k) gw.w[k] = weights9[k];
-  dim3 grid((unsigned)((full.s1 + kTpChunk - 1) / kTpChunk), 1u, (unsigned)(2 * P));
-  if (full.s2 % 4 == 0 && full.s2 >= 128 && (reinterpret_cast<uintptr_t>(out) & 15) == 0)
-    hipLaunchKernelGGL(k_tp_interp_fwd_gs<4>, grid, dim3(kBlock), 0, (hipStream_t)stream, vel, s1, out, T, full, (int)C, add_identity,
-                       scale, disp_out, gw, gscale, (int)P);
-  else
-    hipLaunchKernelGGL(k_tp_interp_fwd_gs<1>, grid, dim3(kBlock), 0, (hipStream_t)stream, vel, s1, out, T, full, (int)C, add_identity,
-                       scale, disp_out, gw, gscale, (int)P);
+  dim3 grid((unsigned)((full.s1 + rows - 1) / rows), 1u, (unsigned)(2 * P));
+  if (full.s2 % 4 == 0 && full.s2 >= 128 && (reinterpret_cast<uintptr_t>(out) & 15) == 0) {
+#define TP_GO(WB_) hipLaunchKernelGGL((k_tp_interp_fwd_gs<4, WB_>), grid, dim3(kBlock), 0, (hipStream_t)stream, vel, s1, out, T, full, (int)C, \
+                                      add_identity, scale, disp_out, gw, gscale, (int)P, rows)
+    TP_WIDE_GO(tp_wide_band(T), TP_GO)
+#undef TP_GO
+  } else
+    hipLaunchKernelGGL((k_tp_interp_fwd_gs<1, 0>), grid, dim3(kBlock), 0, (hipStream_t)stream, vel, s1, out, T, full, (int)C, add_identity,
+                       scale, disp_out, gw, gscale, (int)P, rows);
   ADVCHAIN_LAUNCH_CHECK();
   return ADVCHAIN_OK;
+}
+
+int advchain_tp_interp_fwd_smoothed_pair(const float* vel, float* s1, float* out, const int32_t* itab, const float* ftab,
+                                         const int64_t* S, const int64_t* g, const int64_t* B, int64_t P, int64_t C,
+                                         int add_identity, float scale, float* disp_out, const float* weights9, float gscale,
+                                         void* stream) {
+  return advchain_tp_interp_fwd_smoothed_pair_rows(vel, s1, out, itab, ftab, S, g, B, P, C, add_identity, scale, disp_out, weights9,
+                                                   gscale, 0, stream);
 }
 
 int advchain_band_reduce_axis(const float* in, const float* in2, float* out, const int32_t* itab, const float* ftab,
@@ -1671,11 +1804,13 @@
   const int rows = rows_per_wg ? rows_per_wg : bias_rows_rule(S[0], S[1], N);
   ADVCHAIN_CHECK_ARG(S[0] < 65536 && (S[1] + rows - 1) / rows < (1ll << 31), "bias_field_fwd: grid too large");
   dim3 grid((unsigned)((full.s1 + rows - 1) / rows), (unsigned)full.s0, (unsigned)N);
-  if (full.s2 % 4 == 0 && ((reinterpret_cast<uintptr_t>(data) | reinterpret_cast<uintptr_t>(out) | reinterpret_cast<uintptr_t>(field)) & 15) == 0)
-    hipLaunchKernelGGL(k_bias_fwd<4>, grid, dim3(kBlock), 0, (hipStream_t)stream, cp, data, out, field, T, full, (int)C, eps,
-                       use_log, cp_scale, rows);
-  else
-    hipLaunchKernelGGL(k_bias_fwd<1>, grid, dim3(kBlock), 0, (hipStream_t)stream, cp, data, out, field, T, full, (int)C, eps,
+  if (full.s2 % 4 == 0 && ((reinterpret_cast<uintptr_t>(data) | reinterpret_cast<uintptr_t>(out) | reinterpret_cast<uintptr_t>(field)) & 15) == 0) {
+#define TP_GO(WB_) hipLaunchKernelGGL((k_bias_fwd<4, WB_>), grid, dim3(kBlock), 0, (hipStream_t)stream, cp, data, out, field, T, full, (int)C, eps, \
+                                      use_log, cp_scale, rows)
+    TP_WIDE_GO(tp_wide_band(T), TP_GO)
+#undef TP_GO
+  } else
+    hipLaunchKernelGGL((k_bias_fwd<1, 0>), grid, dim3(kBlock), 0, (hipStream_t)stream, cp, data, out, field, T, full, (int)C, eps,
                        use_log, cp_scale, rows);
   ADVCHAIN_LAUNCH_CHECK();
   return ADVCHAIN_OK;
@@ -1705,11 +1840,13 @@
   ADVCHAIN_CHECK_ARG(S[0] < 65536 && (S[1] + rows - 1) / rows < (1ll << 31), "bias_field_bwd: grid too large");
   dim3 grid((unsigned)((full.s1 + rows - 1) / rows), (unsigned)full.s0, (unsigned)N);
   if (full.s2 % 4 == 0 && ((reinterpret_cast<uintptr_t>(data) | reinterpret_cast<uintptr_t>(grad_out) |
-                            reinterpret_cast<uintptr_t>(grad_L) | reinterpret_cast<uintptr_t>(grad_data)) & 15) == 0)
-    hipLaunchKernelGGL((k_bias_bwd<4, false>), grid, dim3(kBlock), 0, (hipStream_t)stream, cp, data, grad_out, grad_L, grad_data, T,
-                       full, (int)C, eps, use_log, cp_scale, rows, (float*)nullptr, (const float*)nullptr, (const int*)nullptr, 0);
-  else
-    hipLaunchKernelGGL((k_bias_bwd<1, false>), grid, dim3(kBlock), 0, (hipStream_t)stream, cp, data, grad_out, grad_L, grad_data, T,
+                            reinterpret_cast<uintptr_t>(grad_L) | reinterpret_cast<uintptr_t>(grad_data)) & 15) == 0) {
+#define TP_GO(WB_) hipLaunchKernelGGL((k_bias_bwd<4, false, WB_>), grid, dim3(kBlock), 0, (hipStream_t)stream, cp, data, grad_out, grad_L, grad_data, T, \
+                                      full, (int)C, eps, use_log, cp_scale, rows, (float*)nullptr, (const float*)nullptr, (const int*)nullptr, 0)
+    TP_WIDE_GO(tp_wide_band(T), TP_GO)
+#undef TP_GO
+  } else
+    hipLaunchKernelGGL((k_bias_bwd<1, false, 0>), grid, dim3(kBlock), 0, (hipStream_t)stream, cp, data, grad_out, grad_L, grad_data, T,
                        full, (int)C, eps, use_log, cp_scale, rows, (float*)nullptr, (const float*)nullptr, (const int*)nullptr, 0);
   ADVCHAIN_LAUNCH_CHECK();
   return ADVCHAIN_OK;
@@ -1748,8 +1885,10 @@
   ADVCHAIN_CHECK_ARG(full.voxels() < (1ll << 31), "bias_field_bwd_reduced: volume too large");
   ADVCHAIN_CHECK_ARG(S[0] < 65536 && (S[1] + rows - 1) / rows < (1ll << 31), "bias_field_bwd_reduced: grid too large");
   dim3 grid((unsigned)((full.s1 + rows - 1) / rows), (unsigned)full.s0, (unsigned)N);
-  hipLaunchKernelGGL((k_bias_bwd<4, true>), grid, dim3(kBlock), lds, (hipStream_t)stream, cp, data, grad_out, (float*)nullptr,
-                     grad_data, T, full, (int)C, eps, use_log, cp_scale, rows, t1, wd, (const int*)lo, (int)WB);
+#define TP_GO(WB_) hipLaunchKernelGGL((k_bias_bwd<4, true, WB_>), grid, dim3(kBlock), lds, (hipStream_t)stream, cp, data, grad_out, (float*)nullptr, \
+                                      grad_data, T, full, (int)C, eps, use_log, cp_scale, rows, t1, wd, (const int*)lo, (int)WB)
+  TP_WIDE_GO(tp_wide_band(T), TP_GO)
+#undef TP_GO
   ADVCHAIN_LAUNCH_CHECK();
   return ADVCHAIN_OK;
 }
diff --git a/advchain_amd/ops.py b/advchain_amd/ops.py
--- a/advchain_amd/ops.py
+++ b/advchain_amd/ops.py
@@ -190,6 +190,14 @@
 
 def is_deterministic():
     return bool(_lib.load().advchain_get_deterministic())
+
+
+def set_tp_wide_loads(on):
+    _lib.load().advchain_set_tp_wide_loads(1 if on else 0)
+
+
+def tp_wide_loads():
+    return bool(_lib.load().advchain_get_tp_wide_loads())
 
 
 def _scatter_workspace(N, dims, device):
diff --git a/include/advchain_hip.h b/include/advchain_hip.h
--- a/include/advchain_hip.h
+++ b/include/advchain_hip.h
@@ -120,11 +120,18 @@
                                          const int64_t* S, const int64_t* g, const int64_t* B, int64_t P, int64_t C,
                                          int add_identity, float scale, float* disp_out, const float* weights9, float gscale,
                                          void* stream);
+int advchain_tp_interp_fwd_smoothed_pair_rows(const float* vel, float* s1, float* out, const int32_t* itab, const float* ftab,
+                                              const int64_t* S, const int64_t* g, const int64_t* B, int64_t P, int64_t C,
+                                              int add_identity, float scale, float* disp_out, const float* weights9, float gscale,
+                                              int rows_per_wg, void* stream);
 int advchain_band_reduce_axis(const float* in, const float* in2, float* out, const int32_t* itab, const float* ftab,
                               const int64_t* S, const int64_t* g, const int64_t* B, int axis, int64_t outer,
                               int64_t inner, float scale, void* stream);
 int advchain_band_reduce_rows_dense(const float* in, const float* in2, float* out, const float* wd, const int32_t* lo,
                                     int64_t rows, int64_t S, int64_t g, int64_t WB, float scale, void* stream);
+void advchain_set_tp_wide_loads(int on);
+int advchain_get_tp_wide_loads(void);
+int advchain_tp_wide_band(int64_t B2);
 
 int advchain_bias_field_fwd(const float* cp, const float* data, float* out, float* field, const int32_t* itab,
                             const float* ftab, const int64_t* S, const int64_t* g, const int64_t* B, int64_t N,
```

Measured after the change: 4523 (median of 6 runs). 1.01x the previous value.
